# salesforce/ALPRO

Hardware: AMD Instinct MI355X
Metric: video-text pairs/sec (8f x 224^2, 40-tok) (higher is better)
Workload: dtype fp16

## Files before the change

alpro_amd/csrc/common.hpp:

```cpp
#pragma once
#include <hip/hip_runtime.h>
#include <stdint.h>

#include "../../include/alpro_hip.h"

namespace alpro {

typedef float f32x4 __attribute__((ext_vector_type(4)));
typedef uint32_t u32x4 __attribute__((ext_vector_type(4)));
typedef uint32_t u32x2 __attribute__((ext_vector_type(2)));
__device__ __forceinline__ u32x4 mk4(uint32_t a, uint32_t b, uint32_t c, uint32_t d) { return u32x4{a, b, c, d}; }
__device__ __forceinline__ u32x2 mk2(uint32_t a, uint32_t b) { return u32x2{a, b}; }
__device__ __forceinline__ float u2f(uint32_t u) { return __builtin_bit_cast(float, u); }
__device__ __forceinline__ uint32_t f2u(float f) { return __builtin_bit_cast(uint32_t, f); }
typedef float f32x16 __attribute__((ext_vector_type(16)));
typedef __bf16 bf16x8_t __attribute__((ext_vector_type(8)));
typedef _Float16 f16x8_t __attribute__((ext_vector_type(8)));

struct bf16_t { uint16_t v; };
struct f16_t { uint16_t v; };

__device__ __forceinline__ float to_f32(float x) { return x; }
__device__ __forceinline__ float to_f32(bf16_t x) { return __builtin_bit_cast(float, (uint32_t)x.v << 16); }
__device__ __forceinline__ float to_f32(f16_t x) { return (float)__builtin_bit_cast(_Float16, x.v); }
// ... 134 lines not shown
  const f32x2v cdf = {0.5f + copysignf(0.5f - h.x, x.x), 0.5f + copysignf(0.5f - h.y, x.y)};
  y = x * cdf;
  dy = cdf + x * (e * (f32x2v){0.39894228040143267794f, 0.39894228040143267794f});
}

__device__ __forceinline__ f32x2v gelu_fast2(f32x2v x) {
  const f32x2v z = (f32x2v){fabsf(x.x), fabsf(x.y)} * (f32x2v){0.70710678118654752440f, 0.70710678118654752440f};
  f32x2v q = z * (f32x2v){-0.00296695f, -0.00296695f} + (f32x2v){0.02966973f, 0.02966973f};
  q = z * q + (f32x2v){-0.14875628f, -0.14875628f};
  q = z * q + (f32x2v){-0.91847146f, -0.91847146f};
  q = z * q + (f32x2v){-1.62789348f, -1.62789348f};
  q = z * q + (f32x2v){-1.0f, -1.0f};
  const f32x2v h = {__builtin_amdgcn_exp2f(q.x), __builtin_amdgcn_exp2f(q.y)};
  const f32x2v cdf = {0.5f + copysignf(0.5f - h.x, x.x), 0.5f + copysignf(0.5f - h.y, x.y)};
  return x * cdf;
}

template <typename T> __device__ __forceinline__ void gelu_and_grad(float x, float& y, float& dy) {
  if constexpr (sizeof(T) == 4) {
    const float cdf = 0.5f * (1.0f + erff(x * 0.70710678118654752440f));
    y = x * cdf;
    dy = cdf + x * 0.39894228040143267794f * __expf(-0.5f * x * x);
  } else {
    const float h = half_erfc_pos(fabsf(x) * 0.70710678118654752440f);
    const float cdf = 0.5f + copysignf(0.5f - h, x);
    const float pdf = 0.39894228040143267794f * __builtin_amdgcn_exp2f(x * x * -0.72134752044448170368f);
    y = x * cdf;
    dy = cdf + x * pdf;
  }
}

__device__ __forceinline__ uint32_t mix32(uint32_t h) {
  h ^= h >> 16; h *= 0x7FEB352Du; h ^= h >> 15; h *= 0x846CA68Bu; h ^= h >> 16;
  return h;
}
__device__ __forceinline__ bool drop_keep(uint32_t seed, uint64_t idx, uint32_t thresh24) {
  const uint32_t h = mix32(seed ^ ((uint32_t)idx * 0x9E3779B1u) ^ ((uint32_t)(idx >> 32) * 0x85EBCA77u));
  return (h >> 8) >= thresh24;
}
__host__ __device__ inline uint32_t drop_thresh24(float p) { return (uint32_t)(p * 16777216.0f + 0.5f); }

__device__ __forceinline__ void dma16(const void* src, uint32_t lds_addr) {
#pragma clang diagnostic push
#pragma clang diagnostic ignored "-Winline-asm"
  asm volatile("s_mov_b32 m0, %1\n\ts_nop 0\n\tglobal_load_lds_dwordx4 %0, off" ::"v"(src), "s"(lds_addr) : "memory", "m0");
#pragma clang diagnostic pop
}
__device__ __forceinline__ void store16_sc1(void* p, const u32x4& v) {
  asm volatile("global_store_dwordx4 %0, %1, off sc1\n\ts_nop 1" ::"v"(p), "v"(v) : "memory");
}
__device__ __forceinline__ float sload_f32(const float* p, uint32_t idx) {
  return *((const __attribute__((address_space(4))) float*)p + __builtin_amdgcn_readfirstlane(idx));
}
__device__ __forceinline__ uint32_t lds_addr_of(const void* p) { return (uint32_t)(uintptr_t)(__attribute__((address_space(3))) const char*)p; }

void set_error(const char* fmt, ...);
int attn_long_fwd(const void* qkv, void* out, int dtype, int batch, int L, int H, float scale, const float* key_bias, float* lse, float drop_p,
                  uint32_t drop_seed, const float* cls_q, int cls_group, float* cls_out, hipStream_t st);
int attn_long_bwd(const void* qkv, const void* out, const void* dout, const float* lse, void* dqkv, int dtype, int batch, int L, int H, float scale,
                  const float* key_bias, float drop_p, uint32_t drop_seed, hipStream_t st);
int attn_temporal_any_fwd(const void* qkv, void* out, int dtype, int64_t rows, int T, int H, float scale, float* lse, hipStream_t st);
int attn_temporal_any_bwd(const void* qkv, const void* out, const void* dout, const float* lse, void* dqkv, int dtype, int64_t rows, int T, int H,
                          float scale, hipStream_t st);

__device__ __forceinline__ void attn_unit(int blk, int nblk, int H, int order, int& b, int& h) {
  const int batch = nblk / H;
  if (order == 1 && (batch & 7) == 0) {
    const int x = blk & 7, i = blk >> 3, j = i / H;
    h = i - j * H;
    b = j * 8 + x;
  } else {
    b = blk / H;
    h = blk - b * H;
  }
}
enum { OPT_GEMM_TILE = 0, OPT_GEMM_GRID = 1, OPT_GEMM_TUNE = 2, OPT_TN_SPLITS = 3, OPT_TN_KIND = 4, OPT_GEMM_TAIL = 5, OPT_ATTN_BWD = 6, OPT_ATTN_ORDER = 7, OPT_GEMM_KIND = 8, OPT_CU_BUDGET = 9, OPT_LN_GRID = 10, OPT_GEMM_SCHED = 11, OPT_GEMM_EPI = 12, OPT_COUNT = 13 };
int get_option(int which);
int get_stream_option(int which, hipStream_t st);

constexpr int SCHED_CLAIM0 = 8, SCHED_MAX_WG = 256, SCHED_BLOCK_U32 = SCHED_CLAIM0 + SCHED_MAX_WG;
struct TileSched {
  uint32_t* blk;
  uint32_t* prev;
  uint32_t magic_ntn;
  uint32_t epi;
};
struct SchedLaunch {
  uint32_t* cur = nullptr;
  uint32_t* prev = nullptr;
  void* slot = nullptr;
  SchedLaunch(hipStream_t st, bool enabled);
  void commit(bool launched);
  ~SchedLaunch();
};
int sched_set_workspace(hipStream_t st, void* ptr, size_t bytes);
inline uint32_t magic_u32(uint32_t d) { return (uint32_t)(((1ull << 32) + d - 1) / d); }
inline int cu_budget(hipStream_t st) {
  int v = get_stream_option(OPT_CU_BUDGET, st);
  if (v < 0) v = get_option(OPT_CU_BUDGET);
  return (v >= 64 && v < 256) ? (v / 8 * 8) : 256;
}

struct DeviceOnce {
  unsigned long long mask = 0;
  template <typename F> void run(F&& f) {
    int dev = 0;
    (void)hipGetDevice(&dev);
    const unsigned long long bit = 1ull << (dev & 63);
    if (!(__atomic_load_n(&mask, __ATOMIC_ACQUIRE) & bit)) {
      f();
      __atomic_fetch_or(&mask, bit, __ATOMIC_RELEASE);
    }
  }
};
template <typename K> void set_lds_once(DeviceOnce& once, K* kern, size_t lds) {
  once.run([&] { (void)hipFuncSetAttribute((const void*)kern, hipFuncAttributeMaxDynamicSharedMemorySize, (int)lds); });
}
#define ALPRO_CHECK(cond, ...)            \
  do {                                    \
    if (!(cond)) {                        \
      alpro::set_error(__VA_ARGS__);      \
      return ALPRO_ERR_INVALID;           \
    }                                     \
  } while (0)
int check_launch(const char* what);

#define ALPRO_DISPATCH_DTYPE(dt, T, ...)                                         \
  switch (dt) {                                                                  \
    case ALPRO_F32: { typedef float T; __VA_ARGS__; break; }                     \
    case ALPRO_BF16: { typedef alpro::bf16_t T; __VA_ARGS__; break; }            \
    case ALPRO_F16: { typedef alpro::f16_t T; __VA_ARGS__; break; }              \
    default: alpro::set_error("bad dtype %d", (int)(dt)); return ALPRO_ERR_INVALID; \
  }

}
```

alpro_amd/csrc/core.hip:

```cpp
#include <stdarg.h>
#include <stdio.h>
#include <stdlib.h>
#include <string.h>

#include "common.hpp"

namespace alpro {

static thread_local char g_err[512] = "";

void set_error(const char* fmt, ...) {
  va_list ap;
  va_start(ap, fmt);
  vsnprintf(g_err, sizeof(g_err), fmt, ap);
  va_end(ap);
}

namespace {
const char* const kOptNames[OPT_COUNT] = {"gemm_tile", "gemm_grid", "gemm_tune", "tn_splits", "tn_kind", "gemm_tail", "attn_bwd", "attn_order", "gemm_kind", "cu_budget", "ln_grid", "gemm_sched", "gemm_epi"};
const char* const kOptEnv[OPT_COUNT] = {"ALPRO_GEMM_TILE", "ALPRO_GEMM_GRID", "ALPRO_GEMM_TUNE", "ALPRO_TN_SPLITS", "ALPRO_TN_KIND", "ALPRO_GEMM_TAIL", "ALPRO_ATTN_BWD", "ALPRO_ATTN_ORDER", "ALPRO_GEMM_KIND", "ALPRO_CU_BUDGET", "ALPRO_LN_GRID", "ALPRO_GEMM_SCHED", "ALPRO_GEMM_EPI"};
int g_opts[OPT_COUNT];
bool option_allowed(int which, int value) {
#ifdef ALPRO_ABLATIONS
  (void)which; (void)value;
// ... 757 lines not shown
    ALPRO_ADD_LN_CASE(ALPRO_ADD_PRE_MLP)
    ALPRO_ADD_LN_CASE(ALPRO_ADD_PRE_TEMPORAL)
  }
#undef ALPRO_ADD_LN_CASE
  return check_launch("alpro_add_layernorm_fwd");
}
}

extern "C" int alpro_add_layernorm_fwd(const float* x_in, const void* delta, int dtype, const float* delta_bias, int add_mode, float* x_out,
                                       const float* gamma, const float* beta, float eps, void* y, float* y32, int64_t rows, int D, int p0, int p1,
                                       void* stream) {
  ALPRO_CHECK(x_in && delta && gamma && beta && y && rows > 0, "alpro_add_layernorm_fwd: bad args");
  ALPRO_CHECK(D == LN_D, "alpro_add_layernorm_fwd: D=%d unsupported (hidden size is 768 on this path)", D);
  ALPRO_CHECK(add_mode >= ALPRO_ADD_IDENTITY && add_mode <= ALPRO_ADD_PRE_TEMPORAL, "alpro_add_layernorm_fwd: bad add_mode %d", add_mode);
  ALPRO_CHECK(add_mode == ALPRO_ADD_IDENTITY || (p0 > 0 && p1 > 0), "alpro_add_layernorm_fwd: the divided space-time modes need p0 = T, p1 = N");
  ALPRO_CHECK(add_mode == ALPRO_ADD_IDENTITY || rows % (add_mode == ALPRO_ADD_PRE_SPATIAL ? (int64_t)p0 * (p1 + 1) : 1 + (int64_t)p0 * p1) == 0,
              "alpro_add_layernorm_fwd: rows=%lld is not a whole number of clips", (long long)rows);
  ALPRO_CHECK(!(dtype == ALPRO_F32 && y32), "alpro_add_layernorm_fwd: y already is fp32 in exact mode");
  ALPRO_CHECK(((uintptr_t)x_in % 16) == 0 && ((uintptr_t)delta % 16) == 0 && ((uintptr_t)y % 16) == 0, "alpro_add_layernorm_fwd: pointers must be 16-byte aligned");
  ALPRO_DISPATCH_DTYPE(dtype, T, return launch_add_ln<T>(add_mode, x_in, delta, delta_bias, x_out, gamma, beta, eps, y, y32, rows, p0, p1, (hipStream_t)stream));
  return ALPRO_OK;
}

extern "C" int alpro_add_layernorm_pre_mlp2(const float* x_in, const void* delta_t, const float* delta_t_bias, const void* delta_s, int dtype, float* x_out,
                                            const float* gamma, const float* beta, float eps, void* y, int64_t rows, int D, int T, int N, void* stream) {
  ALPRO_CHECK(x_in && delta_t && delta_s && gamma && beta && y && rows > 0, "alpro_add_layernorm_pre_mlp2: bad args");
  ALPRO_CHECK(D == LN_D, "alpro_add_layernorm_pre_mlp2: D=%d unsupported (hidden size is 768 on this path)", D);
  ALPRO_CHECK(T > 0 && N > 0 && rows % (1 + (int64_t)T * N) == 0, "alpro_add_layernorm_pre_mlp2: rows=%lld is not a whole number of clips of 1 + %d x %d tokens", (long long)rows, N, T);
  ALPRO_CHECK(((uintptr_t)x_in % 16) == 0 && ((uintptr_t)delta_t % 16) == 0 && ((uintptr_t)delta_s % 16) == 0 && ((uintptr_t)y % 16) == 0,
              "alpro_add_layernorm_pre_mlp2: pointers must be 16-byte aligned");
  const dim3 grid(grid_for(rows, 4, 256 * 32)), blk(256);
  ALPRO_DISPATCH_DTYPE(dtype, T_, hipLaunchKernelGGL((add_layernorm_fwd_kernel<T_, ALPRO_ADD_PRE_MLP>), grid, blk, 0, (hipStream_t)stream, x_in, (const T_*)delta_s,
                                                     (const float*)nullptr, x_out, gamma, beta, eps, (T_*)y, (float*)nullptr, rows, T, N, (const T_*)delta_t, delta_t_bias));
  return check_launch("alpro_add_layernorm_pre_mlp2");
}

extern "C" int alpro_vit_final_pool(const float* x, const float* gamma, const float* beta, float eps, float* out32, void* out_t,
                                    int dtype, int B, int T, int N, int D, void* stream) {
  ALPRO_CHECK(x && gamma && beta && out32 && B > 0 && T > 0 && N > 0, "alpro_vit_final_pool: bad args");
  ALPRO_CHECK(D == LN_D, "alpro_vit_final_pool: D=%d unsupported", D);
  const int64_t total = (int64_t)B * (N + 1);
  ALPRO_DISPATCH_DTYPE(dtype, T_, hipLaunchKernelGGL(vit_final_pool_kernel<T_>, dim3((unsigned)((total + 3) / 4)), dim3(256), 0, (hipStream_t)stream, x, gamma, beta, eps, out32, (T_*)out_t, B, T, N));
  return check_launch("alpro_vit_final_pool");
}

extern "C" int alpro_bert_embed_fwd(const int64_t* ids, const float* word, const float* pos, const float* type0,
                                    const float* gamma, const float* beta, float eps, float* y32, void* y_t, int dtype,
                                    float* mean, float* rstd, int rows, int L, int D, float drop_p, uint32_t drop_seed, void* stream) {
  ALPRO_CHECK(ids && word && pos && type0 && gamma && beta && y32 && rows > 0 && L > 0, "alpro_bert_embed_fwd: bad args");
  ALPRO_CHECK(D == LN_D, "alpro_bert_embed_fwd: D=%d unsupported", D);
  ALPRO_DISPATCH_DTYPE(dtype, T, hipLaunchKernelGGL(bert_embed_kernel<T>, dim3((rows + 3) / 4), dim3(256), 0, (hipStream_t)stream, ids, word, pos, type0, gamma, beta, eps, y32, (T*)y_t, mean, rstd, rows, L, drop_p, drop_seed));
  return check_launch("alpro_bert_embed_fwd");
}
```

alpro_amd/csrc/gemm.hip:

```cpp
#include <stdarg.h>
#include <stdio.h>
#include <stdlib.h>

#include <type_traits>

#include "common.hpp"

namespace alpro {

namespace {
constexpr int BM = 128, BN = 128, ROWB = 128, NT = 256;
constexpr int TILE_BYTES = BM * ROWB;

__device__ __forceinline__ int lds_off(int row, int chunk) { return row * ROWB + ((chunk ^ ((row >> 1) & 7)) << 4); }

struct RowDst {
  int64_t out, res;
  bool side;
};
template <int mode>
__device__ __forceinline__ RowDst map_row(int p0, int p1, int m) {
  RowDst d;
  d.side = false;
  if (mode == ALPRO_MAP_IDENTITY) {
// ... 227 lines not shown
    }
    if (ACT == ALPRO_ACT_GELU_BWD || ACT == ALPRO_ACT_MUL_SAVED) {
      float pre[8];
      unpack_chunk<T>(pre_c2 ? pre_c2[p] : *(const u32x4*)((const T*)g.C2 + m * g.ldc2 + n), pre);
#pragma unroll
      for (int e = 0; e < 8; ++e) v[e] *= (ACT == ALPRO_ACT_MUL_SAVED) ? pre[e] : gelu_grad<T>(pre[e]);
    }
    if constexpr (ACT == ALPRO_ACT_GELU && sizeof(T) == 2) {
#pragma unroll
      for (int e = 0; e < 8; e += 2) {
        const f32x2v yy = gelu_fast2((f32x2v){v[e], v[e + 1]});
        v[e] = yy.x * rs;
        v[e + 1] = yy.y * rs;
      }
    } else {
#pragma unroll
      for (int e = 0; e < 8; ++e) v[e] = apply_act<T, ACT>(v[e]) * rs;
    }
    if (g.drop_seed) {
      float dp = g.drop_p;
      asm volatile("" : "+s"(dp));
      const uint32_t th = drop_thresh24(dp);
      const float ks = 1.0f / (1.0f - dp);
      const uint64_t i0 = (uint64_t)(g.m_off + m) * (uint64_t)g.N + (uint64_t)n;
#pragma unroll
      for (int e = 0; e < 8; ++e) v[e] = drop_keep(g.drop_seed, i0 + e, th) ? v[e] * ks : 0.f;
    }
    if constexpr (RES) {
      if (g.residual) {
        const f32x4 r0 = __builtin_nontemporal_load((const f32x4*)(g.residual + m * g.ldr + n)), r1 = __builtin_nontemporal_load((const f32x4*)(g.residual + m * g.ldr + n + 4));
        v[0] += r0.x; v[1] += r0.y; v[2] += r0.z; v[3] += r0.w; v[4] += r1.x; v[5] += r1.y; v[6] += r1.z; v[7] += r1.w;
      }
    }
    if (ABL == 1) {
      u32x4 keep = pack_chunk<T>(v);
      asm volatile("" ::"v"(keep));
    } else {
      __builtin_nontemporal_store(pack_chunk<T>(v), (u32x4*)((T*)g.C + m * g.ldc + n));
    }
  }
}

__device__ __forceinline__ bool epi_fast_ok(const alpro_gemm_desc_t& g, int m_base, int rows, int n_base) {
  return (m_base + rows <= g.M) && (n_base + 64 <= g.N) && ((g.ldc & 3) == 0) && (!g.residual || (g.ldr & 3) == 0) &&
         ((g.ld_side & 3) == 0);
}

__device__ __forceinline__ void load_bias4(const alpro_gemm_desc_t& g, int n, float (&bias)[4]) {
#pragma unroll
  for (int e = 0; e < 4; ++e) bias[e] = (g.bias && n + e < g.N) ? g.bias[n + e] : 0.f;
}

template <typename T, int ACT, int MAP>
__device__ __forceinline__ void gemm_nt_tile(const alpro_gemm_desc_t& g, const int bid, char* smem) {
  const int tid = threadIdx.x, lane = tid & 63, wave = tid >> 6;
  const int wr = wave >> 1, wc = wave & 1;
  const int ntn = (g.N + BN - 1) / BN, ntm = (g.M + BM - 1) / BM;
  const int nblk = ntn * ntm;
  if (bid >= nblk) return;
  int tile;
  {
    const int xcd = bid & 7, idx = bid >> 3;
    const int q = nblk >> 3, r = nblk & 7;
    tile = (xcd < r ? xcd * (q + 1) : r * (q + 1) + (xcd - r) * q) + idx;
  }
  const int tm = tile / ntn, tn = tile - tm * ntn;
  const int m0 = tm * BM, n0 = tn * BN;

  const char* Ab = (const char*)g.A;
  const char* Wb = (const char*)g.W;
  const int64_t lda_b = g.lda * (int64_t)sizeof(T), ldw_b = g.ldw * (int64_t)sizeof(T);

  const char* a_src[4];
  const char* w_src[4];
  int st_off[4];
#pragma unroll
  for (int i = 0; i < 4; ++i) {
    const int c = tid + i * NT, row = c >> 3, ch = c & 7;
    const int am = min(m0 + row, g.M - 1), wn = min(n0 + row, g.N - 1);
    a_src[i] = Ab + am * lda_b + ch * 16;
    w_src[i] = Wb + wn * ldw_b + ch * 16;
    st_off[i] = lds_off(row, ch);
  }
  int a_row[2], b_row[2];
#pragma unroll
  for (int i = 0; i < 2; ++i) {
    a_row[i] = wr * 64 + i * 32 + (lane & 31);
    b_row[i] = wc * 64 + i * 32 + (lane & 31);
  }
  const int khalf = lane >> 5;

  f32x16 acc[2][2];
#pragma unroll
  for (int i = 0; i < 2; ++i)
#pragma unroll
    for (int j = 0; j < 2; ++j)
#pragma unroll
      for (int r = 0; r < 16; ++r) acc[i][j][r] = 0.f;

  const int nk = (g.K * (int)sizeof(T)) / ROWB;
  u32x4 ra[4], rw[4];
#pragma unroll
  for (int i = 0; i < 4; ++i) {
    ra[i] = *(const u32x4*)(a_src[i]);
    rw[i] = *(const u32x4*)(w_src[i]);
  }
  char* bufA = smem;
  char* bufW = smem + 2 * TILE_BYTES;
#pragma unroll
  for (int i = 0; i < 4; ++i) {
    *(u32x4*)(bufA + st_off[i]) = ra[i];
    *(u32x4*)(bufW + st_off[i]) = rw[i];
  }
  __syncthreads();

  int cur = 0;
  for (int kt = 0; kt < nk; ++kt) {
    {
      const int64_t ko = (int64_t)min(kt + 1, nk - 1) * ROWB;
#pragma unroll
// ... 5 lines not shown
    __builtin_amdgcn_sched_barrier(0);
    const char* cA = bufA + cur * TILE_BYTES;
    const char* cW = bufW + cur * TILE_BYTES;
#pragma unroll
    for (int s = 0; s < 4; ++s) {
      u32x4 fa[2], fb[2];
#pragma unroll
      for (int i = 0; i < 2; ++i) {
        fa[i] = *(const u32x4*)(cA + lds_off(a_row[i], 2 * s + khalf));
        fb[i] = *(const u32x4*)(cW + lds_off(b_row[i], 2 * s + khalf));
      }
#pragma unroll
      for (int i = 0; i < 2; ++i)
#pragma unroll
        for (int j = 0; j < 2; ++j) mma_chunk<T>(acc[i][j], fa[i], fb[j]);
    }
    __builtin_amdgcn_sched_barrier(0);
    {
      char* nA = bufA + (cur ^ 1) * TILE_BYTES;
      char* nW = bufW + (cur ^ 1) * TILE_BYTES;
#pragma unroll
      for (int i = 0; i < 4; ++i) {
        *(u32x4*)(nA + st_off[i]) = ra[i];
        *(u32x4*)(nW + st_off[i]) = rw[i];
      }
    }
    __syncthreads();
    cur ^= 1;
  }

  float* stage = (float*)(smem + wave * (64 * 64 * 4));
#pragma unroll
  for (int r = 0; r < 16; ++r) {
    const int row = acc_row(r, lane), col = lane & 31;
    stage[row * 64 + col] = acc[0][0][r];
    stage[row * 64 + 32 + col] = acc[0][1][r];
    stage[(32 + row) * 64 + col] = acc[1][0][r];
    stage[(32 + row) * 64 + 32 + col] = acc[1][1][r];
  }
  wave_lds_sync();
  const int mb = m0 + wr * 64, nb = n0 + wc * 64;
  float bias[4];
  load_bias4(g, nb + (lane & 15) * 4, bias);
  if (epi_fast_ok(g, mb, 64, nb)) {
#pragma unroll
    for (int c = 0; c < 4; ++c) epi_rows16<T, ACT, MAP, true>(g, stage + c * 16 * 64, mb + c * 16, nb, lane, bias);
  } else {
#pragma unroll 1
    for (int c = 0; c < 4; ++c) epi_rows16<T, ACT, MAP, false>(g, stage + c * 16 * 64, mb + c * 16, nb, lane, bias);
  }
}

template <typename T, int ACT, int MAP>
__global__ __launch_bounds__(NT, 2) void gemm_nt_kernel(const alpro_gemm_desc_t g) {
  extern __shared__ __attribute__((aligned(16))) char smem[];
  gemm_nt_tile<T, ACT, MAP>(g, blockIdx.x, smem);
}

template <typename T, int ACT, int MAP>
__global__ __launch_bounds__(NT, 2) void gemm_nt_batch_kernel(const alpro_gemm_desc_t* __restrict__ descs) {
  extern __shared__ __attribute__((aligned(16))) char smem[];
  const alpro_gemm_desc_t g = descs[blockIdx.y];
  gemm_nt_tile<T, ACT, MAP>(g, blockIdx.x, smem);
}

constexpr int BM2 = 256, BN2 = 256, NT2 = 512;
constexpr int TILE2_BYTES = BM2 * ROWB;

constexpr int EPI_BYTES = 8 * 16 * 64 * 4;

__device__ __forceinline__ constexpr int copy_slot(int tune, int q, int pos) {
  if (tune == 0) return ((q & 1) && ((q >> 1) & 1) == pos) ? (q >> 2) : -1;
  if (tune == 1 || tune >= 3) { const int r = q - 1 - pos; return (r >= 0 && r < 16 && (r & 1) == 0) ? (r >> 1) : -1; }
  const int r = q - 1 - pos;
  return (r >= 0 && r < 24 && r % 3 == 0) ? r / 3 : -1;
}

template <typename T, int ACT, int MAP, int TUNE = 1>
__global__ __launch_bounds__(NT2, 2) void gemm_nt256p_kernel(const alpro_gemm_desc_t g, const int tail_split) {
  extern __shared__ __attribute__((aligned(16))) char smem[];
  const int tid = threadIdx.x, lane = tid & 63, wave = __builtin_amdgcn_readfirstlane(tid >> 6);
  const int wr = wave >> 2, wc = wave & 3;
  const int ntn = (g.N + BN2 - 1) / BN2, ntm = (g.M + BM2 - 1) / BM2;
  const int nblk = ntn * ntm;
  const int64_t lda_b = g.lda * (int64_t)sizeof(T), ldw_b = g.ldw * (int64_t)sizeof(T);
  const int nk = (g.K * (int)sizeof(T)) / ROWB;
  const int per_xcd = (gridDim.x + 7) >> 3;
  const int slot = (blockIdx.x & 7) * per_xcd + (blockIdx.x >> 3);
  typedef __attribute__((address_space(3))) void* lds_ptr;
  typedef const __attribute__((address_space(1))) void* gbl_ptr;

  const char* a_src[4];
  const char* w_src[4];
  int m0 = 0, n0 = 0;
  const int G = gridDim.x;
  const int q_full = nblk / G, rem = nblk - q_full * G;
  const bool split = tail_split && rem > 0 && 2 * rem <= G;
  auto locate = [&](int it, int& t, int& hf) -> bool {
    hf = -1;
    if (it < q_full) { t = slot + it * G; return true; }
    if (it > q_full) return false;
    if (split) {
      if (slot >= 2 * rem) return false;
      t = q_full * G + (slot >> 1);
      hf = slot & 1;
      return true;
    }
    t = q_full * G + slot;
    return slot < rem;
  };
  auto setup = [&](int tile, int hf) {
    const int tm = tile / ntn, tn = tile - tm * ntn;
    m0 = tm * BM2 + (hf > 0 ? BM2 / 2 : 0);
    n0 = tn * BN2;
#pragma unroll
    for (int i = 0; i < 4; ++i) {
      const int row = (wave + 8 * i) * 8 + (lane >> 3);
      const int ch = (lane & 7) ^ ((row >> 1) & 7);
      a_src[i] = (const char*)g.A + min(m0 + row, g.M - 1) * lda_b + ch * 16;
      w_src[i] = (const char*)g.W + min(n0 + row, g.N - 1) * ldw_b + ch * 16;
    }
  };
  const uint32_t lds_base = lds_addr_of(smem);
  auto copy_piece = [&](int c, int kt, int buf, bool half_a = false) {
    const int i = c >> 1;
    if (half_a && !(c & 1) && i >= 2) return;
    const char* src = ((c & 1) ? w_src[i] : a_src[i]) + (int64_t)kt * ROWB;
    dma16(src, __builtin_amdgcn_readfirstlane(lds_base + buf * 2 * TILE2_BYTES + (c & 1) * TILE2_BYTES + (wave + 8 * i) * 1024));
  };
  auto stage_tile = [&](int kt, int buf, bool half_a = false) {
#pragma unroll
    for (int c = 0; c < 8; ++c) copy_piece(c, kt, buf, half_a);
  };
  int a_row[4], b_row[2];
#pragma unroll
  for (int i = 0; i < 4; ++i) a_row[i] = wr * 128 + i * 32 + (lane & 31);
#pragma unroll
  for (int j = 0; j < 2; ++j) b_row[j] = wc * 64 + j * 32 + (lane & 31);
  const int khalf = lane >> 5;
  float* stage = (float*)(smem + 4 * TILE2_BYTES + wave * (16 * 64 * 4));

  int it = 0, tile, hf;
  if (!locate(0, tile, hf)) return;
  const int pos = wave >> 2;
  auto wait_vm0 = [] { asm volatile("s_waitcnt vmcnt(0)" ::: "memory"); };
  auto block_sync = [] {
    asm volatile("s_waitcnt lgkmcnt(0)" ::: "memory");
    __builtin_amdgcn_s_barrier();
    asm volatile("" ::: "memory");
  };
  setup(tile, hf);
  int s0 = 0;
  stage_tile(0, 0, hf >= 0);
  stage_tile(1, 1, hf >= 0);
  wait_vm0();
  while (true) {
    const int tm0 = m0, tn0 = n0;
    int next, next_hf;
    const bool more = locate(it + 1, next, next_hf);
    const bool active = hf < 0 || wr == 0;
    f32x16 acc[4][2];
#pragma unroll
    for (int i = 0; i < 4; ++i)
#pragma unroll
      for (int j = 0; j < 2; ++j)
// ... 139 lines not shown
      }
    }
    if (!more) break;
    tile = next;
    hf = next_hf;
    ++it;
    setup(tile, hf);
  }
}


static bool q_kernel_takes(const alpro_gemm_desc_t& g, bool* ragged_in_kernel) {
  constexpr int BM2q = 256, BN2q = 256;
  if (g.dtype == ALPRO_F32 || g.map_mode != ALPRO_MAP_IDENTITY) return false;
  const int m_full = g.M / BM2q * BM2q, m_rem = g.M - m_full;
  const bool c16 = g.c_dtype != ALPRO_F32 && (g.ldc & 7) == 0 && (!g.C2 || g.c2_tiled || (g.ldc2 & 7) == 0) && (!g.residual || (g.ldr & 3) == 0) && ((uintptr_t)g.C % 16) == 0 &&
                   (!g.row_scale || g.row_scale_group >= 8);
  const bool c32 = g.c_dtype == ALPRO_F32 && g.act == ALPRO_ACT_NONE && !g.C2 && !g.drop_seed && (g.ldc & 3) == 0 && (!g.residual || ((g.ldr & 3) == 0 && ((uintptr_t)g.residual % 16) == 0)) &&
                   ((uintptr_t)g.C % 16) == 0 && (!g.row_scale || g.row_scale_group >= 16);
  const bool shape = (g.N % BN2q) == 0 && ((g.lda * 2) % 128) == 0 && ((g.ldw * 2) % 128) == 0 && (g.K % 128) == 0 && g.K >= 256 &&
                     (int64_t)g.M * g.lda * 2 < (int64_t)0xFFFF0000 && (int64_t)g.N * g.ldw * 2 < (int64_t)0xFFFF0000;
  *ragged_in_kernel = m_rem > 0 && (m_rem % 16) == 0;
  const int full_tiles = (g.N / BN2q) * (m_full / BM2q);
  const int force = get_option(OPT_GEMM_TILE);
  return get_option(OPT_GEMM_KIND) == 1 && (c16 || c32) && shape && (force ? force == 256 : full_tiles >= 160);
}
static bool c2_tiled_ok(const alpro_gemm_desc_t& g) {
  const int m_rem = g.M % 256;
  return (g.act == ALPRO_ACT_GELU_SAVE_GRAD || g.act == ALPRO_ACT_MUL_SAVED) && g.C2 && ((uintptr_t)g.C2 % 16) == 0 && g.c_dtype != ALPRO_F32 && !g.residual && !g.row_scale &&
         !g.drop_seed && (m_rem % 16) == 0;
}

constexpr int HALF2_BYTES = 128 * ROWB;
constexpr int STAGE2_BYTES = 4 * HALF2_BYTES;

template <typename T> struct Mma16;
template <> struct Mma16<bf16_t> {
  static __device__ __forceinline__ f32x4 run(const u32x4& a, const u32x4& b, const f32x4& c) {
    return __builtin_amdgcn_mfma_f32_16x16x32_bf16(__builtin_bit_cast(bf16x8_t, a), __builtin_bit_cast(bf16x8_t, b), c, 0, 0, 0);
  }
};
template <> struct Mma16<f16_t> {
  static __device__ __forceinline__ f32x4 run(const u32x4& a, const u32x4& b, const f32x4& c) {
    return __builtin_amdgcn_mfma_f32_16x16x32_f16(__builtin_bit_cast(f16x8_t, a), __builtin_bit_cast(f16x8_t, b), c, 0, 0, 0);
  }
};

template <typename T, int ACT, int MAP>
__global__ __launch_bounds__(NT2, 2) __attribute__((amdgpu_num_vgpr(127))) void gemm_nt256q_kernel(const alpro_gemm_desc_t g, const TileSched sc) {
  static_assert(sizeof(T) == 2, "16-bit operands only");
  extern __shared__ __attribute__((aligned(16))) char smem[];
  const int tid = threadIdx.x, lane = tid & 63, wave = __builtin_amdgcn_readfirstlane(tid >> 6);
  const int wr = wave >> 2, wc = wave & 3;
  const int ntn = (g.N + BN2 - 1) / BN2, ntm = (g.M + BM2 - 1) / BM2;
  const int nblk = ntn * ntm;
  const int64_t lda_b = g.lda * 2, ldw_b = g.ldw * 2;
  const int nk = g.K >> 6;
  const uint32_t lds_base = lds_addr_of(smem);

  const uint32_t p = gridDim.x >> 3;
  const uint64_t t_start = wall_clock64();
  constexpr uint32_t RESCUE_TICKS = 1000;
  auto list_tile = [&](int y, uint32_t j) -> int {
    const uint32_t t = ((j >> 5) << 8) + ((uint32_t)y << 5) + (j & 31u);
    return (j < 0x100000u && t < (uint32_t)nblk) ? (int)t : -1;
  };
  auto list_len = [&](int y) -> int {
    const int rem = (nblk & 255) - 32 * y;
    return (nblk >> 8) * 32 + (rem < 0 ? 0 : (rem > 32 ? 32 : rem));
  };
  typedef __attribute__((address_space(3))) volatile int lds_int_t;
  lds_int_t* mbox = (lds_int_t*)(__attribute__((address_space(3))) char*)(smem + STAGE2_BYTES + HALF2_BYTES);
  uint32_t wstate = sc.blk ? 0u : (uint32_t)(blockIdx.x >> 3) + 2 * p;
  int quota = 0;
  bool pending = false;
  if (sc.blk) {
    const int mine = list_len((int)(blockIdx.x & 7u)) - (int)(2 * p);
    quota = mine > 0 ? (mine + (int)p - 1) / (int)p : 0;
  }
  auto ticket_issue = [&](uint32_t& r, bool on) {
    uint64_t sv;
    const uint32_t m = (uint32_t)__builtin_amdgcn_readfirstlane(on ? 1 : 0);
    asm volatile("s_mov_b64 %1, exec\n\ts_mov_b32 exec_lo, %5\n\ts_mov_b32 exec_hi, 0\n\tglobal_atomic_add %0, %2, %3, %4 sc0\n\ts_mov_b64 exec, %1"
                 : "+v"(r), "=&s"(sv) : "v"(((blockIdx.x + wstate) & 7u) * 4u), "v"(1u), "s"(sc.blk), "s"(m) : "memory");
  };
  auto claim_issue = [&](uint32_t& r, uint32_t w, uint32_t bits, bool on) {
    uint64_t sv;
    const uint32_t m = (uint32_t)__builtin_amdgcn_readfirstlane(on ? 1 : 0);
    asm volatile("s_mov_b64 %1, exec\n\ts_mov_b32 exec_lo, %5\n\ts_mov_b32 exec_hi, 0\n\tglobal_atomic_or %0, %2, %3, %4 sc0\n\ts_mov_b64 exec, %1"
                 : "+v"(r), "=&s"(sv) : "v"((SCHED_CLAIM0 + w) * 4u), "v"(bits), "s"(sc.blk), "s"(m) : "memory");
  };
  auto ticket_issue_tk = [&](bool on) {
    uint64_t sv;
    const uint32_t m = (uint32_t)__builtin_amdgcn_readfirstlane(on ? 1 : 0);
#pragma clang diagnostic push
#pragma clang diagnostic ignored "-Winline-asm"
    asm volatile("s_mov_b64 %0, exec\n\ts_mov_b32 exec_lo, %4\n\ts_mov_b32 exec_hi, 0\n\tglobal_atomic_add v255, %1, %2, %3 sc0\n\ts_mov_b64 exec, %0"
                 : "=&s"(sv) : "v"(((blockIdx.x + wstate) & 7u) * 4u), "v"(1u), "s"(sc.blk), "s"(m) : "memory", "v255");
#pragma clang diagnostic pop
  };
  auto claim_issue_tk = [&](uint32_t w, uint32_t bits, bool on) {
    uint64_t sv;
    const uint32_t m = (uint32_t)__builtin_amdgcn_readfirstlane(on ? 1 : 0);
#pragma clang diagnostic push
#pragma clang diagnostic ignored "-Winline-asm"
    asm volatile("s_mov_b64 %0, exec\n\ts_mov_b32 exec_lo, %4\n\ts_mov_b32 exec_hi, 0\n\tglobal_atomic_or v255, %1, %2, %3 sc0\n\ts_mov_b64 exec, %0"
                 : "=&s"(sv) : "v"((SCHED_CLAIM0 + w) * 4u), "v"(bits), "s"(sc.blk), "s"(m) : "memory", "v255");
// ... 37 lines not shown
          asm volatile("s_waitcnt vmcnt(0)" ::: "memory");
          a = list_tile(y, 2 * p + __builtin_amdgcn_readfirstlane(k0));
          continue;
        }
        const uint32_t w0 = 4u * lane;
        const uint32_t words[4] = {clm.x, clm.y, clm.z, clm.w};
        uint64_t open[8];
        int total = 0;
#pragma unroll
        for (int sl = 0; sl < 8; ++sl) {
          open[sl] = __builtin_amdgcn_ballot_w64(w0 + (sl >> 1) < gridDim.x && ((words[sl >> 1] >> (sl & 1)) & 1u) == 0u);
          total += __builtin_popcountll(open[sl]);
        }
        if (total == 0) break;
        while ((uint32_t)(wall_clock64() - t_start) < RESCUE_TICKS) __builtin_amdgcn_s_sleep(8);
        int q = (int)(((blockIdx.x + 1u) * 0x9E3779B1u >> 12) % (uint32_t)total);
        uint32_t w = 0, bit = 0;
#pragma unroll
        for (int sl = 0; sl < 8; ++sl) {
          const int n = __builtin_popcountll(open[sl]);
          if (bit == 0 && q < n) {
            uint64_t msk = open[sl];
            for (int i = 0; i < q; ++i) msk &= msk - 1;
            w = 4u * (uint32_t)__builtin_ctzll(msk) + (uint32_t)(sl >> 1);
            bit = 1u << (sl & 1);
          }
          q -= n;
        }
        uint32_t old = 3;
        claim_issue(old, w, bit, true);
        asm volatile("s_waitcnt vmcnt(0)" ::: "memory");
        if ((__builtin_amdgcn_readfirstlane(old) & bit) == 0) a = list_tile((int)(w & 7u), (w >> 3) + (bit == 2u ? p : 0u));
      }
      const int b = -1;
      mbox[0] = a;
      mbox[1] = b;
    }
    asm volatile("s_waitcnt lgkmcnt(0)" ::: "memory");
    __builtin_amdgcn_s_barrier();
    asm volatile("" ::: "memory");
    t0 = __builtin_amdgcn_readfirstlane(mbox[0]);
    t1 = __builtin_amdgcn_readfirstlane(mbox[1]);
  };

  const int r0 = wave * 16 + (lane >> 3);
  const uint32_t sw0 = (uint32_t)(((lane & 7) ^ ((r0 >> 1) & 7)) << 4);
  uint32_t oa[2], ow[2][2];
#pragma unroll
  for (int i = 0; i < 2; ++i) {
    oa[i] = (uint32_t)((r0 + i * 8) * lda_b) + (sw0 ^ (uint32_t)(i * 64));
#pragma unroll
    for (int h = 0; h < 2; ++h) ow[h][i] = (uint32_t)((r0 + h * 128 + i * 8) * ldw_b) + (sw0 ^ (uint32_t)(i * 64));
  }
  struct Tile { const char* a[2]; const char* w; };
  auto tile_base = [&](int tile) {
    const int tm = ntn == 1 ? tile : (int)__umulhi((uint32_t)tile, sc.magic_ntn), tn = tile - tm * ntn;
    const int vr = g.M - tm * BM2;
    const char* a0 = (const char*)g.A + (int64_t)tm * BM2 * lda_b;
    Tile t;
#pragma unroll
    for (int h = 0; h < 2; ++h) t.a[h] = a0 + (int64_t)((h * 128 + wave * 16 < vr) ? h * 128 : -(wave * 16)) * lda_b;
    t.w = (const char*)g.W + (int64_t)tn * BN2 * ldw_b;
    return t;
  };
  auto copy_half = [&](const char* kbase, int hs, int par) {
#pragma unroll
    for (int i = 0; i < 2; ++i) {
      const uint32_t vo = hs < 2 ? oa[i] : ow[hs & 1][i];
      const uint32_t dst = __builtin_amdgcn_readfirstlane(lds_base + par * STAGE2_BYTES + hs * HALF2_BYTES + (wave * 2 + i) * 1024);
#pragma clang diagnostic push
#pragma clang diagnostic ignored "-Winline-asm"
      asm volatile("s_mov_b32 m0, %2\n\ts_nop 0\n\tglobal_load_lds_dwordx4 %0, %1" ::"v"(vo), "s"(kbase), "s"(dst) : "memory", "m0");
#pragma clang diagnostic pop
    }
  };
  const int l15 = lane & 15, kg = lane >> 4;
  const int frag0 = l15 * ROWB + ((kg ^ ((l15 >> 1) & 7)) << 4);
  const char* aF[2] = {smem + wr * HALF2_BYTES + frag0, smem + wr * HALF2_BYTES + (frag0 ^ 64)};
  const char* bF[2] = {smem + (2 + (wc >> 1)) * HALF2_BYTES + (wc & 1) * 64 * ROWB + frag0,
                       smem + (2 + (wc >> 1)) * HALF2_BYTES + (wc & 1) * 64 * ROWB + (frag0 ^ 64)};
  float* stage = (float*)(smem + 2 * STAGE2_BYTES + wave * (16 * 64 * 4));

  auto barrier = [] {
    __builtin_amdgcn_sched_barrier(0);
    __builtin_amdgcn_s_barrier();
    __builtin_amdgcn_sched_barrier(0);
  };

  int cur_t = list_tile((int)(blockIdx.x & 7u), blockIdx.x >> 3), nxt_t = list_tile((int)(blockIdx.x & 7u), (blockIdx.x >> 3) + p);
  if (sc.prev && blockIdx.x == 0 && wave == 0) {
#pragma unroll
    for (int i = 0; i < (SCHED_BLOCK_U32 + 63) / 64; ++i)
      if (i * 64 + lane < SCHED_BLOCK_U32) sc.prev[i * 64 + lane] = 0u;
  }
  claim_issue_tk(blockIdx.x, 3u, wave == 0 && sc.blk);
  bool fresh = sc.blk != nullptr;
  bool have = cur_t >= 0;
  while (true) {
  if (!have) {
    if (!sc.blk) break;
    fresh = false;
    asm volatile("s_waitcnt vmcnt(0)" ::: "memory");
    steal(cur_t, nxt_t);
    if (cur_t < 0) break;
    quota = 0;
  }
  have = false;
  Tile cur = tile_base(cur_t);
  Tile nxt = tile_base(nxt_t >= 0 ? nxt_t : cur_t);
#pragma unroll
  for (int hs = 0; hs < 4; ++hs) copy_half(hs < 2 ? cur.a[hs] : cur.w, hs, 0);
  copy_half(cur.w + ROWB, 2, 1);
  asm volatile("s_waitcnt vmcnt(0)" ::: "memory");
  if (fresh && wave == 0) {
    mbox[0] = (int)(tk_read() & 3u);
    asm volatile("s_waitcnt lgkmcnt(0)" ::: "memory");
  }
  barrier();
  if (fresh) {
    fresh = false;
    const int gone = __builtin_amdgcn_readfirstlane(mbox[0]);
    if (gone) {
      barrier();
      int t0 = (gone & 1) ? -1 : cur_t, t1 = (gone & 2) ? -1 : nxt_t;
      if (t0 < 0) { t0 = t1; t1 = -1; }
      cur_t = t0;
      nxt_t = t1;
      have = cur_t >= 0;
      continue;
    }
  }
  pending = sc.blk && nxt_t >= 0 && quota > 0;
  quota -= pending ? 1 : 0;
  ticket_issue_tk(wave == 0 && pending);

  while (true) {
    const int tile = cur_t;
    const int tm0 = (ntn == 1 ? tile : (int)__umulhi((uint32_t)tile, sc.magic_ntn)) * BM2, tn0 = (tile - (tm0 >> 8) * ntn) * BN2;
    f32x4 acc[8][4];
#pragma unroll
    for (int i = 0; i < 8; ++i)
#pragma unroll
      for (int j = 0; j < 4; ++j) acc[i][j] = f32x4{0.f, 0.f, 0.f, 0.f};
    if (wr == 1) barrier();

    auto ktile = [&](auto par_tag, int t) {
      constexpr int P = decltype(par_tag)::value;
      u32x4 fa[4][2], fb[2][2][2];
      const bool in1 = t + 1 < nk, in2 = t + 2 < nk;
      const int k1 = in1 ? t + 1 : 0, k2 = in2 ? t + 2 : t + 2 - nk;
      const char* a10 = (in1 ? cur.a[0] : nxt.a[0]) + (int64_t)k1 * ROWB;
      const char* a11 = (in1 ? cur.a[1] : nxt.a[1]) + (int64_t)k1 * ROWB;
      const char* w1 = (in1 ? cur.w : nxt.w) + (int64_t)k1 * ROWB;
      const char* w2 = (in2 ? cur.w : nxt.w) + (int64_t)k2 * ROWB;
      auto load_a = [&](int mi) {
#pragma unroll
        for (int f = 0; f < 4; ++f)
#pragma unroll
          for (int ks = 0; ks < 2; ++ks) fa[f][ks] = *(const u32x4*)(aF[ks] + P * STAGE2_BYTES + (mi * 64 + f * 16) * ROWB);
      };
      auto load_b = [&](int ni) {
#pragma unroll
        for (int f = 0; f < 2; ++f)
#pragma unroll
          for (int ks = 0; ks < 2; ++ks) fb[ni][f][ks] = *(const u32x4*)(bF[ks] + P * STAGE2_BYTES + (ni * 32 + f * 16) * ROWB);
      };
      auto mma = [&](int mi, int ni) {
        __builtin_amdgcn_s_setprio(1);
#pragma unroll
        for (int ks = 0; ks < 2; ++ks)
#pragma unroll
          for (int f = 0; f < 4; ++f)
#pragma unroll
            for (int e = 0; e < 2; ++e) acc[mi * 4 + f][ni * 2 + e] = Mma16<T>::run(fa[f][ks], fb[ni][e][ks], acc[mi * 4 + f][ni * 2 + e]);
        __builtin_amdgcn_s_setprio(0);
      };
      load_b(0);
      load_a(0);
      copy_half(a10, 0, P ^ 1);
      barrier();
      mma(0, 0);
      barrier();
      load_b(1);
      copy_half(a11, 1, P ^ 1);
      barrier();
      mma(0, 1);
      barrier();
      load_a(1);
      copy_half(w1, 3, P ^ 1);
      barrier();
      mma(1, 1);
// ... 207 lines not shown
            for (int mf = 0; mf < 8; ++mf) {
              if (!rows_ok(mf)) break;
              if constexpr (HAS_RES) {
                if (mf + PD < 8 && rows_ok(mf + PD)) load_res(mf + PD, ring[(mf + PD) % RING]);
              }
              float rs_lo = 1.0f, rs_hi = 1.0f;
              uint32_t edge = 0;
              if (g.row_scale) {
                const uint32_t m0 = (uint32_t)g.m_off + (uint32_t)(mb + mf * 16);
                const uint32_t gi = (uint32_t)__builtin_amdgcn_readfirstlane((int)(m0 / (uint32_t)g.row_scale_group));
                edge = (gi + 1) * (uint32_t)g.row_scale_group;
                rs_lo = sload_f32(g.row_scale, gi);
                rs_hi = sload_f32(g.row_scale, edge < (uint32_t)g.m_off + (uint32_t)g.M ? gi + 1 : gi);
              }
              stage_rows(mf);
#pragma unroll
              for (int j = 0; j < 4; ++j) {
                const int row = r0e + 4 * j;
                const int64_t m = mb + mf * 16 + row;
                const float4 a = *(const float4*)(stage + row * 64 + c4);
                const float rs = ((uint32_t)g.m_off + (uint32_t)m) >= edge ? rs_hi : rs_lo;
                f32x4 v = {(g.alpha * a.x + bias4[0]) * rs, (g.alpha * a.y + bias4[1]) * rs, (g.alpha * a.z + bias4[2]) * rs, (g.alpha * a.w + bias4[3]) * rs};
                if constexpr (HAS_RES) v += ring[mf % RING][j];
                __builtin_nontemporal_store(v, (f32x4*)(Cf + m * g.ldc + nb + c4));
              }
              if constexpr (!HAS_RES) {
                if (mf == 0) early_ticket();
              }
            }
          };
          if (g.residual) f32_rows(std::true_type{});
          else f32_rows(std::false_type{});
        }
      }
    }
    if (nxt_t < 0) break;
    cur = nxt;
    cur_t = nxt_t;
    nxt_t = __builtin_amdgcn_readfirstlane(mbox[0]);
    nxt = tile_base(nxt_t >= 0 ? nxt_t : cur_t);
    if (!early) {
      pending = sc.blk && nxt_t >= 0 && quota > 0;
      quota -= pending ? 1 : 0;
      ticket_issue_tk(wave == 0 && pending);
    }
  }
  asm volatile("s_waitcnt vmcnt(0)" ::: "memory");
  cur_t = -1;
  }
  asm volatile("s_waitcnt vmcnt(0)" ::: "memory");
}

template <typename T, int ACT, int MAP>
int launch_gemm_inst(const alpro_gemm_desc_t& g, hipStream_t st) {
  static DeviceOnce attr_once;
  attr_once.run([&] {
    (void)hipFuncSetAttribute((const void*)gemm_nt_kernel<T, ACT, MAP>, hipFuncAttributeMaxDynamicSharedMemorySize, 4 * TILE_BYTES);
    (void)hipFuncSetAttribute((const void*)gemm_nt256p_kernel<T, ACT, MAP>, hipFuncAttributeMaxDynamicSharedMemorySize, 4 * TILE2_BYTES + EPI_BYTES);
    if constexpr (std::is_same<T, bf16_t>::value && ACT == ALPRO_ACT_NONE && MAP == ALPRO_MAP_IDENTITY) {
      (void)hipFuncSetAttribute((const void*)gemm_nt256p_kernel<T, ACT, MAP, 1>, hipFuncAttributeMaxDynamicSharedMemorySize, 4 * TILE2_BYTES + EPI_BYTES);
      (void)hipFuncSetAttribute((const void*)gemm_nt256p_kernel<T, ACT, MAP, 2>, hipFuncAttributeMaxDynamicSharedMemorySize, 4 * TILE2_BYTES + EPI_BYTES);
#ifdef ALPRO_ABLATIONS
      (void)hipFuncSetAttribute((const void*)gemm_nt256p_kernel<T, ACT, MAP, 3>, hipFuncAttributeMaxDynamicSharedMemorySize, 4 * TILE2_BYTES + EPI_BYTES);
      (void)hipFuncSetAttribute((const void*)gemm_nt256p_kernel<T, ACT, MAP, 4>, hipFuncAttributeMaxDynamicSharedMemorySize, 4 * TILE2_BYTES + EPI_BYTES);
      (void)hipFuncSetAttribute((const void*)gemm_nt256p_kernel<T, ACT, MAP, 12>, hipFuncAttributeMaxDynamicSharedMemorySize, 4 * TILE2_BYTES + EPI_BYTES);
      (void)hipFuncSetAttribute((const void*)gemm_nt256p_kernel<T, ACT, MAP, 11>, hipFuncAttributeMaxDynamicSharedMemorySize, 4 * TILE2_BYTES + EPI_BYTES);
      (void)hipFuncSetAttribute((const void*)gemm_nt256p_kernel<T, ACT, MAP, 10>, hipFuncAttributeMaxDynamicSharedMemorySize, 4 * TILE2_BYTES + EPI_BYTES);
      (void)hipFuncSetAttribute((const void*)gemm_nt256p_kernel<T, ACT, MAP, 5>, hipFuncAttributeMaxDynamicSharedMemorySize, 4 * TILE2_BYTES + EPI_BYTES);
      (void)hipFuncSetAttribute((const void*)gemm_nt256p_kernel<T, ACT, MAP, 6>, hipFuncAttributeMaxDynamicSharedMemorySize, 4 * TILE2_BYTES + EPI_BYTES);
#endif
    }
  });
  const int big_tiles = ((g.N + BN2 - 1) / BN2) * ((g.M + BM2 - 1) / BM2);
  const int force = get_option(OPT_GEMM_TILE);
  const int nk = (g.K * (int)sizeof(T)) / ROWB;
  const bool use256 = nk >= 2 && (force ? force == 256 : big_tiles >= 160);
  if constexpr (sizeof(T) == 2 && MAP == ALPRO_MAP_IDENTITY) {
    static DeviceOnce attr_q;
    attr_q.run([&] {
      (void)hipFuncSetAttribute((const void*)gemm_nt256q_kernel<T, ACT, MAP>, hipFuncAttributeMaxDynamicSharedMemorySize, 2 * STAGE2_BYTES + EPI_BYTES);
    });
    const int m_full = g.M / BM2 * BM2, m_rem = g.M - m_full;
    bool ragged_in_kernel = false;
    const bool take_q = q_kernel_takes(g, &ragged_in_kernel);
    ALPRO_CHECK(!g.c2_tiled || (take_q && c2_tiled_ok(g)), "alpro_gemm: c2_tiled is not available for this descriptor (M=%d N=%d K=%d act=%d): ask alpro_gemm_c2_tiled_rows first", g.M, g.N, g.K, g.act);
    if (take_q) {
      alpro_gemm_desc_t gq = g;
      if (!ragged_in_kernel) gq.M = m_full;
      int grid = cu_budget(st);
      if (const int cap = get_option(OPT_GEMM_GRID)) grid = cap < grid ? (cap + 7) / 8 * 8 : grid;
      const int ntn_q = g.N / BN2, ntm_q = (gq.M + BM2 - 1) / BM2;
      const int tiles = ntn_q * ntm_q;
      int tail_panels = 0;
      if (get_option(OPT_GEMM_TAIL) == 1 && !g.c2_tiled && tiles > grid && g.K >= 2048) {
        const int R = tiles % grid;
        if (R > 0 && 5 * R <= 2 * grid) tail_panels = (R + ntn_q - 1) / ntn_q;
      }
      int64_t m_tail0 = -1;
      if (tail_panels > 0 && tail_panels < ntm_q) {
        m_tail0 = (int64_t)(ntm_q - tail_panels) * BM2;
        gq.M = (int)m_tail0;
      } else if (m_rem && !ragged_in_kernel) {
        m_tail0 = m_full;
      }
      TileSched sc;
      sc.blk = sc.prev = nullptr;
      sc.magic_ntn = magic_u32((uint32_t)(g.N / BN2));
      sc.epi = (uint32_t)get_option(OPT_GEMM_EPI);
      {
        SchedLaunch blocks(get_option(OPT_GEMM_SCHED) == 1 ? st : nullptr, get_option(OPT_GEMM_SCHED) == 1);
        sc.blk = blocks.cur;
        sc.prev = blocks.prev;
        hipLaunchKernelGGL((gemm_nt256q_kernel<T, ACT, MAP>), dim3(grid), dim3(NT2), 2 * STAGE2_BYTES + EPI_BYTES, st, gq, sc);
        blocks.commit(hipPeekAtLastError() == hipSuccess);
      }
      if (m_tail0 >= 0) {
        alpro_gemm_desc_t gr = g;
        gr.M = (int)(g.M - m_tail0);
        gr.A = (const char*)g.A + m_tail0 * g.lda * 2;
        gr.C = (char*)g.C + m_tail0 * g.ldc * (g.c_dtype == ALPRO_F32 ? 4 : 2);
        gr.m_off = g.m_off + m_tail0;
        if (g.C2) gr.C2 = (char*)g.C2 + m_tail0 * g.ldc2 * 2;
        if (g.residual) gr.residual = g.residual + m_tail0 * g.ldr;
        const int ntn = (gr.N + BN - 1) / BN, ntm = (gr.M + BM - 1) / BM;
        hipLaunchKernelGGL((gemm_nt_kernel<T, ACT, MAP>), dim3(ntn * ntm), dim3(NT), 4 * TILE_BYTES, st, gr);
      }
      return check_launch("alpro_gemm");
    }
  }
  if (use256) {
    const int cus = cu_budget(st);
    int grid = big_tiles < cus ? (big_tiles + 7) / 8 * 8 : cus;
    if (const int cap = get_option(OPT_GEMM_GRID)) grid = cap < grid ? (cap + 7) / 8 * 8 : grid;
    const int tune = get_option(OPT_GEMM_TUNE);
    const int tail = get_option(OPT_GEMM_TAIL);
    if constexpr (std::is_same<T, bf16_t>::value && ACT == ALPRO_ACT_NONE && MAP == ALPRO_MAP_IDENTITY) {
      if (tune == 0) { hipLaunchKernelGGL((gemm_nt256p_kernel<T, ACT, MAP, 0>), dim3(grid), dim3(NT2), 4 * TILE2_BYTES + EPI_BYTES, st, g, tail); return check_launch("alpro_gemm"); }
      if (tune == 2) { hipLaunchKernelGGL((gemm_nt256p_kernel<T, ACT, MAP, 2>), dim3(grid), dim3(NT2), 4 * TILE2_BYTES + EPI_BYTES, st, g, tail); return check_launch("alpro_gemm"); }
#ifdef ALPRO_ABLATIONS
      if (tune == 3) { hipLaunchKernelGGL((gemm_nt256p_kernel<T, ACT, MAP, 3>), dim3(grid), dim3(NT2), 4 * TILE2_BYTES + EPI_BYTES, st, g, tail); return check_launch("alpro_gemm"); }
      if (tune == 4) { hipLaunchKernelGGL((gemm_nt256p_kernel<T, ACT, MAP, 4>), dim3(grid), dim3(NT2), 4 * TILE2_BYTES + EPI_BYTES, st, g, tail); return check_launch("alpro_gemm"); }
      if (tune == 12) { hipLaunchKernelGGL((gemm_nt256p_kernel<T, ACT, MAP, 12>), dim3(grid), dim3(NT2), 4 * TILE2_BYTES + EPI_BYTES, st, g, tail); return check_launch("alpro_gemm"); }
      if (tune == 11) { hipLaunchKernelGGL((gemm_nt256p_kernel<T, ACT, MAP, 11>), dim3(grid), dim3(NT2), 4 * TILE2_BYTES + EPI_BYTES, st, g, tail); return check_launch("alpro_gemm"); }
      if (tune == 10) { hipLaunchKernelGGL((gemm_nt256p_kernel<T, ACT, MAP, 10>), dim3(grid), dim3(NT2), 4 * TILE2_BYTES + EPI_BYTES, st, g, tail); return check_launch("alpro_gemm"); }
      if (tune == 5) { hipLaunchKernelGGL((gemm_nt256p_kernel<T, ACT, MAP, 5>), dim3(grid), dim3(NT2), 4 * TILE2_BYTES + EPI_BYTES, st, g, tail); return check_launch("alpro_gemm"); }
      if (tune == 6) { hipLaunchKernelGGL((gemm_nt256p_kernel<T, ACT, MAP, 6>), dim3(grid), dim3(NT2), 4 * TILE2_BYTES + EPI_BYTES, st, g, tail); return check_launch("alpro_gemm"); }
#endif
    }
    hipLaunchKernelGGL((gemm_nt256p_kernel<T, ACT, MAP>), dim3(grid), dim3(NT2), 4 * TILE2_BYTES + EPI_BYTES, st, g, tail);
  } else {
    const int ntn = (g.N + BN - 1) / BN, ntm = (g.M + BM - 1) / BM;
    hipLaunchKernelGGL((gemm_nt_kernel<T, ACT, MAP>), dim3(ntn * ntm), dim3(NT), 4 * TILE_BYTES, st, g);
  }
  return check_launch("alpro_gemm");
}

template <typename T>
int launch_gemm(const alpro_gemm_desc_t& g, hipStream_t st) {
#ifdef ALPRO_ISA_QUICK
  return g.act == ALPRO_ACT_MUL_SAVED ? launch_gemm_inst<T, ALPRO_ACT_MUL_SAVED, ALPRO_MAP_IDENTITY>(g, st) : launch_gemm_inst<T, ALPRO_ACT_NONE, ALPRO_MAP_IDENTITY>(g, st);
#else
  if (g.act != ALPRO_ACT_NONE) {
    if (g.map_mode != ALPRO_MAP_IDENTITY) {
      set_error("alpro_gemm: an activation cannot be combined with a row map");
      return ALPRO_ERR_INVALID;
    }
    if (g.act == ALPRO_ACT_GELU_BWD) return launch_gemm_inst<T, ALPRO_ACT_GELU_BWD, ALPRO_MAP_IDENTITY>(g, st);
    if (g.act == ALPRO_ACT_GELU_SAVE_GRAD) return launch_gemm_inst<T, ALPRO_ACT_GELU_SAVE_GRAD, ALPRO_MAP_IDENTITY>(g, st);
    if (g.act == ALPRO_ACT_MUL_SAVED) return launch_gemm_inst<T, ALPRO_ACT_MUL_SAVED, ALPRO_MAP_IDENTITY>(g, st);
    return g.act == ALPRO_ACT_GELU ? launch_gemm_inst<T, ALPRO_ACT_GELU, ALPRO_MAP_IDENTITY>(g, st)
                                   : launch_gemm_inst<T, ALPRO_ACT_RELU, ALPRO_MAP_IDENTITY>(g, st);
  }
  switch (g.map_mode) {
    case ALPRO_MAP_IDENTITY: return launch_gemm_inst<T, ALPRO_ACT_NONE, ALPRO_MAP_IDENTITY>(g, st);
    case ALPRO_MAP_SKIP_CLS: return launch_gemm_inst<T, ALPRO_ACT_NONE, ALPRO_MAP_SKIP_CLS>(g, st);
    case ALPRO_MAP_FRAME_TOKENS: return launch_gemm_inst<T, ALPRO_ACT_NONE, ALPRO_MAP_FRAME_TOKENS>(g, st);
    default: return launch_gemm_inst<T, ALPRO_ACT_NONE, ALPRO_MAP_PATCH_EMBED>(g, st);
  }
#endif
}
}
}

namespace alpro {
namespace {
template <typename T>
int launch_gemm_batch(const alpro_gemm_desc_t* descs_dev, int njobs, int max_tiles, int with_residual_map, hipStream_t st) {
  (void)with_residual_map;
  static DeviceOnce attr_once;
  attr_once.run([&] {
    (void)hipFuncSetAttribute((const void*)gemm_nt_batch_kernel<T, ALPRO_ACT_NONE, ALPRO_MAP_IDENTITY>, hipFuncAttributeMaxDynamicSharedMemorySize, 4 * TILE_BYTES);
  });
  hipLaunchKernelGGL((gemm_nt_batch_kernel<T, ALPRO_ACT_NONE, ALPRO_MAP_IDENTITY>), dim3(max_tiles, njobs), dim3(NT), 4 * TILE_BYTES, st, descs_dev);
  return check_launch("alpro_gemm_batch");
}
}
}

static int check_gemm_desc(const alpro_gemm_desc_t* d);

extern "C" int alpro_gemm_batch(const alpro_gemm_desc_t* descs_host, const alpro_gemm_desc_t* descs_device, int njobs, void* stream) {
  using namespace alpro;
  ALPRO_CHECK(descs_host && descs_device && njobs > 0, "alpro_gemm_batch: bad args");
  int max_tiles = 0;
  for (int i = 0; i < njobs; ++i) {
    const alpro_gemm_desc_t* d = descs_host + i;
    if (const int rc = check_gemm_desc(d)) return rc;
    ALPRO_CHECK(d->dtype == descs_host[0].dtype, "alpro_gemm_batch: all jobs must share the operand dtype");
    ALPRO_CHECK(d->act == ALPRO_ACT_NONE && d->map_mode == ALPRO_MAP_IDENTITY && !d->drop_seed && !d->bias2 && !d->C2,
                "alpro_gemm_batch: plain epilogues only (bias, alpha, row scale, fp32 residual)");
    const int t = ((d->N + BN - 1) / BN) * ((d->M + BM - 1) / BM);
    max_tiles = t > max_tiles ? t : max_tiles;
  }
  ALPRO_DISPATCH_DTYPE(descs_host[0].dtype, T, return launch_gemm_batch<T>(descs_device, njobs, max_tiles, 0, (hipStream_t)stream));
  return ALPRO_OK;
}

static int check_gemm_desc(const alpro_gemm_desc_t* d) {
  using namespace alpro;
  ALPRO_CHECK(d && d->A && d->W && d->C, "alpro_gemm: null operand");
  ALPRO_CHECK(d->M > 0 && d->N > 0 && d->K > 0, "alpro_gemm: bad shape M=%d N=%d K=%d", d->M, d->N, d->K);
  const int esz = d->dtype == ALPRO_F32 ? 4 : 2;
  ALPRO_CHECK((d->K * esz) % 128 == 0, "alpro_gemm: K=%d must be a multiple of %d for dtype %d", d->K, 128 / esz, d->dtype);
  ALPRO_CHECK((d->lda * esz) % 16 == 0 && (d->ldw * esz) % 16 == 0, "alpro_gemm: lda/ldw must keep rows 16-byte aligned");
  ALPRO_CHECK(((uintptr_t)d->A % 16) == 0 && ((uintptr_t)d->W % 16) == 0, "alpro_gemm: A/W must be 16-byte aligned");
  ALPRO_CHECK(d->c_dtype == d->dtype || d->c_dtype == ALPRO_F32, "alpro_gemm: c_dtype must be dtype or F32");
  ALPRO_CHECK(d->map_mode >= 0 && d->map_mode <= 3, "alpro_gemm: bad map_mode %d", d->map_mode);
  ALPRO_CHECK(d->act >= 0 && d->act <= ALPRO_ACT_MUL_SAVED, "alpro_gemm: bad act %d", d->act);
  ALPRO_CHECK(!d->bias2 || d->map_mode == ALPRO_MAP_SKIP_CLS, "alpro_gemm: bias2 is only defined under the SKIP_CLS map");
  ALPRO_CHECK((d->act != ALPRO_ACT_GELU_BWD && d->act != ALPRO_ACT_MUL_SAVED && d->act != ALPRO_ACT_GELU_SAVE_GRAD) || (d->C2 && d->N % 8 == 0 && (d->c2_tiled || d->ldc2 % 8 == 0)),
              "alpro_gemm: GELU_BWD / MUL_SAVED / GELU_SAVE_GRAD need the C2 buffer (N, ldc2 multiples of 8)");
  ALPRO_CHECK(!d->drop_seed || (d->map_mode == ALPRO_MAP_IDENTITY && d->drop_p > 0.f && d->drop_p < 1.f), "alpro_gemm: dropout needs the identity map and 0 < p < 1");
  ALPRO_CHECK(!d->C2 || (d->N % 4 == 0 && (d->c2_tiled || d->ldc2 % 4 == 0) && d->ldc % 4 == 0), "alpro_gemm: C2 needs N, ldc, ldc2 multiples of 4");
  ALPRO_CHECK(!d->c2_tiled || d->act == ALPRO_ACT_GELU_SAVE_GRAD || d->act == ALPRO_ACT_MUL_SAVED, "alpro_gemm: c2_tiled is for GELU_SAVE_GRAD / MUL_SAVED only");
  ALPRO_CHECK(d->map_mode != ALPRO_MAP_FRAME_TOKENS || d->side, "alpro_gemm: FRAME_TOKENS needs a side buffer");
  ALPRO_CHECK(!d->row_scale || d->row_scale_group > 0, "alpro_gemm: row_scale_group must be > 0");
  return ALPRO_OK;
}

extern "C" int64_t alpro_gemm_c2_tiled_rows(int64_t M, int64_t N, int64_t K, int dtype) {
  using namespace alpro;
  if (M <= 0 || N <= 0 || K <= 0 || M > 0x7fffffff || N > 0x7fffffff || K > 0x7fffffff || (dtype != ALPRO_F16 && dtype != ALPRO_BF16)) return 0;
  alpro_gemm_desc_t g = {};
  g.A = g.W = (const void*)(uintptr_t)256;
  g.C = g.C2 = (void*)(uintptr_t)256;
  g.M = (int)M; g.N = (int)N; g.K = (int)K;
  g.lda = g.ldw = K; g.ldc = N;
  g.dtype = g.c_dtype = dtype;
  g.act = ALPRO_ACT_GELU_SAVE_GRAD;
  g.c2_tiled = 1;
  bool ragged = false;
  return (q_kernel_takes(g, &ragged) && c2_tiled_ok(g)) ? (M + 255) / 256 * 256 : 0;
}

extern "C" int alpro_gemm(const alpro_gemm_desc_t* d, void* stream) {
  using namespace alpro;
  if (const int rc = check_gemm_desc(d)) return rc;
#ifdef ALPRO_ISA_QUICK
  return launch_gemm<f16_t>(*d, (hipStream_t)stream);
#else
  ALPRO_DISPATCH_DTYPE(d->dtype, T, return launch_gemm<T>(*d, (hipStream_t)stream));
  return ALPRO_OK;
#endif
}
```

alpro_amd/csrc/gemm_tn.hip:

```cpp
#include "common.hpp"

namespace alpro {
namespace {

constexpr int TM = 32;
constexpr int NSTAGE = 4;
constexpr int TW = 256;
constexpr int ROW_BYTES = TW * 2;
constexpr int IMG_BYTES = TM * ROW_BYTES;
constexpr int NT3 = 512;

__device__ u32x4 g_zero_page[4];

typedef short s16x4 __attribute__((ext_vector_type(4)));

__device__ __forceinline__ u32x2 tr4(const char* img, int m0, int colblk16, int lane) {
  const int p = lane & 15;
  const int row = m0 + (p >> 2);
  const int chunk = (colblk16 << 1) | ((p >> 1) & 1);
  const char* a = img + row * ROW_BYTES + ((chunk ^ ((row & 3) << 2)) << 4) + ((p & 1) << 3);
  const s16x4 r = __builtin_amdgcn_ds_read_tr16_b64_v4i16((__attribute__((address_space(3))) s16x4*)a);
  return __builtin_bit_cast(u32x2, r);
}
__device__ __forceinline__ u32x4 frag8(const char* img, int ks, int col0, int lane) {
  const int g = lane >> 5;
  const int blk = (col0 >> 4) + ((lane >> 4) & 1);
  const u32x2 a = tr4(img, ks * 16 + 4 * g, blk, lane);
  const u32x2 b = tr4(img, ks * 16 + 8 + 4 * g, blk, lane);
  const uint32_t ax = a.x, ay = a.y, bx = b.x, by = b.y;
  return mk4(ax, ay, bx, by);
}

template <typename T, int PP = 0>
__global__ __launch_bounds__(NT3, 1) void gemm_tn_kernel(const T* __restrict__ A, int64_t lda, const T* __restrict__ B, int64_t ldb,
                                                         float* __restrict__ C, int64_t ldc, int M, int N, int K, int per,
                                                         int tiles, int units, int tn_cnt, float* __restrict__ colsum, float* __restrict__ part,
                                                         float* __restrict__ part_cs, int ablate) {
  extern __shared__ __attribute__((aligned(16))) char smem[];
  const int tid = threadIdx.x, lane = tid & 63, wave = __builtin_amdgcn_readfirstlane(tid >> 6);
  const int wr = wave >> 2, wc = wave & 3;
  const int upx = (units + 7) >> 3;
  const int unit = (blockIdx.x & 7) * upx + (blockIdx.x >> 3);
  if (unit >= units) return;
  const int range = unit / tiles, tile = unit - range * tiles;
  const int total_steps = (M + TM - 1) / TM;
  const int s0 = range * per, s1 = min(s0 + per, total_steps);
  const int n0 = (tile % tn_cnt) * TW, k0 = (tile / tn_cnt) * TW;
  if (s0 >= s1) return;

  const char* zero = (const char*)g_zero_page;
  const int rows_end = min(s1 * TM, M);
  const char* curA[2];
  const char* curB[2];
  int mrow[2];
  int64_t strA[2], strB[2];
#pragma unroll
  for (int i = 0; i < 2; ++i) {
    const int row = (wave + 8 * i) * 2 + (lane >> 5);
    const int col = ((lane & 31) ^ ((row & 3) << 2)) * 8;
    const int64_t m = (int64_t)s0 * TM + row;
    const bool ca = n0 + col < N, cb = k0 + col < K;
    mrow[i] = s0 * TM + row;
    curA[i] = ca ? (const char*)(A + m * lda + n0 + col) : zero;
    curB[i] = cb ? (const char*)(B + m * ldb + k0 + col) : zero;
    strA[i] = ca ? (int64_t)TM * lda * (int64_t)sizeof(T) : 0;
    strB[i] = cb ? (int64_t)TM * ldb * (int64_t)sizeof(T) : 0;
  }
  const uint32_t lds_base = (uint32_t)(uintptr_t)(__attribute__((address_space(3))) char*)smem;
  const uint32_t lds_piece[2] = {lds_base + wave * 1024u, lds_base + (wave + 8) * 1024u};
  auto copy = [&](int d, int buf) {
    const int i = d >> 1;
    const char* src = (d & 1) ? curB[i] : curA[i];
    src = mrow[i] < rows_end ? src : zero;
    dma16(src, __builtin_amdgcn_readfirstlane(lds_piece[i] + buf * 2 * IMG_BYTES + (d & 1) * IMG_BYTES));
  };
  auto advance = [&](int i) {
    curA[i] += strA[i];
    curB[i] += strB[i];
    mrow[i] += TM;
  };

  f32x16 acc[4][2];
#pragma unroll
  for (int i = 0; i < 4; ++i)
#pragma unroll
    for (int j = 0; j < 2; ++j)
#pragma unroll
      for (int r = 0; r < 16; ++r) acc[i][j][r] = 0.f;

  if constexpr (PP == 0) {
#pragma unroll
    for (int p = 0; p < 3; ++p) {
#pragma unroll
      for (int d = 0; d < 4; ++d) copy(d, p);
      advance(0);
      advance(1);
    }
    copy(0, 3);
    copy(1, 3);
    advance(0);
  } else {
#pragma unroll
    for (int p = 0; p < 2; ++p) {
#pragma unroll
      for (int d = 0; d < 4; ++d) copy(d, p);
      advance(0);
      advance(1);
    }
    copy(0, 2);
    copy(1, 2);
    advance(0);
  }
  [[maybe_unused]] const int pos = wave >> 2;
  auto load_frags = [&](u32x4* fa, u32x4* fb, const char* cA, const char* cB, int ks) {
#pragma unroll
    for (int j = 0; j < 2; ++j) fb[j] = frag8(cB, ks, wc * 64 + j * 32, lane);
#pragma unroll
    for (int i = 0; i < 4; ++i) fa[i] = frag8(cA, ks, wr * 128 + i * 32, lane);
  };
  const int tk_cnt = tiles / tn_cnt, tk = tile / tn_cnt;
  const bool do_cs = colsum != nullptr;
  int cs_turn = s0 % tk_cnt;
  float cs = 0.f;
  auto add_cols = [&](const u32x4* fa) {
#pragma unroll
    for (int i = 0; i < 4; ++i)
      if (i == wc) {
        float f[8];
        unpack_chunk<T>(fa[i], f);
        cs += ((f[0] + f[1]) + (f[2] + f[3])) + ((f[4] + f[5]) + (f[6] + f[7]));
      }
  };
// ... 208 lines not shown
  if (forced > 0) {
    p.ranges = forced;
  } else {
    const double set_us = (ws ? 0.4e-6 : 1.14e-6) * 4.0 * (double)N * (double)K;
    double best_t = 1e30;
    for (int r = 1; r <= 256; ++r) {
      const int per_try = (p.total_steps + r - 1) / r;
      if (per_try < 4 && r > 1) break;
      const double t = (double)(((long)p.tiles * r + cus - 1) / cus) * (26.0 + 1.15 * per_try) + set_us * r + (ws && r > 1 ? 6.0 : 0.0);
      if (t < best_t * 0.98) { best_t = t; p.ranges = r; }
    }
  }
  p.per = (p.total_steps + p.ranges - 1) / p.ranges;
  p.ranges = (p.total_steps + p.per - 1) / p.per;
  p.units = p.ranges * p.tiles;
  p.part_floats = p.ranges > 1 ? (size_t)p.units * TW * TW : 0;
  p.cs_floats = (ws || p.ranges > 1) ? (size_t)p.ranges * (p.tiles / p.tn) * p.tn * TW : 0;
  return p;
}
}

extern "C" size_t alpro_gemm_tn_workspace_bytes(int M, int N, int K) {
  if (M <= 0 || N <= 0 || K <= 0) return 0;
  struct Memo { int M, N, K, forced; size_t bytes; };
  static Memo memo[64];
  static int n_memo = 0, lock = 0;
  const int forced = get_option(OPT_TN_SPLITS);
  while (__atomic_exchange_n(&lock, 1, __ATOMIC_ACQUIRE)) {}
  for (int i = 0; i < n_memo; ++i)
    if (memo[i].M == M && memo[i].N == N && memo[i].K == K && memo[i].forced == forced) {
      const size_t b = memo[i].bytes;
      __atomic_store_n(&lock, 0, __ATOMIC_RELEASE);
      return b;
    }
  __atomic_store_n(&lock, 0, __ATOMIC_RELEASE);
  size_t best = 0;
  for (int cus = 64; cus <= 256; cus += 8) {
    const TnPlan p = tn_plan(M, N, K, true, cus);
    const size_t b = (p.part_floats + p.cs_floats) * sizeof(float);
    best = b > best ? b : best;
  }
  while (__atomic_exchange_n(&lock, 1, __ATOMIC_ACQUIRE)) {}
  if (n_memo < 64) memo[n_memo++] = Memo{M, N, K, forced, best};
  __atomic_store_n(&lock, 0, __ATOMIC_RELEASE);
  return best;
}

extern "C" int alpro_gemm_tn_ranges(int M, int N, int K, int compute_units) {
  if (M <= 0 || N <= 0 || K <= 0) return 0;
  const int cus = (compute_units >= 64 && compute_units < 256) ? compute_units / 8 * 8 : 256;
  return tn_plan(M, N, K, true, cus).ranges;
}

extern "C" int alpro_gemm_tn_acc_ws(const void* A, int64_t lda, const void* B, int64_t ldb, float* C, int64_t ldc, int dtype, int M, int N,
                                    int K, float* colsum, void* workspace, size_t workspace_bytes, void* stream) {
  ALPRO_CHECK(A && B && C && M > 0 && N > 0 && K > 0, "alpro_gemm_tn_acc: bad args");
  ALPRO_CHECK(dtype == ALPRO_BF16 || dtype == ALPRO_F16, "alpro_gemm_tn_acc: 16-bit operands only (fp32 mode uses alpro_transpose + alpro_gemm)");
  ALPRO_CHECK(lda % 8 == 0 && ldb % 8 == 0 && lda >= (N + 7) / 8 * 8 && ldb >= (K + 7) / 8 * 8,
              "alpro_gemm_tn_acc: lda/ldb must be multiples of 8 covering N/K rounded up to 8 (16-byte chunks are read whole)");
  ALPRO_CHECK(((uintptr_t)A % 16) == 0 && ((uintptr_t)B % 16) == 0, "alpro_gemm_tn_acc: operands must be 16-byte aligned");
  const bool ws = workspace != nullptr;
  const TnPlan p = tn_plan(M, N, K, ws, cu_budget((hipStream_t)stream));
  float* part = nullptr;
  float* part_cs = nullptr;
  if (ws) {
    ALPRO_CHECK(((uintptr_t)workspace % 16) == 0 && workspace_bytes >= (p.part_floats + p.cs_floats) * sizeof(float),
                "alpro_gemm_tn_acc_ws: workspace must be 16-byte aligned and hold alpro_gemm_tn_workspace_bytes(M, N, K) bytes");
    part = p.ranges > 1 ? (float*)workspace : nullptr;
    part_cs = colsum ? (float*)workspace + p.part_floats : nullptr;
  }
  const int kind_opt = get_option(OPT_TN_KIND);
  const bool pp = kind_opt == 2;
#ifdef ALPRO_ABLATIONS
  const int kind = kind_opt == 1 ? 1 : 0;
#else
  const int kind = 0;
#endif
  const unsigned grid = (unsigned)((p.units + 7) / 8 * 8);
  const size_t lds = (size_t)NSTAGE * 2 * IMG_BYTES;
  hipStream_t st = (hipStream_t)stream;
  if (dtype == ALPRO_BF16) {
    static DeviceOnce once;
    once.run([&] {
      (void)hipFuncSetAttribute((const void*)gemm_tn_kernel<bf16_t, 0>, hipFuncAttributeMaxDynamicSharedMemorySize, (int)lds);
      (void)hipFuncSetAttribute((const void*)gemm_tn_kernel<bf16_t, 1>, hipFuncAttributeMaxDynamicSharedMemorySize, (int)lds);
    });
    if (pp) hipLaunchKernelGGL((gemm_tn_kernel<bf16_t, 1>), dim3(grid), dim3(NT3), lds, st, (const bf16_t*)A, lda, (const bf16_t*)B, ldb, C, ldc, M, N, K, p.per, p.tiles, p.units, p.tn, colsum, part, part_cs, kind);
    else hipLaunchKernelGGL((gemm_tn_kernel<bf16_t, 0>), dim3(grid), dim3(NT3), lds, st, (const bf16_t*)A, lda, (const bf16_t*)B, ldb, C, ldc, M, N, K, p.per, p.tiles, p.units, p.tn, colsum, part, part_cs, kind);
  } else {
    static DeviceOnce once;
    once.run([&] {
      (void)hipFuncSetAttribute((const void*)gemm_tn_kernel<f16_t, 0>, hipFuncAttributeMaxDynamicSharedMemorySize, (int)lds);
      (void)hipFuncSetAttribute((const void*)gemm_tn_kernel<f16_t, 1>, hipFuncAttributeMaxDynamicSharedMemorySize, (int)lds);
    });
    if (pp) hipLaunchKernelGGL((gemm_tn_kernel<f16_t, 1>), dim3(grid), dim3(NT3), lds, st, (const f16_t*)A, lda, (const f16_t*)B, ldb, C, ldc, M, N, K, p.per, p.tiles, p.units, p.tn, colsum, part, part_cs, kind);
    else hipLaunchKernelGGL((gemm_tn_kernel<f16_t, 0>), dim3(grid), dim3(NT3), lds, st, (const f16_t*)A, lda, (const f16_t*)B, ldb, C, ldc, M, N, K, p.per, p.tiles, p.units, p.tn, colsum, part, part_cs, kind);
  }
  if ((part || part_cs) && kind != 1)
    hipLaunchKernelGGL(tn_reduce_kernel, dim3((part ? p.tiles * 64 : 0) + (part_cs ? p.tn * (TW / 32) : 0)), dim3(256), 0, st, part, part_cs, C, ldc, colsum, N, K, p.tiles, p.ranges, p.tn);
  return check_launch("alpro_gemm_tn_acc");
}

extern "C" int alpro_gemm_tn_acc(const void* A, int64_t lda, const void* B, int64_t ldb, float* C, int64_t ldc, int dtype, int M, int N,
                                 int K, float* colsum, void* stream) {
  return alpro_gemm_tn_acc_ws(A, lda, B, ldb, C, ldc, dtype, M, N, K, colsum, nullptr, 0, stream);
}

extern "C" int alpro_colsum_acc(const void* A, int64_t lda, float* out, int dtype, int M, int N, void* stream) {
  ALPRO_CHECK(A && out && M > 0 && N > 0, "alpro_colsum_acc: bad args");
  const int esz = dtype == ALPRO_F32 ? 4 : 2;
  ALPRO_CHECK((N * esz) % 16 == 0 && (lda * esz) % 16 == 0, "alpro_colsum_acc: rows must be 16-byte multiples");
  ALPRO_DISPATCH_DTYPE(dtype, T, hipLaunchKernelGGL(colsum_kernel<T>, dim3((N + 64 * Chunk<T>::N - 1) / (64 * Chunk<T>::N), (M + 255) / 256), dim3(256), 0, (hipStream_t)stream, (const T*)A, lda, out, M, N));
  return check_launch("alpro_colsum_acc");
}
```

alpro_amd/hip.py:

```python
import ctypes
import os

import torch

_HERE = os.path.dirname(os.path.abspath(__file__))
LIB_PATH = os.environ.get("ALPRO_HIP_LIB") or os.path.join(_HERE, "lib", "libalpro_hip.so")

F32, BF16, F16 = 0, 1, 2
ACT_NONE, ACT_GELU, ACT_RELU, ACT_GELU_BWD, ACT_GELU_SAVE_GRAD, ACT_MUL_SAVED, ACT_RELU_MASK = 0, 1, 2, 3, 4, 5, 6
POOL_MODES = {"mean": 0, "max": 1, "lse": 2}
MAP_IDENTITY, MAP_SKIP_CLS, MAP_FRAME_TOKENS, MAP_PATCH_EMBED = 0, 1, 2, 3
ADD_IDENTITY, ADD_PRE_SPATIAL, ADD_PRE_MLP, ADD_PRE_TEMPORAL = 0, 1, 2, 3
EMIT_NONE, EMIT_ROWS, EMIT_FRAME, EMIT_SKIP_CLS = 0, 1, 2, 3

_TORCH_DTYPE = {F32: torch.float32, BF16: torch.bfloat16, F16: torch.float16}
_CODE = {v: k for k, v in _TORCH_DTYPE.items()}

EXPORTS = ["alpro_hip_last_error", "alpro_hip_abi_version", "alpro_hip_set_option", "alpro_hip_set_stream_option", "alpro_gemm", "alpro_gemm_c2_tiled_rows", "alpro_layernorm_fwd",
           "alpro_attn_temporal_fwd", "alpro_attn_fwd", "alpro_patchify", "alpro_cls_mean_residual",
           "alpro_vit_final_pool", "alpro_bert_embed_fwd", "alpro_cast_from_f32", "alpro_attn_bwd", "alpro_attn_temporal_bwd",
           "alpro_layernorm_bwd", "alpro_transpose", "alpro_transpose_batch", "alpro_gelu_bwd", "alpro_cls_mean_bwd", "alpro_scatter_add_rows", "alpro_gather_cast", "alpro_sumsq", "alpro_adamw_step", "alpro_gemm_tn_acc", "alpro_gemm_tn_acc_ws", "alpro_gemm_tn_workspace_bytes", "alpro_gemm_tn_ranges", "alpro_colsum_acc", "alpro_softmax_xent", "alpro_vtc_loss_fwd", "alpro_vtc_loss_bwd", "alpro_prepare_clips", "alpro_loss_scale_update", "alpro_add_layernorm_fwd", "alpro_layernorm_bwd_emit", "alpro_gemm_batch", "alpro_tproj_small", "alpro_attn_cls_fwd", "alpro_gemm_rows_f32", "alpro_gather_seq_fwd", "alpro_gather_seq_bwd", "alpro_scatter_add_rows_ordered",
           "alpro_hip_sched_workspace_bytes", "alpro_hip_set_sched_workspace", "alpro_hip_release_stream", "alpro_gemm_qkv_tattn", "alpro_add_layernorm_pre_mlp2", "alpro_adamw_step_lp",
           "alpro_gemm_rows_f32_relu_mask", "alpro_clip_pool"]


class GemmDesc(ctypes.Structure):
    _fields_ = [("A", ctypes.c_void_p), ("W", ctypes.c_void_p), ("C", ctypes.c_void_p),
                ("lda", ctypes.c_int64), ("ldw", ctypes.c_int64), ("ldc", ctypes.c_int64),
                ("M", ctypes.c_int), ("N", ctypes.c_int), ("K", ctypes.c_int),
                ("dtype", ctypes.c_int), ("c_dtype", ctypes.c_int), ("alpha", ctypes.c_float),
                ("bias", ctypes.c_void_p), ("act", ctypes.c_int),
                ("row_scale", ctypes.c_void_p), ("row_scale_group", ctypes.c_int),
                ("residual", ctypes.c_void_p), ("ldr", ctypes.c_int64),
                ("map_mode", ctypes.c_int), ("map_p0", ctypes.c_int), ("map_p1", ctypes.c_int),
                ("side", ctypes.c_void_p), ("ld_side", ctypes.c_int64),
                ("C2", ctypes.c_void_p), ("ldc2", ctypes.c_int64),
                ("drop_p", ctypes.c_float), ("drop_seed", ctypes.c_uint32), ("bias2", ctypes.c_void_p), ("m_off", ctypes.c_int64),
                ("c2_tiled", ctypes.c_int32), ("reserved0", ctypes.c_int32)]


class TprojJob(ctypes.Structure):
    _fields_ = [("wfc", ctypes.c_void_p), ("bp", ctypes.c_void_p), ("b1", ctypes.c_void_p), ("db1", ctypes.c_void_p), ("g_fc", ctypes.c_void_p),
                ("g_bp", ctypes.c_void_p)]


class TransposeJob(ctypes.Structure):
    _fields_ = [("in_", ctypes.c_void_p), ("out", ctypes.c_void_p), ("ld_in", ctypes.c_int64), ("ld_out", ctypes.c_int64),
                ("R", ctypes.c_int32), ("C", ctypes.c_int32), ("Rpad", ctypes.c_int32), ("tile0", ctypes.c_int32)]


ABI_VERSION = 22
_lib = None


def load():
    global _lib
    if _lib is not None:
        return _lib
    hq = os.environ.get("GPU_MAX_HW_QUEUES")
    if hq and hq.isdigit() and int(hq) > 4 and any(os.environ.get(k, "1") != "0" for k in ("ALPRO_WGRAD_STREAM", "ALPRO_TEXT_STREAM", "ALPRO_PROMPTER_STREAM")):
        import warnings
        warnings.warn("alpro_amd: GPU_MAX_HW_QUEUES=%s -- with more than 4 hardware queues the training step's side streams (ALPRO_WGRAD_STREAM / "
                      "ALPRO_TEXT_STREAM / ALPRO_PROMPTER_STREAM) measured 11 %% SLOWER than with the runtime's default of 4 (profiles/r6_hw_queues.txt): "
                      "a fifth queue shares a dispatch pipe with the launch stream's" % hq)
    if not os.path.exists(LIB_PATH):
        raise RuntimeError("libalpro_hip.so not found at %s -- run `python -m alpro_amd.build` "
                           "(there is no CPU fallback for the ALPRO hot path)" % LIB_PATH)
    lib = ctypes.CDLL(LIB_PATH)
    lib.alpro_hip_last_error.restype = ctypes.c_char_p
    for name in EXPORTS:
        getattr(lib, name)
    vp, i32, i64, f32 = ctypes.c_void_p, ctypes.c_int, ctypes.c_int64, ctypes.c_float
    lib.alpro_gemm.argtypes = [ctypes.POINTER(GemmDesc), vp]
    lib.alpro_gemm_batch.argtypes = [ctypes.POINTER(GemmDesc), vp, ctypes.c_int, vp]
    lib.alpro_tproj_small.argtypes = [vp, ctypes.c_int, ctypes.c_int, ctypes.c_int, vp]
    lib.alpro_layernorm_fwd.argtypes = [vp, i64, vp, vp, f32, vp, i32, i64, vp, vp, vp, i32, i32, i32, i32, i32, vp]
    lib.alpro_add_layernorm_fwd.argtypes = [vp, vp, i32, vp, i32, vp, vp, vp, f32, vp, vp, i64, i32, i32, i32, vp]
    lib.alpro_attn_temporal_fwd.argtypes = [vp, vp, i32, i64, i32, i32, f32, vp, vp]
    u32 = ctypes.c_uint32
    lib.alpro_attn_bwd.argtypes = [vp, vp, vp, vp, vp, i32, i32, i32, i32, f32, vp, f32, u32, vp]
    lib.alpro_attn_temporal_bwd.argtypes = [vp, vp, vp, vp, vp, i32, i64, i32, i32, f32, vp]
    lib.alpro_layernorm_bwd.argtypes = [vp, i32, i64, vp, vp, i64, vp, f32, vp, i64, i32, vp, vp, i32, i32, i32, i32, i32, f32, u32, vp, ctypes.c_size_t, vp]
    lib.alpro_layernorm_bwd_emit.argtypes = [vp, i32, i64, vp, vp, i64, vp, f32, vp, i64, i32, vp, vp, i32, i32, i32, i32, i32, f32, u32,
                                             vp, i32, i32, i32, i32, vp, i32, f32, u32, vp, i32, vp, ctypes.c_size_t, vp]
    lib.alpro_transpose.argtypes = [vp, i32, i64, vp, i32, i64, i32, i32, i32, vp, vp]
    lib.alpro_gelu_bwd.argtypes = [vp, vp, vp, i32, i64, vp]
    lib.alpro_sumsq.argtypes = [vp, i64, vp, vp, ctypes.c_size_t, vp]
    lib.alpro_softmax_xent.argtypes = [vp, i64, vp, i32, vp, vp, i32, i64, vp, i32, i32, i32, vp]
    lib.alpro_gemm_tn_acc.argtypes = [vp, i64, vp, i64, vp, i64, i32, i32, i32, i32, vp, vp]
    lib.alpro_gemm_tn_acc_ws.argtypes = [vp, i64, vp, i64, vp, i64, i32, i32, i32, i32, vp, vp, ctypes.c_size_t, vp]
    lib.alpro_gemm_tn_workspace_bytes.argtypes = [i32, i32, i32]
    lib.alpro_gemm_tn_workspace_bytes.restype = ctypes.c_size_t
    lib.alpro_gemm_tn_ranges.argtypes = [i32, i32, i32, i32]
    lib.alpro_colsum_acc.argtypes = [vp, i64, vp, i32, i32, i32, vp]
    lib.alpro_transpose_batch.argtypes = [vp, i32, i32, i32, vp]
    lib.alpro_adamw_step.argtypes = [vp, vp, vp, vp, i64, f32, f32, f32, f32, f32, f32, vp, f32, f32, vp, i32, i32, i32, vp]
    lib.alpro_adamw_step_lp.argtypes = [vp, vp, vp, vp, i64, f32, f32, f32, f32, f32, f32, vp, f32, f32, vp, i32, i32, i32, vp, i32, vp]
    lib.alpro_loss_scale_update.argtypes = [vp, vp, f32, f32, i32, f32, f32, vp]
    lib.alpro_gather_cast.argtypes = [vp, i64, vp, i32, i32, i32, i32, i32, i32, vp, i32, f32, f32, u32, vp, vp, vp, ctypes.c_size_t, vp]
    lib.alpro_cls_mean_bwd.argtypes = [vp, i64, vp, i32, i32, i32, vp]
    lib.alpro_scatter_add_rows.argtypes = [vp, vp, vp, i32, i32, i32, i64, vp]
    lib.alpro_attn_fwd.argtypes = [vp, vp, i32, i32, i32, i32, f32, vp, vp, f32, u32, vp, i32, vp, vp]
    lib.alpro_attn_cls_fwd.argtypes = [vp, i32, vp, vp, vp, i32, i32, i32, i32, f32, f32, u32, vp]
    lib.alpro_gemm_rows_f32.argtypes = [vp, i64, vp, i64, vp, i64, i32, i32, i32, vp, i32, vp, vp, i64, vp, vp, f32, vp]
    lib.alpro_gemm_rows_f32_relu_mask.argtypes = [vp, i64, vp, i64, vp, i64, i32, i32, i32, vp, i64, vp]
    lib.alpro_clip_pool.argtypes = [vp, i64, vp, i64, vp, i32, i32, i32, i32, vp]
    lib.alpro_gemm_c2_tiled_rows.argtypes = [i64, i64, i64, i32]
    lib.alpro_gemm_c2_tiled_rows.restype = i64
    lib.alpro_patchify.argtypes = [vp, vp, i32, i32, i32, i32, i32, vp]
    lib.alpro_cls_mean_residual.argtypes = [vp, i64, vp, vp, i64, i32, i32, i32, vp]
    lib.alpro_vit_final_pool.argtypes = [vp, vp, vp, f32, vp, vp, i32, i32, i32, i32, i32, vp]
    lib.alpro_add_layernorm_pre_mlp2.argtypes = [vp, vp, vp, vp, i32, vp, vp, vp, f32, vp, i64, i32, i32, i32, vp]
    lib.alpro_bert_embed_fwd.argtypes = [vp, vp, vp, vp, vp, vp, f32, vp, vp, i32, vp, vp, i32, i32, i32, f32, u32, vp]
    lib.alpro_cast_from_f32.argtypes = [vp, vp, i32, i64, vp]
    lib.alpro_hip_set_option.argtypes = [ctypes.c_char_p, i32]
    lib.alpro_hip_set_stream_option.argtypes = [vp, ctypes.c_char_p, i32]
    lib.alpro_hip_sched_workspace_bytes.restype = ctypes.c_size_t
    lib.alpro_hip_set_sched_workspace.argtypes = [vp, vp, ctypes.c_size_t]
    lib.alpro_hip_release_stream.argtypes = [vp]
    lib.alpro_gemm_qkv_tattn.argtypes = [vp, i64, vp, i64, vp, vp, i64, i32, i32, i32, i32, i32, f32, vp, i64, vp, vp]
    lib.alpro_scatter_add_rows_ordered.argtypes = [vp, vp, vp, i32, i32, i64, i64, vp, vp]
    lib.alpro_gather_seq_fwd.argtypes = [vp, vp, vp, vp, vp, vp, i32, i32, i32, i32, i32, vp]
    lib.alpro_gather_seq_bwd.argtypes = [vp, vp, i32, vp, vp, vp, vp, i32, i32, i32, i32, i32, i32, vp]
    lib.alpro_prepare_clips.argtypes = [vp, i32, vp, f32, ctypes.POINTER(f32), ctypes.POINTER(f32), vp, vp, vp, i32, i32, i32, i32, vp]
    lib.alpro_vtc_loss_fwd.argtypes = [vp, vp, vp, vp, vp, i32, i32, i32, i32, vp, vp, vp, vp, vp]
    lib.alpro_vtc_loss_bwd.argtypes = [vp, vp, vp, vp, vp, i32, i32, i32, i32, vp, vp, vp, vp, vp, vp, vp, vp, vp, vp, vp, vp]
    if lib.alpro_hip_abi_version() != ABI_VERSION:
# ... 45 lines not shown
    _sched_ws.pop((torch.cuda.current_device() if torch.cuda.is_available() else 0, h.value), None)


def get_option(name):
    return _option_values.get(name, _OPTION_DEFAULTS[name])


class option:

    def __init__(self, name, value):
        self.name, self.value = name, value

    def __enter__(self):
        self.prev = _option_values.get(self.name, _OPTION_DEFAULTS[self.name])
        set_option(self.name, self.value)

    def __exit__(self, *a):
        set_option(self.name, self.prev)


def _check(rc, what):
    if rc != 0:
        raise RuntimeError("%s failed (%d): %s" % (what, rc, load().alpro_hip_last_error().decode()))


def _stream():
    return ctypes.c_void_p(torch.cuda.current_stream().cuda_stream)


def _ptr(t):
    return None if t is None else ctypes.c_void_p(t.data_ptr())


def _dev(t, dtype=None):
    if not t.is_cuda:
        raise RuntimeError("alpro_amd ops need device tensors (got %s): the hot path has no CPU fallback" % t.device)
    if dtype is not None and t.dtype != dtype:
        raise RuntimeError("expected %s, got %s" % (dtype, t.dtype))
    if not (t.is_contiguous() or (t.dim() == 2 and t.stride(1) == 1)):
        raise RuntimeError("expected a contiguous (or row-strided 2-D) tensor")
    return t


def dtype_code(torch_dtype):
    return _CODE[torch_dtype]


def torch_dtype(code):
    return _TORCH_DTYPE[code]


def gemm(a, w, out=None, bias=None, act=ACT_NONE, out_dtype=None, alpha=1.0, row_scale=None, row_scale_group=1,
         residual=None, map_mode=MAP_IDENTITY, map_p0=0, map_p1=0, side=None, out_rows=None, pre_act=None, drop_p=0.0, drop_seed=0, bias2=None,
         c2_tiled=False, _desc_only=False):
    lib = load()
    _dev(a); _dev(w, a.dtype)
    M, K = a.shape
    N = w.shape[0]
    assert w.shape[1] == K
    out_dtype = out_dtype or a.dtype
    if out is None:
        out = torch.empty((out_rows if out_rows is not None else M, N), dtype=out_dtype, device=a.device)
    _dev(out, out_dtype)
    d = GemmDesc()
    d.A, d.W, d.C = a.data_ptr(), w.data_ptr(), out.data_ptr()
    d.lda, d.ldw, d.ldc = a.stride(0), w.stride(0), out.shape[-1]
    d.M, d.N, d.K = M, N, K
    d.dtype, d.c_dtype, d.alpha = _CODE[a.dtype], _CODE[out_dtype], alpha
    d.bias = _dev(bias, torch.float32).data_ptr() if bias is not None else None
    d.act = act
    d.row_scale = _dev(row_scale, torch.float32).data_ptr() if row_scale is not None else None
    d.row_scale_group = row_scale_group
    d.residual = _dev(residual, torch.float32).data_ptr() if residual is not None else None
    d.ldr = residual.shape[-1] if residual is not None else 0
    d.map_mode, d.map_p0, d.map_p1 = map_mode, map_p0, map_p1
    d.side = _dev(side, torch.float32).data_ptr() if side is not None else None
    d.ld_side = side.shape[-1] if side is not None else 0
    d.C2 = _dev(pre_act, a.dtype).data_ptr() if pre_act is not None else None
    d.ldc2 = pre_act.shape[-1] if pre_act is not None else 0
    d.c2_tiled = 1 if c2_tiled else 0
    if c2_tiled and not (pre_act is not None and pre_act.is_contiguous() and pre_act.numel() >= gemm_c2_tiled_rows(M, N, K, a.dtype) * N > 0):
        raise RuntimeError("gemm: c2_tiled needs a contiguous pre_act buffer of gemm_c2_tiled_rows(M, N, K, dtype) x N elements (0 rows = not offered for this shape)")
    d.drop_p, d.drop_seed = drop_p, drop_seed
    d.bias2 = _dev(bias2, torch.float32).data_ptr() if bias2 is not None else None
    if _desc_only:
        return d, out
    _check(lib.alpro_gemm(ctypes.byref(d), _stream()), "alpro_gemm")
    return out


def gemm_c2_tiled_rows(M, N, K, dtype):
    return int(load().alpro_gemm_c2_tiled_rows(M, N, K, _CODE[dtype])) if dtype in (torch.float16, torch.bfloat16) else 0


class GemmBatch:

    def __init__(self):
        self._descs, self._keep = [], []
        self._host = self._dev = None

    def add(self, a, w, out, bias=None, alpha=1.0, residual=None, out_dtype=None):
        d, _ = gemm(a, w, out=out, bias=bias, alpha=alpha, residual=residual, out_dtype=out_dtype or out.dtype, _desc_only=True)
        self._descs.append(d)
        self._keep.append((a, w, out, bias, residual))
        self._host = None

    def signature(self):
        return tuple((d.A, d.W, d.C, d.residual) for d in self._descs)

    def launch(self):
        if self._host is None:
            self._host = (GemmDesc * len(self._descs))(*self._descs)
            self._dev = torch.frombuffer(bytearray(bytes(self._host)), dtype=torch.uint8).to(self._keep[0][0].device)
        _check(load().alpro_gemm_batch(self._host, _ptr(self._dev), len(self._descs), _stream()), "alpro_gemm_batch")


def tproj_jobs(jobs, device):
    arr = (TprojJob * len(jobs))()
    for j, d in zip(arr, jobs):
        for k in ("wfc", "bp", "b1", "db1", "g_fc", "g_bp"):
            t = d.get(k)
            if t is not None:
                _dev(t, torch.float32)
                assert t.is_contiguous()
            setattr(j, k, t.data_ptr() if t is not None else None)
    return torch.frombuffer(bytearray(bytes(arr)), dtype=torch.uint8).to(device), len(jobs)


def tproj_small(table, njobs, D, mode):
    _check(load().alpro_tproj_small(_ptr(table), njobs, D, mode, _stream()), "alpro_tproj_small")


def layernorm(x, gamma, beta, eps, out_dtype, rows=None, out32=False, stats=False, map_mode=MAP_IDENTITY, map_p0=0, map_p1=0):
    lib = load()
    _dev(x, torch.float32)
    D = x.shape[-1]
    rows = rows if rows is not None else x.numel() // D
    y = torch.empty((rows, D), dtype=out_dtype, device=x.device)
    y32 = torch.empty((rows, D), dtype=torch.float32, device=x.device) if out32 else None
    mean = torch.empty(rows, dtype=torch.float32, device=x.device) if stats else None
    rstd = torch.empty(rows, dtype=torch.float32, device=x.device) if stats else None
# ... 390 lines not shown
    if lp is not None:
        _dev(lp)
        if lp.dtype not in (torch.float16, torch.bfloat16) or lp.numel() != p.numel() or not lp.is_contiguous():
            raise RuntimeError("adamw_step: lp must be a contiguous 16-bit tensor with p's number of elements")
    _check(lib.alpro_adamw_step_lp(_ptr(p), _ptr(g), _ptr(m), _ptr(v), p.numel(), lr, beta1, beta2, eps, weight_decay, step_size,
                                   _ptr(gnorm_sq), max_norm, grad_scale, _ptr(dyn_state), int(bool(grads_scaled)), int(bool(correct_bias)), int(bool(zero_grad)),
                                   _ptr(lp), _CODE[lp.dtype] if lp is not None else 0, _stream()),
           "alpro_adamw_step")


def loss_scale_update(dyn_state, gnorm_sq, growth=2.0, backoff=0.5, window=2000, min_scale=1.0, max_scale=2.0 ** 24):
    _dev(dyn_state, torch.float32); _dev(gnorm_sq, torch.float32)
    _check(load().alpro_loss_scale_update(_ptr(dyn_state), _ptr(gnorm_sq), growth, backoff, int(window), min_scale, max_scale, _stream()),
           "alpro_loss_scale_update")


_TN_WORKSPACE = {}


def _tn_workspace(device, nbytes):
    key = (device.index, torch.cuda.current_stream(device).cuda_stream)
    ws = _TN_WORKSPACE.get(key)
    if ws is None or ws.numel() < nbytes:
        ws = _TN_WORKSPACE[key] = torch.empty(max(nbytes, 64 << 20), dtype=torch.uint8, device=device)
    return ws


_DETERMINISTIC_WGRAD = [os.environ.get("ALPRO_ATOMIC_WGRAD", "0") != "1"]
_DETERMINISTIC = [os.environ.get("ALPRO_DETERMINISTIC", "1") != "0"]


def set_deterministic_wgrad(on=True):
    _DETERMINISTIC_WGRAD[0] = bool(on)


def set_deterministic(on=True):
    _DETERMINISTIC[0] = bool(on)


def deterministic():
    return _DETERMINISTIC[0]


_REDUCE_WS_BYTES = 8192 * 3 * 768 * 4 + 4096 * 768 * 4


def _reduce_ws(device):
    if not _DETERMINISTIC[0]:
        return None, 0
    ws = _tn_workspace(device, _REDUCE_WS_BYTES)
    return _ptr(ws), _REDUCE_WS_BYTES


def gemm_tn_acc(a, b, c, colsum=None, atomic=None):
    lib = load()
    _dev(a); _dev(b, a.dtype); _dev(c, torch.float32)
    assert a.shape[0] == b.shape[0] and tuple(c.shape) == (a.shape[1], b.shape[1])
    if colsum is not None:
        _dev(colsum, torch.float32)
        assert colsum.numel() >= a.shape[1]
    M, N, K = a.shape[0], a.shape[1], b.shape[1]
    if atomic is None:
        atomic = not _DETERMINISTIC_WGRAD[0] and M > 65536 and ((N + 255) // 256) * ((K + 255) // 256) > 9
    if atomic:
        _check(lib.alpro_gemm_tn_acc(_ptr(a), a.stride(0), _ptr(b), b.stride(0), _ptr(c), c.stride(0), _CODE[a.dtype], M, N, K, _ptr(colsum), _stream()),
               "alpro_gemm_tn_acc")
        return c
    ws = _tn_workspace(a.device, lib.alpro_gemm_tn_workspace_bytes(M, N, K))
    _check(lib.alpro_gemm_tn_acc_ws(_ptr(a), a.stride(0), _ptr(b), b.stride(0), _ptr(c), c.stride(0), _CODE[a.dtype], M, N, K, _ptr(colsum),
                                    _ptr(ws), ws.numel(), _stream()), "alpro_gemm_tn_acc_ws")
    return c


def transpose_jobs(pairs):
    jobs = (TransposeJob * len(pairs))()
    t0 = 0
    for j, (src, out) in zip(jobs, pairs):
        _dev(src, torch.float32); _dev(out)
        assert src.dim() == 2 and out.dim() == 2 and src.stride(1) == 1 and out.stride(1) == 1 and out.shape[0] == src.shape[1] and out.shape[1] >= src.shape[0]
        j.in_, j.out, j.ld_in, j.ld_out = src.data_ptr(), out.data_ptr(), src.stride(0), out.stride(0)
        j.R, j.C, j.Rpad, j.tile0 = src.shape[0], src.shape[1], out.shape[1], t0
        t0 += ((src.shape[1] + 63) // 64) * ((out.shape[1] + 63) // 64)
    table = torch.frombuffer(bytearray(bytes(jobs)), dtype=torch.uint8).to(pairs[0][0].device)
    return table, len(pairs), t0


def transpose_batch(table, njobs, total_tiles, out_dtype):
    _check(load().alpro_transpose_batch(_ptr(table), njobs, total_tiles, _CODE[out_dtype], _stream()), "alpro_transpose_batch")


def colsum_acc(a, out):
    lib = load()
    _dev(a); _dev(out, torch.float32)
    _check(lib.alpro_colsum_acc(_ptr(a), a.stride(0), _ptr(out), _CODE[a.dtype], a.shape[0], a.shape[1], _stream()), "alpro_colsum_acc")
    return out


def softmax_xent(logits, labels, grad_dtype=None, grad_scale=None, ignore_index=-100, pad_to=64):
    lib = load()
    _dev(logits, torch.float32); _dev(labels, torch.int64)
    M, V = logits.shape
    loss_rows = torch.empty(M, dtype=torch.float32, device=logits.device)
    dl, Vp = None, (V + pad_to - 1) // pad_to * pad_to
    if grad_dtype is not None:
        dl = torch.empty((M, Vp), dtype=grad_dtype, device=logits.device)
        _dev(grad_scale, torch.float32)
    _check(lib.alpro_softmax_xent(_ptr(logits), logits.stride(0), _ptr(labels), ignore_index, _ptr(loss_rows), _ptr(dl),
                                  _CODE[grad_dtype] if grad_dtype is not None else 0, Vp, _ptr(grad_scale), M, V, Vp, _stream()),
           "alpro_softmax_xent")
    return (loss_rows, dl) if dl is not None else loss_rows


def vtc_loss_fwd(v, t, gv, gt, temp, col0):
    lib = load()
    for x in (v, t, gv, gt):
        _dev(x, torch.float32)
# ... 45 lines not shown
```

alpro_amd/modeling/timesformer/vit.py:

```python
import math
import os
from functools import partial

import torch
import torch.nn as nn

from alpro_amd import config as rt
from alpro_amd import hip
from alpro_amd.modeling import train as tr
from alpro_amd.modeling.weights import OperandCache, param_version

VIT_EPS = 1e-6


def trunc_normal_(tensor, mean=0., std=1., a=-2., b=2.):
    return nn.init.trunc_normal_(tensor, mean=mean, std=std, a=a, b=b)


def to_2tuple(x):
    return tuple(x) if isinstance(x, (tuple, list)) else (x, x)


class DropPath(nn.Module):

# ... 91 lines not shown
    from alpro_amd.modeling import weights
    main, aux = torch.cuda.current_stream(dev), _aux_stream(dev)
    h = B // 2
    lo, hi = tok[:h], tok[h:]
    lockstep = rt.split_lockstep()
    ev = main.record_event()
    for i, blk in enumerate(blocks):
        r0 = weights.operand_rebuilds()
        blk(lo, h, T, W)
        if weights.operand_rebuilds() != r0:
            ev = main.record_event()
        with torch.cuda.stream(aux):
            if ev is not None:
                aux.wait_event(ev)
                ev = None
            blk(hi, h, T, W)
            if lockstep or i == len(blocks) - 1:
                _ClsSide.join(dev)
                ev_hi = aux.record_event()
        if lockstep or i == len(blocks) - 1:
            _ClsSide.join(dev)
            main.wait_event(ev_hi)
            if lockstep:
                ev = main.record_event()
    return tok


class Block(nn.Module):
    def __init__(self, dim, num_heads, layer_num, mlp_ratio=4., qkv_bias=False, qk_scale=None, drop=0., attn_drop=0.,
                 drop_path=0.1, act_layer=nn.GELU, norm_layer=nn.LayerNorm, attention_type='divided_space_time',
                 use_grad_checkpointing=False):
        super().__init__()
        assert attention_type == 'divided_space_time', "TimeSformer.__init__ hard-codes divided_space_time (vit.py:435)"
        self.attention_type = attention_type
        self.norm1 = norm_layer(dim)
        self.attn = Attention(dim, num_heads=num_heads, qkv_bias=qkv_bias, qk_scale=qk_scale, attn_drop=attn_drop, proj_drop=drop)
        self.temporal_norm1 = norm_layer(dim)
        self.temporal_attn = Attention(dim, num_heads=num_heads, qkv_bias=qkv_bias, qk_scale=qk_scale, attn_drop=attn_drop, proj_drop=drop)
        self.temporal_fc = nn.Linear(dim, dim)
        self.drop_path = DropPath(drop_path) if drop_path > 0. else nn.Identity()
        self.norm2 = norm_layer(dim)
        self.mlp = Mlp(in_features=dim, hidden_features=int(dim * mlp_ratio), act_layer=act_layer, drop=drop)
        self.layer_num = layer_num
        self.use_grad_checkpointing = use_grad_checkpointing
        self._ops = OperandCache()

    def _w(self, name, lin, dt):
        return self._ops.get(name, lin.weight, dt)

    merge_temporal_proj = True
    fuse_ln_bwd_emit = os.environ.get("ALPRO_FUSE_LN_BWD", "1") != "0"
    fuse_residual_ln = os.environ.get("ALPRO_FUSE_RESIDUAL_LN", "1") != "0"

    batch_merged_tproj = os.environ.get("ALPRO_BATCH_TPROJ", "1") != "0"

    def _bank(self):
        bank = getattr(self, "_bank_obj", None) if (self.batch_merged_tproj and self.merge_temporal_proj) else None
        if bank is not None and (len(bank.blocks) <= self._bank_idx or bank.blocks[self._bank_idx] is not self):
            return None
        return bank

    def _merged_tproj(self, dt):
        bank = self._bank()
        if bank is not None:
            return bank.get(self._bank_idx, dt)
        wp, bp, wf = self.temporal_attn.proj.weight, self.temporal_attn.proj.bias, self.temporal_fc.weight
        ver = (param_version(wp), param_version(bp), param_version(wf), dt)
        hit = self._ops._store.get("t_merged")
        if hit is not None and hit[0] == ver:
            return hit[1]
        with torch.no_grad():
            we = hip.gemm(wf.detach().contiguous(), hip.transpose(wp.detach().contiguous()), out_dtype=torch.float32)
            b1 = torch.mv(wf.detach(), bp.detach()).contiguous()
            m = dict(w=we if dt == torch.float32 else hip.cast(we, dt), wT=hip.transpose(we, out_dtype=dt, pad_to=64), b1=b1)
        self._ops._store["t_merged"] = (ver, m)
        from alpro_amd.modeling import weights
        weights.note_operand_rebuild()
        return m

    def _cls_qkv(self, x_cls_in, out=None):
        sa = self.attn
        D = x_cls_in.shape[-1]
        if out is None:
            out = torch.empty((x_cls_in.shape[0], 3 * D), dtype=torch.float32, device=x_cls_in.device)
        hip.gemm_rows(x_cls_in, self._w("s_qkv", sa.qkv, torch.float32)[:D], bias=sa.qkv.bias[:D], ln=(self.norm1.weight, self.norm1.bias, VIT_EPS), out=out[:, :D])
        return out

    def _cls_side_begin(self, side, x, B, T, snapshot):
        main = torch.cuda.current_stream()
        D = x.shape[-1]
        ev_in = main.record_event()
        with torch.cuda.stream(side.stream):
            side.stream.wait_event(ev_in)
            if snapshot:
                x_cls_in = side.buf("x_cls_in", (B, D), x.device)
                x_cls_in.copy_(x[:, 0])
            else:
                x_cls_in = x[:, 0]
            cls_q = self._cls_qkv(x_cls_in, out=side.buf("cls_q", (B, 3 * D), x.device))
            side.ev_q = side.stream.record_event()
        return x_cls_in, cls_q, side.buf("o_c", (B * T, D), x.device)

    def _cls_side_finish(self, side, ev_mid, ev_out, x_cls_in, o_c, B, T, drop_s, drop_m, x2_out, out_out):
        D = o_c.shape[-1]
        sa, f32, dev = self.attn, torch.float32, o_c.device
        with torch.cuda.stream(side.stream):
# ... 57 lines not shown
        else:
            x_cls_in = x[:, 0].clone() if cp else None
        h = hip.layernorm(x, self.temporal_norm1.weight, self.temporal_norm1.bias, VIT_EPS, dt, rows=B * N * T,
                          map_mode=hip.MAP_SKIP_CLS, map_p0=N * T)
        if rt.fuse_temporal_attention() and hip.qkv_tattn_ok(h, T) and ta.qkv.bias is not None:
            a = hip.gemm_qkv_tattn(h, self._w("t_qkv", ta.qkv, dt), ta.qkv.bias, T, H, ta.scale)
        else:
            qkv = hip.gemm(h, self._w("t_qkv", ta.qkv, dt), bias=ta.qkv.bias)
            a = hip.attn_temporal(qkv, T, H, ta.scale)
        if self.fuse_residual_ln and self.merge_temporal_proj:
            mg = self._merged_tproj(dt)
            d_t = hip.gemm(a, mg["w"], bias=mg["b1"], row_scale=drop_t, row_scale_group=T)
            if side is not None:
                side.wait_done()
            defer = rt.defer_temporal_add()
            hs, _ = hip.add_layernorm(x, d_t, self.norm1.weight, self.norm1.bias, VIT_EPS, mode=hip.ADD_PRE_SPATIAL, x_out=None if defer else x,
                                      want_x=not defer, delta_bias=self.temporal_fc.bias, T=T, N=N)
            qkv = hip.gemm(hs, self._w("s_qkv", sa.qkv, dt), bias=sa.qkv.bias)
            if side is not None:
                torch.cuda.current_stream().wait_event(side.ev_q)
                a, o_c = hip.attn(qkv, B * T, N + 1, H, sa.scale, cls_q=cls_q, cls_group=T, cls_out=o_c_buf)
                ev_attn = torch.cuda.current_stream().record_event()
            elif cp:
                a, o_c = hip.attn(qkv, B * T, N + 1, H, sa.scale, cls_q=self._cls_qkv(x_cls_in), cls_group=T)
            else:
                a = hip.attn(qkv, B * T, N + 1, H, sa.scale)
            d_s = hip.gemm(a, self._w("s_proj", sa.proj, dt), bias=sa.proj.bias, row_scale=drop_s, row_scale_group=N + 1)
            if defer:
                h2 = hip.add_layernorm_pre_mlp2(x, d_t, self.temporal_fc.bias, d_s, self.norm2.weight, self.norm2.bias, VIT_EPS, T, N, x_out=x)
            else:
                h2, _ = hip.add_layernorm(x, d_s, self.norm2.weight, self.norm2.bias, VIT_EPS, mode=hip.ADD_PRE_MLP, x_out=x, T=T, N=N)
        else:
            self._forward_halves_unfused(x, xf, a, B, T, N, H, D, dt, drop_t, drop_s)
            h2 = hip.layernorm(x, self.norm2.weight, self.norm2.bias, VIT_EPS, dt)
        f1 = hip.gemm(h2, self._w("fc1", self.mlp.fc1, dt), bias=self.mlp.fc1.bias, act=hip.ACT_GELU)
        hip.gemm(f1, self._w("fc2", self.mlp.fc2, dt), out=xf, bias=self.mlp.fc2.bias, out_dtype=torch.float32, residual=xf,
                 row_scale=drop_m, row_scale_group=S)
        if side is not None:
            self._cls_side_finish(side, ev_attn, torch.cuda.current_stream().record_event(), x_cls_in, o_c, B, T, drop_s, drop_m,
                                  side.buf("x2_c", (B, D), x.device), x[:, 0])
        elif cp:
            self._cls_chain(x_cls_in, o_c, B, T, drop_s, drop_m, torch.empty_like(x_cls_in), x[:, 0])
        return x

    def forward_train(self, x, B, T, W):
        dt = rt.compute_dtype()
        S, D = x.shape[1], x.shape[2]
        N = (S - 1) // T
        H = self.attn.num_heads
        ta, sa = self.temporal_attn, self.attn
        dev = x.device
        sv = {"x": x, "dims": (B, T, N, S, D, H), "dt": dt}
        sv["drop_t"], sv["drop_s"], sv["drop_m"] = self._drop(B * N, dev), self._drop(B * T, dev), self._drop(B, dev)
        cside = None
        if rt.cls_precise(dt) and rt.cls_stream(True) and x.is_cuda and self.fuse_residual_ln and self.merge_temporal_proj:
            cside = _ClsSide.get(dev)
            x_cls_in, cls_q, o_c_buf = self._cls_side_begin(cside, x, B, T, snapshot=False)
        h = hip.layernorm(x, self.temporal_norm1.weight, self.temporal_norm1.bias, VIT_EPS, dt, rows=B * N * T,
                          map_mode=hip.MAP_SKIP_CLS, map_p0=N * T)
        if rt.fuse_temporal_attention(training=True) and hip.qkv_tattn_ok(h, T) and ta.qkv.bias is not None:
            a_t, qkv_t, lse_t = hip.gemm_qkv_tattn(h, self._w("t_qkv", ta.qkv, dt), ta.qkv.bias, T, H, ta.scale, want_qkv=True)
        else:
            qkv_t = hip.gemm(h, self._w("t_qkv", ta.qkv, dt), bias=ta.qkv.bias)
            a_t, lse_t = hip.attn_temporal(qkv_t, T, H, ta.scale, want_lse=True)
        sv["merged"] = self.merge_temporal_proj
        if self.fuse_residual_ln and self.merge_temporal_proj:
            pr = None
            mg = self._merged_tproj(dt)
            d_t = hip.gemm(a_t, mg["w"], bias=mg["b1"], row_scale=sv["drop_t"], row_scale_group=T)
            if cside is not None:
                cside.wait_done()
            hs, xt = hip.add_layernorm(x, d_t, self.norm1.weight, self.norm1.bias, VIT_EPS, mode=hip.ADD_PRE_SPATIAL,
                                       delta_bias=self.temporal_fc.bias, T=T, N=N)
            del d_t
            qkv_s = hip.gemm(hs, self._w("s_qkv", sa.qkv, dt), bias=sa.qkv.bias)
            o_c = None
            if cside is not None:
                torch.cuda.current_stream().wait_event(cside.ev_q)
                a_s, lse_s, o_c = hip.attn(qkv_s, B * T, N + 1, H, sa.scale, want_lse=True, cls_q=cls_q, cls_group=T, cls_out=o_c_buf)
            elif rt.cls_precise(dt):
                a_s, lse_s, o_c = hip.attn(qkv_s, B * T, N + 1, H, sa.scale, want_lse=True, cls_q=self._cls_qkv(x[:, 0]), cls_group=T)
            else:
                a_s, lse_s = hip.attn(qkv_s, B * T, N + 1, H, sa.scale, want_lse=True)
            d_s = hip.gemm(a_s, self._w("s_proj", sa.proj, dt), bias=sa.proj.bias, row_scale=sv["drop_s"], row_scale_group=N + 1)
            h2, x2 = hip.add_layernorm(xt, d_s, self.norm2.weight, self.norm2.bias, VIT_EPS, mode=hip.ADD_PRE_MLP, T=T, N=N)
            del d_s
            if cside is not None:
                ev_x2 = torch.cuda.current_stream().record_event()
        else:
            xt = torch.empty_like(x)
            xt[:, 0] = x[:, 0]
            if self.merge_temporal_proj:
                pr = None
                mg = self._merged_tproj(dt)
                hip.gemm(a_t, mg["w"], out=xt.view(B * S, D), bias=mg["b1"], bias2=self.temporal_fc.bias, out_dtype=torch.float32,
                         residual=x.view(B * S, D), row_scale=sv["drop_t"], row_scale_group=T, map_mode=hip.MAP_SKIP_CLS, map_p0=N * T)
            else:
                pr = hip.gemm(a_t, self._w("t_proj", ta.proj, dt), bias=ta.proj.bias, row_scale=sv["drop_t"], row_scale_group=T)
                hip.gemm(pr, self._w("t_fc", self.temporal_fc, dt), out=xt.view(B * S, D), bias=self.temporal_fc.bias, out_dtype=torch.float32,
                         residual=x.view(B * S, D), map_mode=hip.MAP_SKIP_CLS, map_p0=N * T)
            hs = hip.layernorm(xt, self.norm1.weight, self.norm1.bias, VIT_EPS, dt, rows=B * T * (N + 1),
                               map_mode=hip.MAP_FRAME_TOKENS, map_p0=T, map_p1=N)
            qkv_s = hip.gemm(hs, self._w("s_qkv", sa.qkv, dt), bias=sa.qkv.bias)
            a_s, lse_s = hip.attn(qkv_s, B * T, N + 1, H, sa.scale, want_lse=True)
            x2 = torch.empty_like(x)
            side = torch.empty((B * T, D), dtype=torch.float32, device=dev)
            hip.gemm(a_s, self._w("s_proj", sa.proj, dt), out=x2.view(B * S, D), bias=sa.proj.bias, out_dtype=torch.float32,
                     residual=xt.view(B * S, D), row_scale=sv["drop_s"], row_scale_group=N + 1,
                     map_mode=hip.MAP_FRAME_TOKENS, map_p0=T, map_p1=N, side=side)
            hip.cls_mean_residual(xt, side, x2, B, T)
            h2 = hip.layernorm(x2, self.norm2.weight, self.norm2.bias, VIT_EPS, dt)
        u, sv["u_tiled"] = tr.gelu_save_buffer(B * S, self.mlp.fc1.out_features, D, dt, dev)
        sv["u_grad"] = tr.SAVE_GELU_GRAD
        f1 = hip.gemm(h2, self._w("fc1", self.mlp.fc1, dt), bias=self.mlp.fc1.bias, act=hip.ACT_GELU_SAVE_GRAD if sv["u_grad"] else hip.ACT_GELU, pre_act=u,
                      c2_tiled=sv["u_tiled"])
        out = torch.empty_like(x)
        hip.gemm(f1, self._w("fc2", self.mlp.fc2, dt), out=out.view(B * S, D), bias=self.mlp.fc2.bias, out_dtype=torch.float32,
                 residual=x2.view(B * S, D), row_scale=sv["drop_m"], row_scale_group=S)
        if cside is not None:
            self._cls_side_finish(cside, ev_x2, torch.cuda.current_stream().record_event(), x_cls_in, o_c, B, T, sv["drop_s"], sv["drop_m"], x2[:, 0], out[:, 0])
        elif rt.cls_precise(dt) and self.fuse_residual_ln and self.merge_temporal_proj:
            self._cls_chain(x[:, 0], o_c, B, T, sv["drop_s"], sv["drop_m"], x2[:, 0], out[:, 0])
        sv.update(h=h, qkv_t=qkv_t, a_t=a_t, lse_t=lse_t, pr=pr, xt=xt, hs=hs, qkv_s=qkv_s, a_s=a_s, lse_s=lse_s, x2=x2, h2=h2, u=u, f1=f1)
        return out, sv

    def forward_cls(self, x, B, T, W):
        dt = rt.compute_dtype()
        S, D = x.shape[1], x.shape[2]
        N = (S - 1) // T
        H = self.attn.num_heads
        xf = x.view(B * S, D)
        ta, sa = self.temporal_attn, self.attn
        h = hip.layernorm(x, self.temporal_norm1.weight, self.temporal_norm1.bias, VIT_EPS, dt, rows=B * N * T,
                          map_mode=hip.MAP_SKIP_CLS, map_p0=N * T)
        if rt.fuse_temporal_attention() and hip.qkv_tattn_ok(h, T) and ta.qkv.bias is not None:
            a = hip.gemm_qkv_tattn(h, self._w("t_qkv", ta.qkv, dt), ta.qkv.bias, T, H, ta.scale)
        else:
            qkv = hip.gemm(h, self._w("t_qkv", ta.qkv, dt), bias=ta.qkv.bias)
            a = hip.attn_temporal(qkv, T, H, ta.scale)
        if self.fuse_residual_ln and self.merge_temporal_proj:
            mg = self._merged_tproj(dt)
            d_t = hip.gemm(a, mg["w"], bias=mg["b1"])
            hs, _ = hip.add_layernorm(x, d_t, self.norm1.weight, self.norm1.bias, VIT_EPS, mode=hip.ADD_PRE_SPATIAL, want_x=False,
                                      delta_bias=self.temporal_fc.bias, T=T, N=N)
        else:
            if self.merge_temporal_proj:
                mg = self._merged_tproj(dt)
                hip.gemm(a, mg["w"], out=xf, bias=mg["b1"], bias2=self.temporal_fc.bias, out_dtype=torch.float32, residual=xf,
                         map_mode=hip.MAP_SKIP_CLS, map_p0=N * T)
            else:
                pr = hip.gemm(a, self._w("t_proj", ta.proj, dt), bias=ta.proj.bias)
                hip.gemm(pr, self._w("t_fc", self.temporal_fc, dt), out=xf, bias=self.temporal_fc.bias, out_dtype=torch.float32,
                         residual=xf, map_mode=hip.MAP_SKIP_CLS, map_p0=N * T)
            hs = hip.layernorm(x, self.norm1.weight, self.norm1.bias, VIT_EPS, dt, rows=B * T * (N + 1),
                               map_mode=hip.MAP_FRAME_TOKENS, map_p0=T, map_p1=N)
        qkv = hip.gemm(hs, self._w("s_qkv", sa.qkv, dt), bias=sa.qkv.bias)
        a = hip.attn(qkv, B * T, N + 1, H, sa.scale)
        a_cls = a.view(B * T, N + 1, D)[:, 0].contiguous()
        p_cls = hip.gemm(a_cls, self._w("s_proj", sa.proj, dt), bias=sa.proj.bias, out_dtype=torch.float32)
        x_cls = x[:, 0] + p_cls.view(B, T, D).mean(1)
        h2 = hip.layernorm(x_cls.contiguous(), self.norm2.weight, self.norm2.bias, VIT_EPS, dt)
        f1 = hip.gemm(h2, self._w("fc1", self.mlp.fc1, dt), bias=self.mlp.fc1.bias, act=hip.ACT_GELU)
        return hip.gemm(f1, self._w("fc2", self.mlp.fc2, dt), bias=self.mlp.fc2.bias, out_dtype=torch.float32, residual=x_cls.contiguous())

    def _wt(self, name, lin, dt):
        return tr.transposed_operand(self._ops, name + "^T", lin.weight, dt)

    def _merged_tproj_backward(self, sv, dx, B, T, N, D, dt, G=None):
        ta, fc = self.temporal_attn, self.temporal_fc
        wp, bp, wf = ta.proj.weight.detach(), ta.proj.bias.detach(), fc.weight.detach()
        mg = self._merged_tproj(dt)
        dev = dx.device
        if G is None:
            G = hip.gather_cast(dx, dt, rows=B * N * T, map_mode=hip.MAP_SKIP_CLS, map_p0=N * T, row_scale=sv["drop_t"], row_scale_group=T,
                                colsum_pre=tr.bias_grad(fc.bias))
        ws = sv.get("ws")
        if ws is None:
            ws = torch.zeros(D * D + D, dtype=torch.float32, device=dev)
        dWe, db1 = ws[:D * D].view(D, D), ws[D * D:]
        if dt != torch.float32:
            hip.gemm_tn_acc(G, sv["a_t"], dWe, colsum=db1)
        else:
            hip.gemm(hip.transpose(G, colsum=db1), hip.transpose(sv["a_t"]), out=dWe, out_dtype=torch.float32)
        da = tr.dgrad(G, mg["wT"])
        if sv.get("defer_product_rule"):
            return da
        g_fc, g_p = tr.grad_buffer(fc.weight, zero=True)[0], tr.grad_buffer(ta.proj.weight, zero=True)[0]
        if dt != torch.float32:
            hip.gemm(hip.cast(dWe, dt), self._w("t_proj", ta.proj, dt), out=g_fc, out_dtype=torch.float32, residual=g_fc)
            hip.gemm(self._wt("t_fc", fc, dt)[:, :D], hip.transpose(dWe, out_dtype=dt), out=g_p, out_dtype=torch.float32, residual=g_p)
        else:
            hip.gemm(dWe, wp.contiguous(), out=g_fc, out_dtype=torch.float32, residual=g_fc)
            hip.gemm(hip.transpose(wf.contiguous()), hip.transpose(dWe), out=g_p, out_dtype=torch.float32, residual=g_p)
        g_fc.addr_(db1, bp)
        tr.bias_grad(ta.proj.bias).add_(torch.mv(wf.t(), db1))
        return da

    def backward(self, sv, dx, dz=None, emit_for=None):
        B, T, N, S, D, H = sv["dims"]
        dt = sv["dt"]
        ta, sa = self.temporal_attn, self.attn
        fuse = self.fuse_ln_bwd_emit
        if dz is None:
            dz = hip.gather_cast(dx, dt, row_scale=sv["drop_m"], row_scale_group=S)
        tr.wgrad(dz, sv["f1"], self.mlp.fc2.weight, self.mlp.fc2.bias)
        du = tr.dgrad(dz, self._wt("fc2", self.mlp.fc2, dt), gelu_pre=sv["u"], gelu_saved_grad=sv.get("u_grad", False), gelu_tiled=sv.get("u_tiled", False))
        del dz
        tr.wgrad(du, sv["h2"], self.mlp.fc1.weight, self.mlp.fc1.bias)
        dh2 = tr.dgrad(du, self._wt("fc1", self.mlp.fc1, dt))
        g, b_ = tr.grad_buffer(self.norm2.weight, zero=True)[0], tr.grad_buffer(self.norm2.bias, zero=True)[0]
        if fuse:
            _, dpo = hip.layernorm_bwd(dh2, sv["x2"], self.norm2.weight, VIT_EPS, dx, g, b_,
                                       emit=dict(mode=hip.EMIT_FRAME, rows=B * T * (N + 1), dtype=dt, T=T, N=N, scale=sv["drop_s"]))
        else:
            hip.layernorm_bwd(dh2, sv["x2"], self.norm2.weight, VIT_EPS, dx, g, b_)
            dpo = hip.gather_cast(dx, dt, rows=B * T * (N + 1), map_mode=hip.MAP_FRAME_TOKENS, map_p0=T, map_p1=N,
                                  row_scale=sv["drop_s"], row_scale_group=N + 1, cls_scale=1.0 / T)
        tr.wgrad(dpo, sv["a_s"], sa.proj.weight, sa.proj.bias)
        da = tr.dgrad(dpo, self._wt("s_proj", sa.proj, dt))
        del dpo
        dqkv = hip.attn_bwd(sv["qkv_s"], sv["a_s"], da, sv["lse_s"], B * T, N + 1, H, sa.scale)
        tr.wgrad(dqkv, sv["hs"], sa.qkv.weight, sa.qkv.bias)
        dhs = tr.dgrad(dqkv, self._wt("s_qkv", sa.qkv, dt))
        g, b_ = tr.grad_buffer(self.norm1.weight, zero=True)[0], tr.grad_buffer(self.norm1.bias, zero=True)[0]
        G = None
        if fuse and sv["merged"]:
            _, G = hip.layernorm_bwd(dhs, sv["xt"], self.norm1.weight, VIT_EPS, dx, g, b_, rows=B * T * (N + 1), map_mode=hip.MAP_FRAME_TOKENS,
                                     map_p0=T, map_p1=N, emit=dict(mode=hip.EMIT_SKIP_CLS, rows=B * N * T, dtype=dt, T=T, N=N, scale=sv["drop_t"], group=T,
                                                                   colsum_pre=tr.bias_grad(self.temporal_fc.bias)))
        else:
            hip.layernorm_bwd(dhs, sv["xt"], self.norm1.weight, VIT_EPS, dx, g, b_, rows=B * T * (N + 1),
                              map_mode=hip.MAP_FRAME_TOKENS, map_p0=T, map_p1=N)
        if sv["merged"]:
            da = self._merged_tproj_backward(sv, dx, B, T, N, D, dt, G=G)
        else:
            dfo = hip.gather_cast(dx, dt, rows=B * N * T, map_mode=hip.MAP_SKIP_CLS, map_p0=N * T)
            tr.wgrad(dfo, sv["pr"], self.temporal_fc.weight, self.temporal_fc.bias)
            dpp = tr.dgrad(dfo, self._wt("t_fc", self.temporal_fc, dt), row_scale=sv["drop_t"], row_scale_group=T)
            tr.wgrad(dpp, sv["a_t"], ta.proj.weight, ta.proj.bias)
            da = tr.dgrad(dpp, self._wt("t_proj", ta.proj, dt))
        dqkv = hip.attn_temporal_bwd(sv["qkv_t"], sv["a_t"], da, sv["lse_t"], T, H, ta.scale)
        tr.wgrad(dqkv, sv["h"], ta.qkv.weight, ta.qkv.bias)
        dh = tr.dgrad(dqkv, self._wt("t_qkv", ta.qkv, dt))
        g, b_ = tr.grad_buffer(self.temporal_norm1.weight, zero=True)[0], tr.grad_buffer(self.temporal_norm1.bias, zero=True)[0]
        dz_prev = None
        if fuse and emit_for is not None:
            _, dz_prev = hip.layernorm_bwd(dh, sv["x"], self.temporal_norm1.weight, VIT_EPS, dx, g, b_, rows=B * N * T, map_mode=hip.MAP_SKIP_CLS,
                                           map_p0=N * T, emit=dict(mode=hip.EMIT_ROWS, rows=B * S, dtype=dt, T=T, N=N, scale=emit_for["drop_m"], group=S,
                                                                   extra_cls=B))
        else:
            hip.layernorm_bwd(dh, sv["x"], self.temporal_norm1.weight, VIT_EPS, dx, g, b_, rows=B * N * T,
                              map_mode=hip.MAP_SKIP_CLS, map_p0=N * T)
        return dx, dz_prev


_KEEP_CACHE = {}


def sample_drop_paths(blocks, B, T, N, device):
    sizes = (B * N, B * T, B)
    live = [blk for blk in blocks if isinstance(blk.drop_path, DropPath) and blk.drop_path.drop_prob and blk.training]
    if not live:
        return
    per = sum(sizes)
    key = (per, str(device), tuple(blk.drop_path.drop_prob for blk in live))
    keep = _KEEP_CACHE.get(key)
    if keep is None:
        keep = torch.tensor([1.0 - blk.drop_path.drop_prob for blk in live], dtype=torch.float32).repeat_interleave(per).to(device)
        _KEEP_CACHE.clear()
        _KEEP_CACHE[key] = keep
    scale = torch.floor(keep + torch.rand(per * len(live), dtype=torch.float32, device=device)) / keep
    off = 0
    for blk in live:
        blk._presampled = {}
        for n in sizes:
            blk._presampled[n] = scale[off:off + n]
            off += n


class _MergedTProjBank:

    def __init__(self, blocks):
        self.blocks = list(blocks)
        self.state = None
        self.bwd = None
        self._bwd_tables = {}

    def __reduce__(self):
        return (_MergedTProjBank, ([],))

    def _params(self):
        return [p for b in self.blocks for p in (b.temporal_fc.weight, b.temporal_attn.proj.weight, b.temporal_attn.proj.bias)]

    def get(self, idx, dt):
        from alpro_amd.modeling import weights
        ps = self._params()
        fast = (weights.param_epoch(), weights._EXT_EPOCH[0], dt, tuple(p._version for p in ps))
        st = self.state
        if st is None or st["fast"] != fast:
            key = (dt,) + tuple(param_version(p) for p in ps)
            if st is None or st["key"] != key:
                st = self._refresh(dt, key)
            st["fast"] = fast
        return dict(w=st["we_dt"][idx], wT=st["weT_dt"][idx], b1=st["b1"][idx])

    def _refresh(self, dt, key):
        nb = len(self.blocks)
        wf = [b.temporal_fc.weight.detach() for b in self.blocks]
        wp = [b.temporal_attn.proj.weight.detach() for b in self.blocks]
        bp = [b.temporal_attn.proj.bias.detach() for b in self.blocks]
        D, dev = wf[0].shape[0], wf[0].device
        st = self.state
        if st is None or st["dt"] != dt or st["we32"].device != dev:
            we32 = torch.empty((nb, D, D), dtype=torch.float32, device=dev)
            st = dict(dt=dt, we32=we32, wpT32=torch.empty_like(we32), b1=torch.empty((nb, D), dtype=torch.float32, device=dev),
                      we_dt=we32 if dt == torch.float32 else torch.empty((nb, D, D), dtype=dt, device=dev),
                      weT_dt=torch.empty((nb, D, D), dtype=dt, device=dev), sig=None)
        sig = tuple(t.data_ptr() for t in wf + wp + bp)
        if st["sig"] != sig:
            st["t_wp"] = hip.transpose_jobs([(wp[i], st["wpT32"][i]) for i in range(nb)])
            gb = hip.GemmBatch()
            for i in range(nb):
                gb.add(wf[i], st["wpT32"][i], out=st["we32"][i], out_dtype=torch.float32)
            st["gemm"] = gb
            st["t_we"] = hip.transpose_jobs([(st["we32"][i], st["weT_dt"][i]) for i in range(nb)])
            st["t_b1"] = hip.tproj_jobs([dict(wfc=wf[i], bp=bp[i], b1=st["b1"][i]) for i in range(nb)], dev)
            st["sig"] = sig
        with torch.no_grad():
            hip.transpose_batch(*st["t_wp"], torch.float32)
            st["gemm"].launch()
# ... 320 lines not shown
```

alpro_amd/modeling/train.py:

```python
import os
import weakref

import torch

from alpro_amd import hip
from alpro_amd.modeling.weights import param_version


def grad_buffer(p, zero=False):
    if p.grad is not None and (p.grad.numel() <= 1 or any(p.grad.stride())):
        return p.grad, True
    p.grad = torch.zeros_like(p, memory_format=torch.contiguous_format) if zero else torch.empty_like(p, memory_format=torch.contiguous_format)
    return p.grad, False


def add_grad(p, g):
    if p.grad is None or (p.grad.numel() > 1 and not any(p.grad.stride())):
        p.grad = g.detach().clone().reshape(p.shape).contiguous()
    else:
        p.grad.add_(g.reshape(p.shape))


def fused_param_view(params):
    ps = [p.detach() for p in params]
# ... 33 lines not shown
        _WT_REGISTRY.pop((id(cache), key), None)
    return out


def refresh_transposed_operands():
    if os.environ.get("ALPRO_WT_REFRESH", "1") == "0":
        return 0
    live = []
    for k, e in list(_WT_REGISTRY.items()):
        cache, ps = e["cache"](), [r() for r in e["params"]]
        hit = cache._store.get(e["key"]) if cache is not None else None
        if hit is None or hit[1] is not e["out"] or any(p is None for p in ps) or ps[0].data_ptr() != e["src"].data_ptr():
            del _WT_REGISTRY[k]
            continue
        live.append((e, cache, ps))
    if not live:
        return 0
    t = _WT_TABLE
    by_dtype = {}
    for item in live:
        by_dtype.setdefault(item[0]["out"].dtype, []).append(item)
    n = 0
    for dt, items in by_dtype.items():
        sig = tuple((e["src"].data_ptr(), e["out"].data_ptr()) for e, _, _ in items)
        slot = t.setdefault(dt, {})
        if slot.get("sig") != sig:
            slot["table"], slot["njobs"], slot["tiles"] = hip.transpose_jobs([(e["src"], e["out"]) for e, _, _ in items])
            slot["sig"] = sig
        hip.transpose_batch(slot["table"], slot["njobs"], slot["tiles"], dt)
        for e, cache, ps in items:
            cache._store[e["key"]] = (tuple(param_version(p) for p in ps), e["out"])
        n += len(items)
    return n


def bias_grad(bias):
    return grad_buffer(bias, zero=True)[0]


def fused_grad_view(params):
    gs = [p.grad for p in params]
    if any(g is None or not g.is_contiguous() for g in gs):
        return None
    base = gs[0]
    off = base.data_ptr()
    for g in gs:
        if g.untyped_storage().data_ptr() != base.untyped_storage().data_ptr() or g.data_ptr() != off or g.shape[1:] != base.shape[1:]:
            return None
        off += g.numel() * 4
    rows = sum(g.shape[0] for g in gs)
    return torch.as_strided(base, (rows,) + tuple(base.shape[1:]), base.stride())


def wgrad(dy_t, x_t, weight, bias, bias_done=False):
    if bias_done:
        bias = None
    if bias is not None:
        gb = grad_buffer(bias, zero=True)[0]
    gw, existed = grad_buffer(weight, zero=True)
    gw2 = gw.view(gw.shape[0], -1)
    if dy_t.dtype != torch.float32:
        from alpro_amd import config as rt
        side = rt.wgrad_side_stream(dy_t.device)
        if side is None:
            hip.gemm_tn_acc(dy_t, x_t, gw2, colsum=gb if bias is not None else None)
            return
        side.wait_stream(torch.cuda.current_stream(dy_t.device))
        with torch.cuda.stream(side):
            hip.gemm_tn_acc(dy_t, x_t, gw2, colsum=gb if bias is not None else None)
        dy_t.record_stream(side)
        x_t.record_stream(side)
        return
    dyT = hip.transpose(dy_t, colsum=gb if bias is not None else None)
    hip.gemm(dyT, hip.transpose(x_t), out=gw2, out_dtype=torch.float32, residual=gw2)


SAVE_GELU_GRAD = os.environ.get("ALPRO_SAVE_GELU_GRAD", "1") != "0"


TILED_GELU_GRAD = os.environ.get("ALPRO_TILED_GELU_GRAD", "1") != "0"


def gelu_save_buffer(M, N, K, dt, device):
    rows = hip.gemm_c2_tiled_rows(M, N, K, dt) if (SAVE_GELU_GRAD and TILED_GELU_GRAD) else 0
    return torch.empty((rows or M, N), dtype=dt, device=device), rows > 0


def dgrad(dy_t, wT, out_dtype=None, row_scale=None, row_scale_group=1, gelu_pre=None, gelu_saved_grad=False, gelu_tiled=False):
    n = dy_t.shape[1]
    w = wT if wT.shape[1] == n else wT[:, :n]
    if not w.is_contiguous() or n % (64 if dy_t.dtype != torch.float32 else 32) != 0:
        pad = wT.shape[1] - n
        dy_t = torch.nn.functional.pad(dy_t, (0, pad))
        w = wT
    return hip.gemm(dy_t, w, out_dtype=out_dtype or dy_t.dtype, row_scale=row_scale, row_scale_group=row_scale_group,
                    act=(hip.ACT_MUL_SAVED if gelu_saved_grad else hip.ACT_GELU_BWD) if gelu_pre is not None else hip.ACT_NONE, pre_act=gelu_pre,
                    c2_tiled=gelu_tiled and gelu_saved_grad)


_LIVE_ANCHORS = weakref.WeakSet()


BACKWARD_EPOCH = [0]


class Anchor(torch.autograd.Function):

    @staticmethod
    def forward(ctx, run, n_act, *inputs):
        ctx.run = run
        ctx.n_act = n_act
        ctx.n_in = len(inputs)
        from alpro_amd import config as rt
        ctx.dt = rt.compute_dtype()
        ctx.set_materialize_grads(False)
        _LIVE_ANCHORS.add(ctx)
        with torch.no_grad():
            outs = run.forward(*inputs[:n_act])
        ctx.single = torch.is_tensor(outs)
        return outs

    @staticmethod
    def backward(ctx, *grads):
        ctx.run.others_pending = any(c is not ctx for c in _LIVE_ANCHORS)
        BACKWARD_EPOCH[0] += 1
        from alpro_amd import config as rt
        rt.check_backward_precision(getattr(ctx.run, "dt", None) or ctx.dt)
        rt.wgrad_scope(True)
        try:
            with torch.no_grad():
                g = ctx.run.backward(*[None if x is None else x.contiguous() for x in grads])
        finally:
            rt.wgrad_scope(False)
            rt.join_wgrad()
            _LIVE_ANCHORS.discard(ctx)
        if grads and any(x is not None and x.is_cuda for x in grads):
            cur = torch.cuda.current_stream()
            if rt.is_text_side_stream(cur):
                ev = cur.record_event()
                torch.autograd.Variable._execution_engine.queue_callback(lambda: torch.cuda.current_stream().wait_event(ev))
        g = (g,) if (torch.is_tensor(g) or g is None) else tuple(g)
        g = g + (None,) * (ctx.n_act - len(g))
        ctx.run = None
        return (None, None) + tuple(g) + (None,) * (ctx.n_in - ctx.n_act)


def run_anchored(run, activations, params):
    params = [p for p in params if p.requires_grad]
    need = torch.is_grad_enabled() and (any(torch.is_tensor(a) and a.requires_grad for a in activations) or len(params) > 0)
    if not need:
# ... 4 lines not shown
```

include/alpro_hip.h:

```cpp
#ifndef ALPRO_HIP_H
#define ALPRO_HIP_H

#include <stddef.h>
#include <stdint.h>

#ifdef __cplusplus
extern "C" {
#endif

#define ALPRO_HIP_ABI_VERSION 22

enum { ALPRO_OK = 0, ALPRO_ERR_INVALID = 1, ALPRO_ERR_LAUNCH = 2 };
enum { ALPRO_F32 = 0, ALPRO_BF16 = 1, ALPRO_F16 = 2 };
enum { ALPRO_ACT_NONE = 0, ALPRO_ACT_GELU = 1, ALPRO_ACT_RELU = 2, ALPRO_ACT_GELU_BWD = 3,
       ALPRO_ACT_GELU_SAVE_GRAD = 4, ALPRO_ACT_MUL_SAVED = 5,
       ALPRO_ACT_RELU_MASK = 6 };

enum { ALPRO_MAP_IDENTITY = 0, ALPRO_MAP_SKIP_CLS = 1, ALPRO_MAP_FRAME_TOKENS = 2, ALPRO_MAP_PATCH_EMBED = 3 };

const char* alpro_hip_last_error(void);
int alpro_hip_abi_version(void);
int alpro_hip_set_option(const char* name, int value);
int alpro_hip_set_stream_option(void* stream, const char* name, int value);
size_t alpro_hip_sched_workspace_bytes(void);
// ... 105 lines not shown
int alpro_cast_from_f32(const float* src, void* dst, int dtype, int64_t n, void* stream);


int alpro_attn_bwd(const void* qkv, const void* out, const void* dout, const float* lse, void* dqkv, int dtype,
                   int batch, int L, int H, float scale, const float* key_bias, float drop_p, uint32_t drop_seed,
                   void* stream);
int alpro_attn_temporal_bwd(const void* qkv, const void* out, const void* dout, const float* lse, void* dqkv, int dtype,
                            int64_t rows, int T, int H, float scale, void* stream);

int alpro_layernorm_bwd(const void* dy, int dy_dtype, int64_t ld_dy, const float* dy2, const float* x, int64_t ldx,
                        const float* gamma, float eps, float* dx, int64_t ld_dx, int accumulate, float* dgamma,
                        float* dbeta, int rows, int D, int map_mode, int map_p0, int map_p1, float drop_p,
                        uint32_t drop_seed, void* workspace, size_t workspace_bytes, void* stream);

enum { ALPRO_EMIT_NONE = 0, ALPRO_EMIT_ROWS = 1, ALPRO_EMIT_FRAME = 2, ALPRO_EMIT_SKIP_CLS = 3 };
int alpro_layernorm_bwd_emit(const void* dy, int dy_dtype, int64_t ld_dy, const float* dy2, const float* x, int64_t ldx,
                             const float* gamma, float eps, float* dx, int64_t ld_dx, int accumulate, float* dgamma, float* dbeta,
                             int rows, int D, int map_mode, int map_p0, int map_p1, float drop_p, uint32_t drop_seed, void* emit_out,
                             int emit_dtype , int emit_mode, int emit_p0, int emit_p1, const float* emit_scale, int emit_scale_group, float emit_drop_p,
                             uint32_t emit_drop_seed, float* emit_colsum_pre, int emit_extra_cls, void* workspace, size_t workspace_bytes,
                             void* stream);

int alpro_transpose(const void* in, int in_dtype, int64_t ld_in, void* out, int out_dtype, int64_t ld_out, int R, int C,
                    int Rpad, float* colsum, void* stream);

typedef struct alpro_transpose_job {
  const float* in;
  void* out;
  int64_t ld_in, ld_out;
  int32_t R, C, Rpad, tile0;
} alpro_transpose_job_t;
int alpro_transpose_batch(const alpro_transpose_job_t* jobs, int njobs, int total_tiles, int out_dtype, void* stream);

int alpro_gather_cast(const float* src, int64_t ld, void* out, int dtype, int rows, int D, int map_mode, int map_p0,
                      int map_p1, const float* row_scale, int row_scale_group, float cls_scale, float drop_p,
                      uint32_t drop_seed, float* colsum, float* colsum_pre, void* workspace, size_t workspace_bytes, void* stream);

int alpro_gelu_bwd(const void* dh, const void* u, void* du, int dtype, int64_t n, void* stream);

int alpro_cls_mean_bwd(const float* dx_out, int64_t ld_batch, float* dside, int B, int T, int D, void* stream);

int alpro_scatter_add_rows(const float* src, const int64_t* idx, float* dst, int rows, int idx_mod, int D, int64_t skip_idx, void* stream);
int alpro_scatter_add_rows_ordered(const float* src, const int64_t* idx, float* dst, int rows, int D, int64_t dst_rows, int64_t skip_idx, uint32_t* keys_ws,
                                   void* stream);

int alpro_gemm_tn_acc(const void* A, int64_t lda, const void* B, int64_t ldb, float* C, int64_t ldc, int dtype, int M,
                      int N, int K, float* colsum, void* stream);

size_t alpro_gemm_tn_workspace_bytes(int M, int N, int K);
int alpro_gemm_tn_ranges(int M, int N, int K, int compute_units);
int alpro_gemm_tn_acc_ws(const void* A, int64_t lda, const void* B, int64_t ldb, float* C, int64_t ldc, int dtype, int M,
                         int N, int K, float* colsum, void* workspace, size_t workspace_bytes, void* stream);

int alpro_colsum_acc(const void* A, int64_t lda, float* out, int dtype, int M, int N, void* stream);

int alpro_softmax_xent(const float* logits, int64_t ld, const int64_t* labels, int ignore_index, float* loss_rows,
                       void* dlogits, int dtype, int64_t ldd, const float* grad_scale, int M, int V, int Vpad,
                       void* stream);

int alpro_vtc_loss_fwd(const float* v, const float* t, const float* gv, const float* gt, const float* temp, int B, int G, int E, int col0,
                       float* sim_v2t, float* sim_t2v, float* lse, float* loss, void* stream);
int alpro_vtc_loss_bwd(const float* v, const float* t, const float* gv, const float* gt, const float* temp, int B, int G, int E, int col0,
                       const float* sim_v2t, const float* sim_t2v, const float* lse, const float* dloss, float* ds_v2t, float* ds_t2v,
                       float* dv, float* dt, float* dgv, float* dgt, float* dtemp, void* stream);


int alpro_sumsq(const float* x, int64_t n, float* out, void* workspace, size_t workspace_bytes, void* stream);

int alpro_adamw_step(float* p, float* g, float* m, float* v, int64_t n, float lr, float beta1, float beta2,
                     float eps, float weight_decay, float step_size, const float* gnorm_sq, float max_norm,
                     float grad_scale, const float* dyn_state, int grads_scaled, int correct_bias,
                     int zero_grad , void* stream);
int alpro_adamw_step_lp(float* p, float* g, float* m, float* v, int64_t n, float lr, float beta1, float beta2, float eps, float weight_decay,
                        float step_size, const float* gnorm_sq, float max_norm, float grad_scale, const float* dyn_state, int grads_scaled,
                        int correct_bias, int zero_grad, void* lp, int lp_dtype, void* stream);

int alpro_loss_scale_update(float* dyn_state, const float* gnorm_sq, float growth, float backoff, int window, float min_scale,
                            float max_scale, void* stream);

#ifdef __cplusplus
}
#endif
#endif
```

Baseline: 433.3.

## Skip MLP GEMM row panels whose samples are fully dropped by drop-path

Builds per-block compacted lists of 256-row panels that contain at least one sample kept by stochastic depth. The fc1/fc2 forward GEMMs, the dgrad GEMMs and the wgrad TN GEMMs then iterate only over live panels. Outputs for skipped panels are filled by a small kernel, either copying the residual or writing zeros. This removes MLP matmul work for dropped samples, at the cost of extra kernels, scalar indirection in the tile mapping, and tail-split tuning being disabled when panels are in use.

```diff
diff --git a/alpro_amd/csrc/common.hpp b/alpro_amd/csrc/common.hpp
--- a/alpro_amd/csrc/common.hpp
+++ b/alpro_amd/csrc/common.hpp
@@ -210,6 +210,9 @@
 __device__ __forceinline__ float sload_f32(const float* p, uint32_t idx) {
   return *((const __attribute__((address_space(4))) float*)p + __builtin_amdgcn_readfirstlane(idx));
 }
+__device__ __forceinline__ int sload_i32(const int* p, uint32_t idx) {
+  return *((const __attribute__((address_space(4))) int*)p + __builtin_amdgcn_readfirstlane(idx));
+}
 __device__ __forceinline__ uint32_t lds_addr_of(const void* p) { return (uint32_t)(uintptr_t)(__attribute__((address_space(3))) const char*)p; }
 
 void set_error(const char* fmt, ...);
@@ -242,6 +245,7 @@
   uint32_t* prev;
   uint32_t magic_ntn;
   uint32_t epi;
+  const int* panels;
 };
 struct SchedLaunch {
   uint32_t* cur = nullptr;
diff --git a/alpro_amd/csrc/core.hip b/alpro_amd/csrc/core.hip
--- a/alpro_amd/csrc/core.hip
+++ b/alpro_amd/csrc/core.hip
@@ -833,3 +833,72 @@
   ALPRO_DISPATCH_DTYPE(dtype, T, hipLaunchKernelGGL(bert_embed_kernel<T>, dim3((rows + 3) / 4), dim3(256), 0, (hipStream_t)stream, ids, word, pos, type0, gamma, beta, eps, y32, (T*)y_t, mean, rstd, rows, L, drop_p, drop_seed));
   return check_launch("alpro_bert_embed_fwd");
 }
+
+namespace alpro {
+namespace {
+__global__ __launch_bounds__(256) void drop_panels_kernel(const float* __restrict__ scale, int64_t block_stride, int groups, int group_rows, int M,
+                                                          int* __restrict__ out, int npan) {
+  __shared__ int wsum[4];
+  __shared__ int base_s;
+  const float* sc = scale + (int64_t)blockIdx.x * block_stride;
+  int* o = out + (int64_t)blockIdx.x * (2 * npan + 2);
+  const int tid = threadIdx.x, lane = tid & 63, wave = tid >> 6;
+  if (tid == 0) base_s = 0;
+  __syncthreads();
+  for (int p0 = 0; p0 < npan; p0 += 256) {
+    const int p = p0 + tid;
+    int keep = 0;
+    if (p < npan) {
+      const int r0 = p * 256, r1 = min(r0 + 256, M) - 1;
+      const int g0 = r0 / group_rows, g1 = min(r1 / group_rows, groups - 1);
+      for (int g = g0; g <= g1; ++g) keep |= sc[g] != 0.f ? 1 : 0;
+      o[1 + npan + p] = keep;
+    }
+    const uint64_t m = __ballot(keep);
+    const int before = __popcll(m & ((1ull << lane) - 1ull));
+    if (lane == 0) wsum[wave] = __popcll(m);
+    __syncthreads();
+    int off = base_s;
+    for (int w = 0; w < wave; ++w) off += wsum[w];
+    if (keep) o[1 + off + before] = p;
+    __syncthreads();
+    if (tid == 0) base_s += wsum[0] + wsum[1] + wsum[2] + wsum[3];
+    __syncthreads();
+  }
+  const int cnt = base_s;
+  if (tid == 0) o[0] = cnt;
+  __syncthreads();
+  const int last = cnt > 0 ? o[cnt] : 0;
+  for (int i = cnt + tid; i < npan; i += 256) o[1 + i] = last;
+}
+
+__global__ __launch_bounds__(256) void panels_fill_kernel(const int* __restrict__ panels, int npan, int M, char* __restrict__ dst, int64_t ld_dst,
+                                                          const char* __restrict__ src, int64_t ld_src, int row_bytes) {
+  const int p = blockIdx.x;
+  if (panels[1 + npan + p]) return;
+  const int r0 = p * 256, rows = min(256, M - r0), per_row = row_bytes >> 4;
+  const u32x4 z = {0u, 0u, 0u, 0u};
+  for (int i = blockIdx.y * 256 + threadIdx.x; i < rows * per_row; i += gridDim.y * 256) {
+    const int r = r0 + i / per_row, c = (i % per_row) << 4;
+    *(u32x4*)(dst + (int64_t)r * ld_dst + c) = src ? *(const u32x4*)(src + (int64_t)r * ld_src + c) : z;
+  }
+}
+}
+}
+
+extern "C" int alpro_drop_panels(const float* scale, int64_t block_stride, int nblocks, int groups, int group_rows, int M, int* panels, void* stream) {
+  using namespace alpro;
+  ALPRO_CHECK(scale && panels && nblocks > 0 && groups > 0 && group_rows > 0 && M > 0 && (int64_t)groups * group_rows >= M, "alpro_drop_panels: bad args");
+  hipLaunchKernelGGL(drop_panels_kernel, dim3(nblocks), dim3(256), 0, (hipStream_t)stream, scale, block_stride, groups, group_rows, M, panels, (M + 255) / 256);
+  return check_launch("alpro_drop_panels");
+}
+
+extern "C" int alpro_panels_fill(const int* panels, int M, void* dst, int64_t ld_dst_bytes, const void* src, int64_t ld_src_bytes, int row_bytes, void* stream) {
+  using namespace alpro;
+  ALPRO_CHECK(panels && dst && M > 0 && row_bytes > 0, "alpro_panels_fill: bad args");
+  ALPRO_CHECK((row_bytes % 16) == 0 && (ld_dst_bytes % 16) == 0 && (ld_src_bytes % 16) == 0 && ((uintptr_t)dst % 16) == 0 && ((uintptr_t)src % 16) == 0,
+              "alpro_panels_fill: rows must be 16-byte aligned multiples of 16 bytes");
+  hipLaunchKernelGGL(panels_fill_kernel, dim3((M + 255) / 256, 4), dim3(256), 0, (hipStream_t)stream, panels, (M + 255) / 256, M, (char*)dst, ld_dst_bytes,
+                     (const char*)src, ld_src_bytes, row_bytes);
+  return check_launch("alpro_panels_fill");
+}
diff --git a/alpro_amd/csrc/gemm.hip b/alpro_amd/csrc/gemm.hip
--- a/alpro_amd/csrc/gemm.hip
+++ b/alpro_amd/csrc/gemm.hip
@@ -303,10 +303,10 @@
 }
 
 template <typename T, int ACT, int MAP>
-__device__ __forceinline__ void gemm_nt_tile(const alpro_gemm_desc_t& g, const int bid, char* smem) {
+__device__ __forceinline__ void gemm_nt_tile(const alpro_gemm_desc_t& g, const int bid, char* smem, const int* panels = nullptr) {
   const int tid = threadIdx.x, lane = tid & 63, wave = tid >> 6;
   const int wr = wave >> 1, wc = wave & 1;
-  const int ntn = (g.N + BN - 1) / BN, ntm = (g.M + BM - 1) / BM;
+  const int ntn = (g.N + BN - 1) / BN, ntm = panels ? 2 * sload_i32(panels, 0) : (g.M + BM - 1) / BM;
   const int nblk = ntn * ntm;
   if (bid >= nblk) return;
   int tile;
@@ -316,7 +316,8 @@
     tile = (xcd < r ? xcd * (q + 1) : r * (q + 1) + (xcd - r) * q) + idx;
   }
   const int tm = tile / ntn, tn = tile - tm * ntn;
-  const int m0 = tm * BM, n0 = tn * BN;
+  const int m0 = panels ? sload_i32(panels, 1 + (tm >> 1)) * (2 * BM) + (tm & 1) * BM : tm * BM, n0 = tn * BN;
+  if (m0 >= g.M) return;
 
   const char* Ab = (const char*)g.A;
   const char* Wb = (const char*)g.W;
@@ -428,9 +429,9 @@
 }
 
 template <typename T, int ACT, int MAP>
-__global__ __launch_bounds__(NT, 2) void gemm_nt_kernel(const alpro_gemm_desc_t g) {
+__global__ __launch_bounds__(NT, 2) void gemm_nt_kernel(const alpro_gemm_desc_t g, const int* panels) {
   extern __shared__ __attribute__((aligned(16))) char smem[];
-  gemm_nt_tile<T, ACT, MAP>(g, blockIdx.x, smem);
+  gemm_nt_tile<T, ACT, MAP>(g, blockIdx.x, smem, panels);
 }
 
 template <typename T, int ACT, int MAP>
@@ -453,11 +454,11 @@
 }
 
 template <typename T, int ACT, int MAP, int TUNE = 1>
-__global__ __launch_bounds__(NT2, 2) void gemm_nt256p_kernel(const alpro_gemm_desc_t g, const int tail_split) {
+__global__ __launch_bounds__(NT2, 2) void gemm_nt256p_kernel(const alpro_gemm_desc_t g, const int tail_split, const int* panels) {
   extern __shared__ __attribute__((aligned(16))) char smem[];
   const int tid = threadIdx.x, lane = tid & 63, wave = __builtin_amdgcn_readfirstlane(tid >> 6);
   const int wr = wave >> 2, wc = wave & 3;
-  const int ntn = (g.N + BN2 - 1) / BN2, ntm = (g.M + BM2 - 1) / BM2;
+  const int ntn = (g.N + BN2 - 1) / BN2, ntm = panels ? sload_i32(panels, 0) : (g.M + BM2 - 1) / BM2;
   const int nblk = ntn * ntm;
   const int64_t lda_b = g.lda * (int64_t)sizeof(T), ldw_b = g.ldw * (int64_t)sizeof(T);
   const int nk = (g.K * (int)sizeof(T)) / ROWB;
@@ -486,7 +487,8 @@
     return slot < rem;
   };
   auto setup = [&](int tile, int hf) {
-    const int tm = tile / ntn, tn = tile - tm * ntn;
+    const int ctm = tile / ntn, tn = tile - ctm * ntn;
+    const int tm = panels ? sload_i32(panels, 1 + ctm) : ctm;
     m0 = tm * BM2 + (hf > 0 ? BM2 / 2 : 0);
     n0 = tn * BN2;
 #pragma unroll
@@ -732,7 +734,7 @@
   extern __shared__ __attribute__((aligned(16))) char smem[];
   const int tid = threadIdx.x, lane = tid & 63, wave = __builtin_amdgcn_readfirstlane(tid >> 6);
   const int wr = wave >> 2, wc = wave & 3;
-  const int ntn = (g.N + BN2 - 1) / BN2, ntm = (g.M + BM2 - 1) / BM2;
+  const int ntn = (g.N + BN2 - 1) / BN2, ntm = sc.panels ? sload_i32(sc.panels, 0) : (g.M + BM2 - 1) / BM2;
   const int nblk = ntn * ntm;
   const int64_t lda_b = g.lda * 2, ldw_b = g.ldw * 2;
   const int nk = g.K >> 6;
@@ -876,12 +878,14 @@
 #pragma unroll
     for (int h = 0; h < 2; ++h) ow[h][i] = (uint32_t)((r0 + h * 128 + i * 8) * ldw_b) + (sw0 ^ (uint32_t)(i * 64));
   }
-  struct Tile { const char* a[2]; const char* w; };
+  struct Tile { const char* a[2]; const char* w; int m0; };
   auto tile_base = [&](int tile) {
-    const int tm = ntn == 1 ? tile : (int)__umulhi((uint32_t)tile, sc.magic_ntn), tn = tile - tm * ntn;
+    const int ctm = ntn == 1 ? tile : (int)__umulhi((uint32_t)tile, sc.magic_ntn), tn = tile - ctm * ntn;
+    const int tm = sc.panels ? sload_i32(sc.panels, 1 + ctm) : ctm;
     const int vr = g.M - tm * BM2;
     const char* a0 = (const char*)g.A + (int64_t)tm * BM2 * lda_b;
     Tile t;
+    t.m0 = tm * BM2;
 #pragma unroll
     for (int h = 0; h < 2; ++h) t.a[h] = a0 + (int64_t)((h * 128 + wave * 16 < vr) ? h * 128 : -(wave * 16)) * lda_b;
     t.w = (const char*)g.W + (int64_t)tn * BN2 * ldw_b;
@@ -960,7 +964,8 @@
 
   while (true) {
     const int tile = cur_t;
-    const int tm0 = (ntn == 1 ? tile : (int)__umulhi((uint32_t)tile, sc.magic_ntn)) * BM2, tn0 = (tile - (tm0 >> 8) * ntn) * BN2;
+    const int ctm0 = (ntn == 1 ? tile : (int)__umulhi((uint32_t)tile, sc.magic_ntn)) * BM2, tn0 = (tile - (ctm0 >> 8) * ntn) * BN2;
+    const int tm0 = sc.panels ? cur.m0 : ctm0;
     f32x4 acc[8][4];
 #pragma unroll
     for (int i = 0; i < 8; ++i)
@@ -1274,7 +1279,7 @@
 }
 
 template <typename T, int ACT, int MAP>
-int launch_gemm_inst(const alpro_gemm_desc_t& g, hipStream_t st) {
+int launch_gemm_inst(const alpro_gemm_desc_t& g, hipStream_t st, const int* panels) {
   static DeviceOnce attr_once;
   attr_once.run([&] {
     (void)hipFuncSetAttribute((const void*)gemm_nt_kernel<T, ACT, MAP>, hipFuncAttributeMaxDynamicSharedMemorySize, 4 * TILE_BYTES);
@@ -1304,7 +1309,7 @@
     });
     const int m_full = g.M / BM2 * BM2, m_rem = g.M - m_full;
     bool ragged_in_kernel = false;
-    const bool take_q = q_kernel_takes(g, &ragged_in_kernel);
+    const bool take_q = q_kernel_takes(g, &ragged_in_kernel) && !(panels && m_rem && !ragged_in_kernel);
     ALPRO_CHECK(!g.c2_tiled || (take_q && c2_tiled_ok(g)), "alpro_gemm: c2_tiled is not available for this descriptor (M=%d N=%d K=%d act=%d): ask alpro_gemm_c2_tiled_rows first", g.M, g.N, g.K, g.act);
     if (take_q) {
       alpro_gemm_desc_t gq = g;
@@ -1314,7 +1319,7 @@
       const int ntn_q = g.N / BN2, ntm_q = (gq.M + BM2 - 1) / BM2;
       const int tiles = ntn_q * ntm_q;
       int tail_panels = 0;
-      if (get_option(OPT_GEMM_TAIL) == 1 && !g.c2_tiled && tiles > grid && g.K >= 2048) {
+      if (get_option(OPT_GEMM_TAIL) == 1 && !panels && !g.c2_tiled && tiles > grid && g.K >= 2048) {
         const int R = tiles % grid;
         if (R > 0 && 5 * R <= 2 * grid) tail_panels = (R + ntn_q - 1) / ntn_q;
       }
@@ -1329,6 +1334,7 @@
       sc.blk = sc.prev = nullptr;
       sc.magic_ntn = magic_u32((uint32_t)(g.N / BN2));
       sc.epi = (uint32_t)get_option(OPT_GEMM_EPI);
+      sc.panels = panels;
       {
         SchedLaunch blocks(get_option(OPT_GEMM_SCHED) == 1 ? st : nullptr, get_option(OPT_GEMM_SCHED) == 1);
         sc.blk = blocks.cur;
@@ -1345,7 +1351,7 @@
         if (g.C2) gr.C2 = (char*)g.C2 + m_tail0 * g.ldc2 * 2;
         if (g.residual) gr.residual = g.residual + m_tail0 * g.ldr;
         const int ntn = (gr.N + BN - 1) / BN, ntm = (gr.M + BM - 1) / BM;
-        hipLaunchKernelGGL((gemm_nt_kernel<T, ACT, MAP>), dim3(ntn * ntm), dim3(NT), 4 * TILE_BYTES, st, gr);
+        hipLaunchKernelGGL((gemm_nt_kernel<T, ACT, MAP>), dim3(ntn * ntm), dim3(NT), 4 * TILE_BYTES, st, gr, (const int*)nullptr);
       }
       return check_launch("alpro_gemm");
     }
@@ -1357,47 +1363,47 @@
     const int tune = get_option(OPT_GEMM_TUNE);
     const int tail = get_option(OPT_GEMM_TAIL);
     if constexpr (std::is_same<T, bf16_t>::value && ACT == ALPRO_ACT_NONE && MAP == ALPRO_MAP_IDENTITY) {
-      if (tune == 0) { hipLaunchKernelGGL((gemm_nt256p_kernel<T, ACT, MAP, 0>), dim3(grid), dim3(NT2), 4 * TILE2_BYTES + EPI_BYTES, st, g, tail); return check_launch("alpro_gemm"); }
-      if (tune == 2) { hipLaunchKernelGGL((gemm_nt256p_kernel<T, ACT, MAP, 2>), dim3(grid), dim3(NT2), 4 * TILE2_BYTES + EPI_BYTES, st, g, tail); return check_launch("alpro_gemm"); }
+      if (tune == 0) { hipLaunchKernelGGL((gemm_nt256p_kernel<T, ACT, MAP, 0>), dim3(grid), dim3(NT2), 4 * TILE2_BYTES + EPI_BYTES, st, g, tail, panels); return check_launch("alpro_gemm"); }
+      if (tune == 2) { hipLaunchKernelGGL((gemm_nt256p_kernel<T, ACT, MAP, 2>), dim3(grid), dim3(NT2), 4 * TILE2_BYTES + EPI_BYTES, st, g, tail, panels); return check_launch("alpro_gemm"); }
 #ifdef ALPRO_ABLATIONS
-      if (tune == 3) { hipLaunchKernelGGL((gemm_nt256p_kernel<T, ACT, MAP, 3>), dim3(grid), dim3(NT2), 4 * TILE2_BYTES + EPI_BYTES, st, g, tail); return check_launch("alpro_gemm"); }
-      if (tune == 4) { hipLaunchKernelGGL((gemm_nt256p_kernel<T, ACT, MAP, 4>), dim3(grid), dim3(NT2), 4 * TILE2_BYTES + EPI_BYTES, st, g, tail); return check_launch("alpro_gemm"); }
-      if (tune == 12) { hipLaunchKernelGGL((gemm_nt256p_kernel<T, ACT, MAP, 12>), dim3(grid), dim3(NT2), 4 * TILE2_BYTES + EPI_BYTES, st, g, tail); return check_launch("alpro_gemm"); }
-      if (tune == 11) { hipLaunchKernelGGL((gemm_nt256p_kernel<T, ACT, MAP, 11>), dim3(grid), dim3(NT2), 4 * TILE2_BYTES + EPI_BYTES, st, g, tail); return check_launch("alpro_gemm"); }
-      if (tune == 10) { hipLaunchKernelGGL((gemm_nt256p_kernel<T, ACT, MAP, 10>), dim3(grid), dim3(NT2), 4 * TILE2_BYTES + EPI_BYTES, st, g, tail); return check_launch("alpro_gemm"); }
-      if (tune == 5) { hipLaunchKernelGGL((gemm_nt256p_kernel<T, ACT, MAP, 5>), dim3(grid), dim3(NT2), 4 * TILE2_BYTES + EPI_BYTES, st, g, tail); return check_launch("alpro_gemm"); }
-      if (tune == 6) { hipLaunchKernelGGL((gemm_nt256p_kernel<T, ACT, MAP, 6>), dim3(grid), dim3(NT2), 4 * TILE2_BYTES + EPI_BYTES, st, g, tail); return check_launch("alpro_gemm"); }
+      if (tune == 3) { hipLaunchKernelGGL((gemm_nt256p_kernel<T, ACT, MAP, 3>), dim3(grid), dim3(NT2), 4 * TILE2_BYTES + EPI_BYTES, st, g, tail, panels); return check_launch("alpro_gemm"); }
+      if (tune == 4) { hipLaunchKernelGGL((gemm_nt256p_kernel<T, ACT, MAP, 4>), dim3(grid), dim3(NT2), 4 * TILE2_BYTES + EPI_BYTES, st, g, tail, panels); return check_launch("alpro_gemm"); }
+      if (tune == 12) { hipLaunchKernelGGL((gemm_nt256p_kernel<T, ACT, MAP, 12>), dim3(grid), dim3(NT2), 4 * TILE2_BYTES + EPI_BYTES, st, g, tail, panels); return check_launch("alpro_gemm"); }
+      if (tune == 11) { hipLaunchKernelGGL((gemm_nt256p_kernel<T, ACT, MAP, 11>), dim3(grid), dim3(NT2), 4 * TILE2_BYTES + EPI_BYTES, st, g, tail, panels); return check_launch("alpro_gemm"); }
+      if (tune == 10) { hipLaunchKernelGGL((gemm_nt256p_kernel<T, ACT, MAP, 10>), dim3(grid), dim3(NT2), 4 * TILE2_BYTES + EPI_BYTES, st, g, tail, panels); return check_launch("alpro_gemm"); }
+      if (tune == 5) { hipLaunchKernelGGL((gemm_nt256p_kernel<T, ACT, MAP, 5>), dim3(grid), dim3(NT2), 4 * TILE2_BYTES + EPI_BYTES, st, g, tail, panels); return check_launch("alpro_gemm"); }
+      if (tune == 6) { hipLaunchKernelGGL((gemm_nt256p_kernel<T, ACT, MAP, 6>), dim3(grid), dim3(NT2), 4 * TILE2_BYTES + EPI_BYTES, st, g, tail, panels); return check_launch("alpro_gemm"); }
 #endif
     }
-    hipLaunchKernelGGL((gemm_nt256p_kernel<T, ACT, MAP>), dim3(grid), dim3(NT2), 4 * TILE2_BYTES + EPI_BYTES, st, g, tail);
+    hipLaunchKernelGGL((gemm_nt256p_kernel<T, ACT, MAP>), dim3(grid), dim3(NT2), 4 * TILE2_BYTES + EPI_BYTES, st, g, tail, panels);
   } else {
-    const int ntn = (g.N + BN - 1) / BN, ntm = (g.M + BM - 1) / BM;
-    hipLaunchKernelGGL((gemm_nt_kernel<T, ACT, MAP>), dim3(ntn * ntm), dim3(NT), 4 * TILE_BYTES, st, g);
+    const int ntn = (g.N + BN - 1) / BN, ntm = panels ? 2 * ((g.M + BM2 - 1) / BM2) : (g.M + BM - 1) / BM;
+    hipLaunchKernelGGL((gemm_nt_kernel<T, ACT, MAP>), dim3(ntn * ntm), dim3(NT), 4 * TILE_BYTES, st, g, panels);
   }
   return check_launch("alpro_gemm");
 }
 
 template <typename T>
-int launch_gemm(const alpro_gemm_desc_t& g, hipStream_t st) {
+int launch_gemm(const alpro_gemm_desc_t& g, hipStream_t st, const int* panels = nullptr) {
 #ifdef ALPRO_ISA_QUICK
-  return g.act == ALPRO_ACT_MUL_SAVED ? launch_gemm_inst<T, ALPRO_ACT_MUL_SAVED, ALPRO_MAP_IDENTITY>(g, st) : launch_gemm_inst<T, ALPRO_ACT_NONE, ALPRO_MAP_IDENTITY>(g, st);
+  return g.act == ALPRO_ACT_MUL_SAVED ? launch_gemm_inst<T, ALPRO_ACT_MUL_SAVED, ALPRO_MAP_IDENTITY>(g, st, panels) : launch_gemm_inst<T, ALPRO_ACT_NONE, ALPRO_MAP_IDENTITY>(g, st, panels);
 #else
   if (g.act != ALPRO_ACT_NONE) {
     if (g.map_mode != ALPRO_MAP_IDENTITY) {
       set_error("alpro_gemm: an activation cannot be combined with a row map");
       return ALPRO_ERR_INVALID;
     }
-    if (g.act == ALPRO_ACT_GELU_BWD) return launch_gemm_inst<T, ALPRO_ACT_GELU_BWD, ALPRO_MAP_IDENTITY>(g, st);
-    if (g.act == ALPRO_ACT_GELU_SAVE_GRAD) return launch_gemm_inst<T, ALPRO_ACT_GELU_SAVE_GRAD, ALPRO_MAP_IDENTITY>(g, st);
-    if (g.act == ALPRO_ACT_MUL_SAVED) return launch_gemm_inst<T, ALPRO_ACT_MUL_SAVED, ALPRO_MAP_IDENTITY>(g, st);
-    return g.act == ALPRO_ACT_GELU ? launch_gemm_inst<T, ALPRO_ACT_GELU, ALPRO_MAP_IDENTITY>(g, st)
-                                   : launch_gemm_inst<T, ALPRO_ACT_RELU, ALPRO_MAP_IDENTITY>(g, st);
+    if (g.act == ALPRO_ACT_GELU_BWD) return launch_gemm_inst<T, ALPRO_ACT_GELU_BWD, ALPRO_MAP_IDENTITY>(g, st, panels);
+    if (g.act == ALPRO_ACT_GELU_SAVE_GRAD) return launch_gemm_inst<T, ALPRO_ACT_GELU_SAVE_GRAD, ALPRO_MAP_IDENTITY>(g, st, panels);
+    if (g.act == ALPRO_ACT_MUL_SAVED) return launch_gemm_inst<T, ALPRO_ACT_MUL_SAVED, ALPRO_MAP_IDENTITY>(g, st, panels);
+    return g.act == ALPRO_ACT_GELU ? launch_gemm_inst<T, ALPRO_ACT_GELU, ALPRO_MAP_IDENTITY>(g, st, panels)
+                                   : launch_gemm_inst<T, ALPRO_ACT_RELU, ALPRO_MAP_IDENTITY>(g, st, panels);
   }
   switch (g.map_mode) {
-    case ALPRO_MAP_IDENTITY: return launch_gemm_inst<T, ALPRO_ACT_NONE, ALPRO_MAP_IDENTITY>(g, st);
-    case ALPRO_MAP_SKIP_CLS: return launch_gemm_inst<T, ALPRO_ACT_NONE, ALPRO_MAP_SKIP_CLS>(g, st);
-    case ALPRO_MAP_FRAME_TOKENS: return launch_gemm_inst<T, ALPRO_ACT_NONE, ALPRO_MAP_FRAME_TOKENS>(g, st);
-    default: return launch_gemm_inst<T, ALPRO_ACT_NONE, ALPRO_MAP_PATCH_EMBED>(g, st);
+    case ALPRO_MAP_IDENTITY: return launch_gemm_inst<T, ALPRO_ACT_NONE, ALPRO_MAP_IDENTITY>(g, st, panels);
+    case ALPRO_MAP_SKIP_CLS: return launch_gemm_inst<T, ALPRO_ACT_NONE, ALPRO_MAP_SKIP_CLS>(g, st, panels);
+    case ALPRO_MAP_FRAME_TOKENS: return launch_gemm_inst<T, ALPRO_ACT_NONE, ALPRO_MAP_FRAME_TOKENS>(g, st, panels);
+    default: return launch_gemm_inst<T, ALPRO_ACT_NONE, ALPRO_MAP_PATCH_EMBED>(g, st, panels);
   }
 #endif
 }
@@ -1475,6 +1481,19 @@
   return (q_kernel_takes(g, &ragged) && c2_tiled_ok(g)) ? (M + 255) / 256 * 256 : 0;
 }
 
+extern "C" int alpro_gemm_panels(const alpro_gemm_desc_t* d, const int* panels, void* stream) {
+  using namespace alpro;
+  if (const int rc = check_gemm_desc(d)) return rc;
+  ALPRO_CHECK(panels, "alpro_gemm_panels: null panel list");
+  ALPRO_CHECK(d->map_mode == ALPRO_MAP_IDENTITY && d->m_off == 0, "alpro_gemm_panels: identity row map and m_off = 0 only");
+#ifdef ALPRO_ISA_QUICK
+  return launch_gemm<f16_t>(*d, (hipStream_t)stream, panels);
+#else
+  ALPRO_DISPATCH_DTYPE(d->dtype, T, return launch_gemm<T>(*d, (hipStream_t)stream, panels));
+  return ALPRO_OK;
+#endif
+}
+
 extern "C" int alpro_gemm(const alpro_gemm_desc_t* d, void* stream) {
   using namespace alpro;
   if (const int rc = check_gemm_desc(d)) return rc;
diff --git a/alpro_amd/csrc/gemm_tn.hip b/alpro_amd/csrc/gemm_tn.hip
--- a/alpro_amd/csrc/gemm_tn.hip
+++ b/alpro_amd/csrc/gemm_tn.hip
@@ -35,7 +35,7 @@
 __global__ __launch_bounds__(NT3, 1) void gemm_tn_kernel(const T* __restrict__ A, int64_t lda, const T* __restrict__ B, int64_t ldb,
                                                          float* __restrict__ C, int64_t ldc, int M, int N, int K, int per,
                                                          int tiles, int units, int tn_cnt, float* __restrict__ colsum, float* __restrict__ part,
-                                                         float* __restrict__ part_cs, int ablate) {
+                                                         float* __restrict__ part_cs, int ablate, const int* __restrict__ panels) {
   extern __shared__ __attribute__((aligned(16))) char smem[];
   const int tid = threadIdx.x, lane = tid & 63, wave = __builtin_amdgcn_readfirstlane(tid >> 6);
   const int wr = wave >> 2, wc = wave & 3;
@@ -43,24 +43,48 @@
   const int unit = (blockIdx.x & 7) * upx + (blockIdx.x >> 3);
   if (unit >= units) return;
   const int range = unit / tiles, tile = unit - range * tiles;
-  const int total_steps = (M + TM - 1) / TM;
+  int total_steps = (M + TM - 1) / TM;
+  int npan = 0;
+  if (panels) {
+    npan = sload_i32(panels, 0);
+    const int all = (M + 8 * TM - 1) / (8 * TM);
+    const int last = npan > 0 ? sload_i32(panels, (uint32_t)npan) : -1;
+    total_steps = npan * 8 - (last == all - 1 ? all * 8 - total_steps : 0);
+    const int ranges = units / tiles;
+    per = (total_steps + ranges - 1) / ranges;
+  }
   const int s0 = range * per, s1 = min(s0 + per, total_steps);
   const int n0 = (tile % tn_cnt) * TW, k0 = (tile / tn_cnt) * TW;
-  if (s0 >= s1) return;
+  if (s0 >= s1) {
+    if (part) {
+      float* dst = part + (int64_t)unit * (TW * TW) + wave * 8192 + lane * 4;
+      const f32x4 z = {0.f, 0.f, 0.f, 0.f};
+#pragma unroll 4
+      for (int q = 0; q < 32; ++q) __builtin_nontemporal_store(z, (f32x4*)(dst + q * 256));
+    }
+    if (colsum && part_cs && lane < 32)
+      part_cs[((int64_t)range * (tiles / tn_cnt) + tile / tn_cnt) * (tn_cnt * TW) + n0 + wr * 128 + wc * 32 + lane] = 0.f;
+    return;
+  }
+  auto panel_at = [&](int i) { return sload_i32(panels, (uint32_t)(1 + min(i, npan - 1))); };
+  const int o0 = panels ? panel_at(s0 >> 3) * 8 + (s0 & 7) : s0;
 
   const char* zero = (const char*)g_zero_page;
-  const int rows_end = min(s1 * TM, M);
   const char* curA[2];
   const char* curB[2];
-  int mrow[2];
+  int mrow[2], jst[2] = {s0, s0}, pc[2] = {0, 0}, pn[2] = {0, 0};
+  if (panels) {
+    pc[0] = pc[1] = panel_at(s0 >> 3);
+    pn[0] = pn[1] = panel_at((s0 >> 3) + 1);
+  }
   int64_t strA[2], strB[2];
 #pragma unroll
   for (int i = 0; i < 2; ++i) {
     const int row = (wave + 8 * i) * 2 + (lane >> 5);
     const int col = ((lane & 31) ^ ((row & 3) << 2)) * 8;
-    const int64_t m = (int64_t)s0 * TM + row;
+    const int64_t m = (int64_t)o0 * TM + row;
     const bool ca = n0 + col < N, cb = k0 + col < K;
-    mrow[i] = s0 * TM + row;
+    mrow[i] = o0 * TM + row;
     curA[i] = ca ? (const char*)(A + m * lda + n0 + col) : zero;
     curB[i] = cb ? (const char*)(B + m * ldb + k0 + col) : zero;
     strA[i] = ca ? (int64_t)TM * lda * (int64_t)sizeof(T) : 0;
@@ -71,13 +95,22 @@
   auto copy = [&](int d, int buf) {
     const int i = d >> 1;
     const char* src = (d & 1) ? curB[i] : curA[i];
-    src = mrow[i] < rows_end ? src : zero;
+    src = (jst[i] < s1 && mrow[i] < M) ? src : zero;
     dma16(src, __builtin_amdgcn_readfirstlane(lds_piece[i] + buf * 2 * IMG_BYTES + (d & 1) * IMG_BYTES));
   };
   auto advance = [&](int i) {
     curA[i] += strA[i];
     curB[i] += strB[i];
     mrow[i] += TM;
+    ++jst[i];
+    if (panels && (jst[i] & 7) == 0) {
+      const int skip = (pn[i] - pc[i] - 1) * 8;
+      curA[i] += strA[i] * skip;
+      curB[i] += strB[i] * skip;
+      mrow[i] += TM * skip;
+      pc[i] = pn[i];
+      pn[i] = panel_at((jst[i] >> 3) + 1);
+    }
   };
 
   f32x16 acc[4][2];
@@ -392,8 +425,8 @@
   return tn_plan(M, N, K, true, cus).ranges;
 }
 
-extern "C" int alpro_gemm_tn_acc_ws(const void* A, int64_t lda, const void* B, int64_t ldb, float* C, int64_t ldc, int dtype, int M, int N,
-                                    int K, float* colsum, void* workspace, size_t workspace_bytes, void* stream) {
+static int gemm_tn_launch(const void* A, int64_t lda, const void* B, int64_t ldb, float* C, int64_t ldc, int dtype, int M, int N,
+                          int K, float* colsum, void* workspace, size_t workspace_bytes, const int* panels, void* stream) {
   ALPRO_CHECK(A && B && C && M > 0 && N > 0 && K > 0, "alpro_gemm_tn_acc: bad args");
   ALPRO_CHECK(dtype == ALPRO_BF16 || dtype == ALPRO_F16, "alpro_gemm_tn_acc: 16-bit operands only (fp32 mode uses alpro_transpose + alpro_gemm)");
   ALPRO_CHECK(lda % 8 == 0 && ldb % 8 == 0 && lda >= (N + 7) / 8 * 8 && ldb >= (K + 7) / 8 * 8,
@@ -425,20 +458,31 @@
       (void)hipFuncSetAttribute((const void*)gemm_tn_kernel<bf16_t, 0>, hipFuncAttributeMaxDynamicSharedMemorySize, (int)lds);
       (void)hipFuncSetAttribute((const void*)gemm_tn_kernel<bf16_t, 1>, hipFuncAttributeMaxDynamicSharedMemorySize, (int)lds);
     });
-    if (pp) hipLaunchKernelGGL((gemm_tn_kernel<bf16_t, 1>), dim3(grid), dim3(NT3), lds, st, (const bf16_t*)A, lda, (const bf16_t*)B, ldb, C, ldc, M, N, K, p.per, p.tiles, p.units, p.tn, colsum, part, part_cs, kind);
-    else hipLaunchKernelGGL((gemm_tn_kernel<bf16_t, 0>), dim3(grid), dim3(NT3), lds, st, (const bf16_t*)A, lda, (const bf16_t*)B, ldb, C, ldc, M, N, K, p.per, p.tiles, p.units, p.tn, colsum, part, part_cs, kind);
+    if (pp) hipLaunchKernelGGL((gemm_tn_kernel<bf16_t, 1>), dim3(grid), dim3(NT3), lds, st, (const bf16_t*)A, lda, (const bf16_t*)B, ldb, C, ldc, M, N, K, p.per, p.tiles, p.units, p.tn, colsum, part, part_cs, kind, panels);
+    else hipLaunchKernelGGL((gemm_tn_kernel<bf16_t, 0>), dim3(grid), dim3(NT3), lds, st, (const bf16_t*)A, lda, (const bf16_t*)B, ldb, C, ldc, M, N, K, p.per, p.tiles, p.units, p.tn, colsum, part, part_cs, kind, panels);
   } else {
     static DeviceOnce once;
     once.run([&] {
       (void)hipFuncSetAttribute((const void*)gemm_tn_kernel<f16_t, 0>, hipFuncAttributeMaxDynamicSharedMemorySize, (int)lds);
       (void)hipFuncSetAttribute((const void*)gemm_tn_kernel<f16_t, 1>, hipFuncAttributeMaxDynamicSharedMemorySize, (int)lds);
     });
-    if (pp) hipLaunchKernelGGL((gemm_tn_kernel<f16_t, 1>), dim3(grid), dim3(NT3), lds, st, (const f16_t*)A, lda, (const f16_t*)B, ldb, C, ldc, M, N, K, p.per, p.tiles, p.units, p.tn, colsum, part, part_cs, kind);
-    else hipLaunchKernelGGL((gemm_tn_kernel<f16_t, 0>), dim3(grid), dim3(NT3), lds, st, (const f16_t*)A, lda, (const f16_t*)B, ldb, C, ldc, M, N, K, p.per, p.tiles, p.units, p.tn, colsum, part, part_cs, kind);
+    if (pp) hipLaunchKernelGGL((gemm_tn_kernel<f16_t, 1>), dim3(grid), dim3(NT3), lds, st, (const f16_t*)A, lda, (const f16_t*)B, ldb, C, ldc, M, N, K, p.per, p.tiles, p.units, p.tn, colsum, part, part_cs, kind, panels);
+    else hipLaunchKernelGGL((gemm_tn_kernel<f16_t, 0>), dim3(grid), dim3(NT3), lds, st, (const f16_t*)A, lda, (const f16_t*)B, ldb, C, ldc, M, N, K, p.per, p.tiles, p.units, p.tn, colsum, part, part_cs, kind, panels);
   }
   if ((part || part_cs) && kind != 1)
     hipLaunchKernelGGL(tn_reduce_kernel, dim3((part ? p.tiles * 64 : 0) + (part_cs ? p.tn * (TW / 32) : 0)), dim3(256), 0, st, part, part_cs, C, ldc, colsum, N, K, p.tiles, p.ranges, p.tn);
   return check_launch("alpro_gemm_tn_acc");
+}
+
+extern "C" int alpro_gemm_tn_acc_ws(const void* A, int64_t lda, const void* B, int64_t ldb, float* C, int64_t ldc, int dtype, int M, int N,
+                                    int K, float* colsum, void* workspace, size_t workspace_bytes, void* stream) {
+  return gemm_tn_launch(A, lda, B, ldb, C, ldc, dtype, M, N, K, colsum, workspace, workspace_bytes, nullptr, stream);
+}
+
+extern "C" int alpro_gemm_tn_acc_panels(const void* A, int64_t lda, const void* B, int64_t ldb, float* C, int64_t ldc, int dtype, int M, int N,
+                                        int K, float* colsum, void* workspace, size_t workspace_bytes, const int* panels, void* stream) {
+  ALPRO_CHECK(panels, "alpro_gemm_tn_acc_panels: null panel list");
+  return gemm_tn_launch(A, lda, B, ldb, C, ldc, dtype, M, N, K, colsum, workspace, workspace_bytes, panels, stream);
 }
 
 extern "C" int alpro_gemm_tn_acc(const void* A, int64_t lda, const void* B, int64_t ldb, float* C, int64_t ldc, int dtype, int M, int N,
diff --git a/alpro_amd/hip.py b/alpro_amd/hip.py
--- a/alpro_amd/hip.py
+++ b/alpro_amd/hip.py
@@ -16,7 +16,7 @@
 _TORCH_DTYPE = {F32: torch.float32, BF16: torch.bfloat16, F16: torch.float16}
 _CODE = {v: k for k, v in _TORCH_DTYPE.items()}
 
-EXPORTS = ["alpro_hip_last_error", "alpro_hip_abi_version", "alpro_hip_set_option", "alpro_hip_set_stream_option", "alpro_gemm", "alpro_gemm_c2_tiled_rows", "alpro_layernorm_fwd",
+EXPORTS = ["alpro_drop_panels", "alpro_gemm_panels", "alpro_gemm_tn_acc_panels", "alpro_panels_fill", "alpro_hip_last_error", "alpro_hip_abi_version", "alpro_hip_set_option", "alpro_hip_set_stream_option", "alpro_gemm", "alpro_gemm_c2_tiled_rows", "alpro_layernorm_fwd",
            "alpro_attn_temporal_fwd", "alpro_attn_fwd", "alpro_patchify", "alpro_cls_mean_residual",
            "alpro_vit_final_pool", "alpro_bert_embed_fwd", "alpro_cast_from_f32", "alpro_attn_bwd", "alpro_attn_temporal_bwd",
            "alpro_layernorm_bwd", "alpro_transpose", "alpro_transpose_batch", "alpro_gelu_bwd", "alpro_cls_mean_bwd", "alpro_scatter_add_rows", "alpro_gather_cast", "alpro_sumsq", "alpro_adamw_step", "alpro_gemm_tn_acc", "alpro_gemm_tn_acc_ws", "alpro_gemm_tn_workspace_bytes", "alpro_gemm_tn_ranges", "alpro_colsum_acc", "alpro_softmax_xent", "alpro_vtc_loss_fwd", "alpro_vtc_loss_bwd", "alpro_prepare_clips", "alpro_loss_scale_update", "alpro_add_layernorm_fwd", "alpro_layernorm_bwd_emit", "alpro_gemm_batch", "alpro_tproj_small", "alpro_attn_cls_fwd", "alpro_gemm_rows_f32", "alpro_gather_seq_fwd", "alpro_gather_seq_bwd", "alpro_scatter_add_rows_ordered",
@@ -73,6 +73,10 @@
     vp, i32, i64, f32 = ctypes.c_void_p, ctypes.c_int, ctypes.c_int64, ctypes.c_float
     lib.alpro_gemm.argtypes = [ctypes.POINTER(GemmDesc), vp]
     lib.alpro_gemm_batch.argtypes = [ctypes.POINTER(GemmDesc), vp, ctypes.c_int, vp]
+    lib.alpro_gemm_panels.argtypes = [ctypes.POINTER(GemmDesc), vp, vp]
+    lib.alpro_gemm_tn_acc_panels.argtypes = [vp, i64, vp, i64, vp, i64, i32, i32, i32, i32, vp, vp, ctypes.c_size_t, vp, vp]
+    lib.alpro_drop_panels.argtypes = [vp, i64, i32, i32, i32, i32, vp, vp]
+    lib.alpro_panels_fill.argtypes = [vp, i32, vp, i64, vp, i64, i32, vp]
     lib.alpro_tproj_small.argtypes = [vp, ctypes.c_int, ctypes.c_int, ctypes.c_int, vp]
     lib.alpro_layernorm_fwd.argtypes = [vp, i64, vp, vp, f32, vp, i32, i64, vp, vp, vp, i32, i32, i32, i32, i32, vp]
     lib.alpro_add_layernorm_fwd.argtypes = [vp, vp, i32, vp, i32, vp, vp, vp, f32, vp, vp, i64, i32, i32, i32, vp]
@@ -224,7 +228,7 @@
 
 def gemm(a, w, out=None, bias=None, act=ACT_NONE, out_dtype=None, alpha=1.0, row_scale=None, row_scale_group=1,
          residual=None, map_mode=MAP_IDENTITY, map_p0=0, map_p1=0, side=None, out_rows=None, pre_act=None, drop_p=0.0, drop_seed=0, bias2=None,
-         c2_tiled=False, _desc_only=False):
+         c2_tiled=False, _desc_only=False, *, panels=None):
     lib = load()
     _dev(a); _dev(w, a.dtype)
     M, K = a.shape
@@ -257,8 +261,42 @@
     d.bias2 = _dev(bias2, torch.float32).data_ptr() if bias2 is not None else None
     if _desc_only:
         return d, out
+    if panels is not None:
+        _check(lib.alpro_gemm_panels(ctypes.byref(d), _ptr(_panels_ok(panels, M)), _stream()), "alpro_gemm_panels")
+        return out
     _check(lib.alpro_gemm(ctypes.byref(d), _stream()), "alpro_gemm")
     return out
+
+
+def panel_words(M):
+    return 2 * ((M + 255) // 256) + 2
+
+
+def _panels_ok(panels, M):
+    assert panels.dtype == torch.int32 and panels.is_cuda and panels.is_contiguous() and panels.numel() == panel_words(M), "panel list of another row count"
+    return panels
+
+
+def drop_panels(scale, block_stride, nblocks, groups, group_rows, M, out=None):
+    lib = load()
+    _dev(scale, torch.float32)
+    assert scale.numel() >= (nblocks - 1) * block_stride + groups
+    if out is None:
+        out = torch.empty((nblocks, panel_words(M)), dtype=torch.int32, device=scale.device)
+    _check(lib.alpro_drop_panels(_ptr(scale), block_stride, nblocks, groups, group_rows, M, _ptr(out), _stream()), "alpro_drop_panels")
+    return out
+
+
+def panels_fill(panels, dst, src=None):
+    lib = load()
+    _dev(dst)
+    M = dst.shape[0]
+    if src is not None:
+        _dev(src, dst.dtype)
+        assert src.shape == dst.shape
+    _check(lib.alpro_panels_fill(_ptr(_panels_ok(panels, M)), M, _ptr(dst), dst.stride(0) * dst.element_size(), _ptr(src),
+                                 src.stride(0) * src.element_size() if src is not None else 0, dst.shape[1] * dst.element_size(), _stream()), "alpro_panels_fill")
+    return dst
 
 
 def gemm_c2_tiled_rows(M, N, K, dtype):
@@ -755,7 +793,7 @@
     return _ptr(ws), _REDUCE_WS_BYTES
 
 
-def gemm_tn_acc(a, b, c, colsum=None, atomic=None):
+def gemm_tn_acc(a, b, c, colsum=None, atomic=None, *, panels=None):
     lib = load()
     _dev(a); _dev(b, a.dtype); _dev(c, torch.float32)
     assert a.shape[0] == b.shape[0] and tuple(c.shape) == (a.shape[1], b.shape[1])
@@ -765,6 +803,11 @@
     M, N, K = a.shape[0], a.shape[1], b.shape[1]
     if atomic is None:
         atomic = not _DETERMINISTIC_WGRAD[0] and M > 65536 and ((N + 255) // 256) * ((K + 255) // 256) > 9
+    if panels is not None:
+        ws = None if atomic else _tn_workspace(a.device, lib.alpro_gemm_tn_workspace_bytes(M, N, K))
+        _check(lib.alpro_gemm_tn_acc_panels(_ptr(a), a.stride(0), _ptr(b), b.stride(0), _ptr(c), c.stride(0), _CODE[a.dtype], M, N, K, _ptr(colsum),
+                                            _ptr(ws), ws.numel() if ws is not None else 0, _ptr(_panels_ok(panels, M)), _stream()), "alpro_gemm_tn_acc_panels")
+        return c
     if atomic:
         _check(lib.alpro_gemm_tn_acc(_ptr(a), a.stride(0), _ptr(b), b.stride(0), _ptr(c), c.stride(0), _CODE[a.dtype], M, N, K, _ptr(colsum), _stream()),
                "alpro_gemm_tn_acc")
diff --git a/alpro_amd/modeling/timesformer/vit.py b/alpro_amd/modeling/timesformer/vit.py
--- a/alpro_amd/modeling/timesformer/vit.py
+++ b/alpro_amd/modeling/timesformer/vit.py
@@ -167,6 +167,8 @@
     fuse_ln_bwd_emit = os.environ.get("ALPRO_FUSE_LN_BWD", "1") != "0"
     fuse_residual_ln = os.environ.get("ALPRO_FUSE_RESIDUAL_LN", "1") != "0"
 
+    drop_compact = os.environ.get("ALPRO_DROP_COMPACT", "1") != "0"
+
     batch_merged_tproj = os.environ.get("ALPRO_BATCH_TPROJ", "1") != "0"
 
     def _bank(self):
@@ -330,6 +332,10 @@
         dev = x.device
         sv = {"x": x, "dims": (B, T, N, S, D, H), "dt": dt}
         sv["drop_t"], sv["drop_s"], sv["drop_m"] = self._drop(B * N, dev), self._drop(B * T, dev), self._drop(B, dev)
+        pan = (getattr(self, "_presampled", None) or {}).pop("panels_m", None)
+        if not (self.drop_compact and dt != torch.float32 and sv["drop_m"] is not None):
+            pan = None
+        sv["panels_m"] = pan
         cside = None
         if rt.cls_precise(dt) and rt.cls_stream(True) and x.is_cuda and self.fuse_residual_ln and self.merge_temporal_proj:
             cside = _ClsSide.get(dev)
@@ -391,10 +397,12 @@
         u, sv["u_tiled"] = tr.gelu_save_buffer(B * S, self.mlp.fc1.out_features, D, dt, dev)
         sv["u_grad"] = tr.SAVE_GELU_GRAD
         f1 = hip.gemm(h2, self._w("fc1", self.mlp.fc1, dt), bias=self.mlp.fc1.bias, act=hip.ACT_GELU_SAVE_GRAD if sv["u_grad"] else hip.ACT_GELU, pre_act=u,
-                      c2_tiled=sv["u_tiled"])
+                      c2_tiled=sv["u_tiled"], panels=pan)
         out = torch.empty_like(x)
         hip.gemm(f1, self._w("fc2", self.mlp.fc2, dt), out=out.view(B * S, D), bias=self.mlp.fc2.bias, out_dtype=torch.float32,
-                 residual=x2.view(B * S, D), row_scale=sv["drop_m"], row_scale_group=S)
+                 residual=x2.view(B * S, D), row_scale=sv["drop_m"], row_scale_group=S, panels=pan)
+        if pan is not None:
+            hip.panels_fill(pan, out.view(B * S, D), x2.view(B * S, D))
         if cside is not None:
             self._cls_side_finish(cside, ev_x2, torch.cuda.current_stream().record_event(), x_cls_in, o_c, B, T, sv["drop_s"], sv["drop_m"], x2[:, 0], out[:, 0])
         elif rt.cls_precise(dt) and self.fuse_residual_ln and self.merge_temporal_proj:
@@ -481,11 +489,14 @@
         fuse = self.fuse_ln_bwd_emit
         if dz is None:
             dz = hip.gather_cast(dx, dt, row_scale=sv["drop_m"], row_scale_group=S)
-        tr.wgrad(dz, sv["f1"], self.mlp.fc2.weight, self.mlp.fc2.bias)
-        du = tr.dgrad(dz, self._wt("fc2", self.mlp.fc2, dt), gelu_pre=sv["u"], gelu_saved_grad=sv.get("u_grad", False), gelu_tiled=sv.get("u_tiled", False))
+        pan = sv.get("panels_m")
+        tr.wgrad(dz, sv["f1"], self.mlp.fc2.weight, self.mlp.fc2.bias, panels=pan)
+        du = tr.dgrad(dz, self._wt("fc2", self.mlp.fc2, dt), gelu_pre=sv["u"], gelu_saved_grad=sv.get("u_grad", False), gelu_tiled=sv.get("u_tiled", False), panels=pan)
         del dz
-        tr.wgrad(du, sv["h2"], self.mlp.fc1.weight, self.mlp.fc1.bias)
-        dh2 = tr.dgrad(du, self._wt("fc1", self.mlp.fc1, dt))
+        tr.wgrad(du, sv["h2"], self.mlp.fc1.weight, self.mlp.fc1.bias, panels=pan)
+        dh2 = tr.dgrad(du, self._wt("fc1", self.mlp.fc1, dt), panels=pan)
+        if pan is not None:
+            hip.panels_fill(pan, dh2)
         g, b_ = tr.grad_buffer(self.norm2.weight, zero=True)[0], tr.grad_buffer(self.norm2.bias, zero=True)[0]
         if fuse:
             _, dpo = hip.layernorm_bwd(dh2, sv["x2"], self.norm2.weight, VIT_EPS, dx, g, b_,
@@ -548,12 +559,18 @@
         _KEEP_CACHE.clear()
         _KEEP_CACHE[key] = keep
     scale = torch.floor(keep + torch.rand(per * len(live), dtype=torch.float32, device=device)) / keep
+    panels = None
+    if Block.drop_compact and scale.is_cuda and rt.compute_dtype() != torch.float32:
+        S = 1 + N * T
+        panels = hip.drop_panels(scale[sizes[0] + sizes[1]:], per, len(live), B, S, B * S)
     off = 0
-    for blk in live:
+    for i, blk in enumerate(live):
         blk._presampled = {}
         for n in sizes:
             blk._presampled[n] = scale[off:off + n]
             off += n
+        if panels is not None:
+            blk._presampled["panels_m"] = panels[i]
 
 
 class _MergedTProjBank:
diff --git a/alpro_amd/modeling/train.py b/alpro_amd/modeling/train.py
--- a/alpro_amd/modeling/train.py
+++ b/alpro_amd/modeling/train.py
@@ -109,7 +109,7 @@
     return torch.as_strided(base, (rows,) + tuple(base.shape[1:]), base.stride())
 
 
-def wgrad(dy_t, x_t, weight, bias, bias_done=False):
+def wgrad(dy_t, x_t, weight, bias, bias_done=False, panels=None):
     if bias_done:
         bias = None
     if bias is not None:
@@ -120,14 +120,17 @@
         from alpro_amd import config as rt
         side = rt.wgrad_side_stream(dy_t.device)
         if side is None:
-            hip.gemm_tn_acc(dy_t, x_t, gw2, colsum=gb if bias is not None else None)
+            hip.gemm_tn_acc(dy_t, x_t, gw2, colsum=gb if bias is not None else None, panels=panels)
             return
         side.wait_stream(torch.cuda.current_stream(dy_t.device))
         with torch.cuda.stream(side):
-            hip.gemm_tn_acc(dy_t, x_t, gw2, colsum=gb if bias is not None else None)
+            hip.gemm_tn_acc(dy_t, x_t, gw2, colsum=gb if bias is not None else None, panels=panels)
+        if panels is not None:
+            panels.record_stream(side)
         dy_t.record_stream(side)
         x_t.record_stream(side)
         return
+    assert panels is None, "panel lists are for the 16-bit weight-gradient kernel"
     dyT = hip.transpose(dy_t, colsum=gb if bias is not None else None)
     hip.gemm(dyT, hip.transpose(x_t), out=gw2, out_dtype=torch.float32, residual=gw2)
 
@@ -143,7 +146,7 @@
     return torch.empty((rows or M, N), dtype=dt, device=device), rows > 0
 
 
-def dgrad(dy_t, wT, out_dtype=None, row_scale=None, row_scale_group=1, gelu_pre=None, gelu_saved_grad=False, gelu_tiled=False):
+def dgrad(dy_t, wT, out_dtype=None, row_scale=None, row_scale_group=1, gelu_pre=None, gelu_saved_grad=False, gelu_tiled=False, panels=None):
     n = dy_t.shape[1]
     w = wT if wT.shape[1] == n else wT[:, :n]
     if not w.is_contiguous() or n % (64 if dy_t.dtype != torch.float32 else 32) != 0:
@@ -152,7 +155,7 @@
         w = wT
     return hip.gemm(dy_t, w, out_dtype=out_dtype or dy_t.dtype, row_scale=row_scale, row_scale_group=row_scale_group,
                     act=(hip.ACT_MUL_SAVED if gelu_saved_grad else hip.ACT_GELU_BWD) if gelu_pre is not None else hip.ACT_NONE, pre_act=gelu_pre,
-                    c2_tiled=gelu_tiled and gelu_saved_grad)
+                    c2_tiled=gelu_tiled and gelu_saved_grad, panels=panels)
 
 
 _LIVE_ANCHORS = weakref.WeakSet()
diff --git a/include/alpro_hip.h b/include/alpro_hip.h
--- a/include/alpro_hip.h
+++ b/include/alpro_hip.h
@@ -181,6 +181,12 @@
 int alpro_gemm_tn_acc_ws(const void* A, int64_t lda, const void* B, int64_t ldb, float* C, int64_t ldc, int dtype, int M,
                          int N, int K, float* colsum, void* workspace, size_t workspace_bytes, void* stream);
 
+int alpro_drop_panels(const float* scale, int64_t block_stride, int nblocks, int groups, int group_rows, int M, int* panels, void* stream);
+int alpro_gemm_panels(const alpro_gemm_desc_t* desc, const int* panels, void* stream);
+int alpro_gemm_tn_acc_panels(const void* A, int64_t lda, const void* B, int64_t ldb, float* C, int64_t ldc, int dtype, int M,
+                             int N, int K, float* colsum, void* workspace, size_t workspace_bytes, const int* panels, void* stream);
+int alpro_panels_fill(const int* panels, int M, void* dst, int64_t ld_dst_bytes, const void* src, int64_t ld_src_bytes, int row_bytes, void* stream);
+
 int alpro_colsum_acc(const void* A, int64_t lda, float* out, int dtype, int M, int N, void* stream);
 
 int alpro_softmax_xent(const float* logits, int64_t ld, const int64_t* labels, int ignore_index, float* loss_rows,
```

Result: no change. 430.4 (-0.7%).
